# psweens/VAN-GAN

Measured on AMD Instinct MI355X. Metric: train Mvoxels/s (VanGan.train_step, 128^3 bf16), higher is better.
Workload: dtype bf16; 1 GPU; VanGan.train_step, 128x128x128 volumes, batch 1 per GPU (global 1), clDice on, disc noise+dropout on; parallelism=dp1

## Files before the change

### van_gan_amd/csrc/vg_c1k3.h

```cpp
#pragma once
#include "vg_common.h"

struct C1K3 {
    const void* x; int x_f32; float sc, sf; int act, pad_mode;
    int D, H, W, C, W4;
    int td0, th0, tw0;
    const void* w; int Ktot, CK;
    const float* bias; void* out; float* sums;
    const void* dy; float* dw; float* db;
    const float* scale; const float* shift;
    VgFin fin;
};
__device__ __forceinline__ int c1_resolve(int p, int n, int reflect, bool& ok) {
    ok = true;
    if (reflect) { if (p < 0) p = -p; if (p >= n) p = 2 * n - 2 - p; return p < 0 ? 0 : (p >= n ? n - 1 : p); }
    ok = p >= 0 && p < n;
    return ok ? p : 0;
}

struct C1M {
    const void* x; int x_f32; float sc, sf; int act, pad_mode;
    const float* scale; const float* shift;
    const void* noise;
    int D, H, W, OD, OH, OW, C;
    int td0, th0, tw0;
    const void* w; int Ktot, CK;
    const float* bias; void* out; float* sums;
    const void* dy; float* dw; float* db; float* part;
    VgFin fin;
};
int c1m_fwd(const vg_conv_desc* d, hipStream_t s);
int c1m_wgrad(const vg_conv_desc* d, const void* dy, int dy_f32, int T_total, float* dw, float* db, float* scratch, int64_t scratch_bytes, hipStream_t s);
```

### van_gan_amd/csrc/vg_c1k3.hip

```cpp
#include "vg_c1k3.h"

namespace {
constexpr int TW = 16, TD = 4;
constexpr int ROWB = TW * 8 + 8;

typedef __attribute__((ext_vector_type(2))) unsigned u32x2;
typedef __attribute__((ext_vector_type(4))) unsigned u32x4;
typedef __attribute__((ext_vector_type(4))) short s16x4;
typedef __attribute__((ext_vector_type(2))) float f32x2;

template <int KS, int ST, int TH> struct Geo {
    static constexpr int IH = ST * TH + KS - ST, ID = ST * TD + KS - ST;
    static constexpr int NROWS = ID * IH, IMGB = NROWS * ROWB;
    static constexpr int NI = 3 * ST + 4;
    static constexpr int NRT = KS * KS;
};

__device__ __forceinline__ float c1_slope(int act) { return act == VG_ACT_RELU ? 0.f : (act == VG_ACT_LRELU ? VG_LRELU : 1.f); }

template <typename S, int KS, int ST, int TH, bool NOISE>
__device__ __forceinline__ void c1_stage_image(const C1M& p, char* img, int n, int od0, int oh0, int ow0, float sc, float sf, float slope, int tid) {
    typedef Geo<KS, ST, TH> G;
    const bool refl = p.pad_mode == VG_PAD_REFLECT;
    for (int item = tid; item < G::NROWS * 4; item += 256) {
// ... 66 lines not shown
        for (int h = 0; h < 2; ++h) {
            const int t = min(8 * s + 2 * kg + h, G::NRT - 1), a = t / KS, b = t - a * KS;
            boff[s][h] = ((ST * wave + a) * G::IH + b) * ROWB + li * 8;
        }
    const int tiles_w = (p.OW + TW - 1) / TW, tiles_h = (p.OH + TH - 1) / TH, tiles_d = (p.OD + TD - 1) / TD;
    const int ntiles = tiles_w * tiles_h * tiles_d;
    float s1[MT][4], s2[MT][4];
#pragma unroll
    for (int mt = 0; mt < MT; ++mt)
#pragma unroll
        for (int r = 0; r < 4; ++r) { s1[mt][r] = 0.f; s2[mt][r] = 0.f; }
    const int cst = 8 * (kg >> 1), jodd = kg & 1;
    const size_t rowpitch = (size_t)p.OW * C;
    for (int tile = blockIdx.x; tile < ntiles; tile += gridDim.x) {
        const int tw = tile % tiles_w, t2 = tile / tiles_w, th = t2 % tiles_h, td = t2 / tiles_h;
        const int od0 = td * TD, oh0 = th * TH, ow0 = tw * TW;
        __syncthreads();
        c1_stage_image<S, KS, ST, TH, NOISE>(p, img, n, od0, oh0, ow0, sc, sf, slope, tid);
        __syncthreads();
        const int od = od0 + wave, ow = ow0 + li;
        const bool dw_ok = od < p.OD && ow < p.OW;
        T* const obase = (T*)p.out + ((((size_t)n * p.OD + min(od, p.OD - 1)) * p.OH + oh0) * p.OW + min(ow, p.OW - 1)) * C + cst;
#pragma unroll
        for (int mt = 0; mt < MT; ++mt) {
            f32x4 acc[8];
#pragma unroll
            for (int j = 0; j < 8; ++j) {
                const int jo = ST * j * ROWB;
                const u32x2 a0 = *(const u32x2*)(img + boff[0][0] + jo), a1 = *(const u32x2*)(img + boff[0][1] + jo);
                const u32x2 c0 = *(const u32x2*)(img + boff[1][0] + jo), c1 = *(const u32x2*)(img + boff[1][1] + jo);
                const bf16x8 b0 = __builtin_bit_cast(bf16x8, ((u32x4){a0[0], a0[1], a1[0], a1[1]}));
                const bf16x8 b1 = __builtin_bit_cast(bf16x8, ((u32x4){c0[0], c0[1], c1[0], c1[1]}));
                acc[j] = VG_MFMA16(wa[mt][0], b0, ((f32x4){0.f, 0.f, 0.f, 0.f}));
                acc[j] = VG_MFMA16(wa[mt][1], b1, acc[j]);
            }
            T* const optr = obase + 16 * mt;
#pragma unroll
            for (int jp = 0; jp < 8; jp += 2) {
                bf16x4 pk[2];
#pragma unroll
                for (int e = 0; e < 2; ++e) {
                    const int j = jp + e;
                    const bool ok = dw_ok && oh0 + j < p.OH;
                    f32x2 v0 = {acc[j][0], acc[j][1]}, v1 = {acc[j][2], acc[j][3]};
                    v0 += eb[mt][0]; v1 += eb[mt][1];
                    pk[e] = (bf16x4){(short)f2bf(v0[0]), (short)f2bf(v0[1]), (short)f2bf(v1[0]), (short)f2bf(v1[1])};
                    f32x2 q0 = {bf2f((bf16_t)pk[e][0]), bf2f((bf16_t)pk[e][1])}, q1 = {bf2f((bf16_t)pk[e][2]), bf2f((bf16_t)pk[e][3])};
                    if (!ok) { q0 = (f32x2){0.f, 0.f}; q1 = q0; }
                    s1[mt][0] += q0[0]; s1[mt][1] += q0[1]; s1[mt][2] += q1[0]; s1[mt][3] += q1[1];
                    s2[mt][0] += q0[0] * q0[0]; s2[mt][1] += q0[1] * q0[1]; s2[mt][2] += q1[0] * q1[0]; s2[mt][3] += q1[1] * q1[1];
                }
                const u32x2 wa_ = __builtin_bit_cast(u32x2, pk[0]), wb_ = __builtin_bit_cast(u32x2, pk[1]);
                const u32x2 x0 = __builtin_amdgcn_permlane16_swap(wa_[0], wb_[0], false, false);
                const u32x2 x1 = __builtin_amdgcn_permlane16_swap(wa_[1], wb_[1], false, false);
                const u32x4 outv = {x0[0], x1[0], x0[1], x1[1]};
                const int j = jp + jodd;
                if (dw_ok && oh0 + j < p.OH) *(u32x4*)(optr + j * rowpitch) = outv;
            }
        }
    }
    if (!p.sums) return;
#pragma unroll
    for (int mt = 0; mt < MT; ++mt)
#pragma unroll
        for (int r = 0; r < 4; ++r) {
            float a = s1[mt][r], b = s2[mt][r];
#pragma unroll
            for (int o = 1; o < 16; o <<= 1) { a += __shfl_xor(a, o); b += __shfl_xor(b, o); }
            if (li == 0) { atomicAdd(&stat[(16 * mt + 4 * kg + r) * 2], a); atomicAdd(&stat[(16 * mt + 4 * kg + r) * 2 + 1], b); }
        }
    __syncthreads();
    if (tid < 32 * MT) {
        const int stripe = blockIdx.x & (VG_STRIPES - 1);
        atomicAdd(&p.sums[((size_t)stripe * gridDim.y + n) * (2 * C) + tid], stat[tid]);
    }
    if (p.fin.ticket) vg_fin_tail(p.fin, p.sums, gridDim.y, C, gridDim.x * gridDim.y, (int*)img);
}

template <typename S, int KS, int ST, int TH, int NT, bool NOISE>
__global__ __launch_bounds__(256, 2) void c1m_wgrad_kernel(const C1M p) {
    typedef bf16_t T;
    typedef Geo<KS, ST, TH> G;
    constexpr int C = 16 * NT, VB = 2 * C;
    constexpr int DYROW = TW * VB, DYB = TD * TH * DYROW;
    constexpr int MTS = (G::NRT + 1 + 3) / 4;
    constexpr int UPT = DYB / 16 / 256;
    static_assert(MTS * NT * 1024 <= DYB, "the accumulator exchange reuses the dY tile");
    __shared__ __attribute__((aligned(16))) char img[G::IMGB + 16];
    __shared__ __attribute__((aligned(16))) char dyt[DYB];
    const int tid = threadIdx.x, lane = tid & 63, wave = __builtin_amdgcn_readfirstlane(tid >> 6);
    const int n = blockIdx.y;
    const float sc = p.scale ? p.scale[n] : p.sc, sf = p.scale ? p.shift[n] : p.sf, slope = c1_slope(p.act);
    if (tid == 0) {
        const unsigned one = f2bf(1.f);
        *(u32x4*)(img + G::IMGB) = (u32x4){one | (one << 16), one | (one << 16), 0u, 0u};
    }
    const int g = lane >> 4, q = (lane >> 2) & 3, pp = lane & 3;
    const int wq = 8 * (g & 1) + q, yq = g >> 1;
    int aoff[MTS], amove[MTS];
#pragma unroll
    for (int mt = 0; mt < MTS; ++mt) {
        const int r = 4 * mt + pp, a = r / KS, b = r - a * KS;
        amove[mt] = r < G::NRT ? 1 : 0;
        aoff[mt] = r < G::NRT ? ((ST * wave + a) * G::IH + ST * yq + b) * ROWB + wq * 8 : (r == G::NRT ? G::IMGB : G::IMGB + 8);
    }
    const int boff = ((wave * TH + yq) * TW + wq) * VB + pp * 8;
    const int tiles_w = (p.OW + TW - 1) / TW, tiles_h = (p.OH + TH - 1) / TH, tiles_d = (p.OD + TD - 1) / TD;
    const int ntiles = tiles_w * tiles_h * tiles_d;
    f32x4 acc[MTS][NT];
#pragma unroll
    for (int mt = 0; mt < MTS; ++mt)
#pragma unroll
        for (int nt = 0; nt < NT; ++nt) acc[mt][nt] = (f32x4){0.f, 0.f, 0.f, 0.f};
    typedef __attribute__((address_space(3))) s16x4 lds_s4;
    for (int tile = blockIdx.x; tile < ntiles; tile += gridDim.x) {
        const int tw = tile % tiles_w, t2 = tile / tiles_w, th = t2 % tiles_h, td = t2 / tiles_h;
        const int od0 = td * TD, oh0 = th * TH, ow0 = tw * TW;
        f32x4 dv[UPT];
#pragma unroll
        for (int i = 0; i < UPT; ++i) {
            const int u = tid + 256 * i, vox = u / (2 * NT), c16 = u - vox * (2 * NT);
            const int w = vox & 15, y = (vox >> 4) % TH, z = vox / (16 * TH);
            const bool ok = od0 + z < p.OD && oh0 + y < p.OH && ow0 + w < p.OW;
            const T* src = (const T*)p.dy + ((((size_t)n * p.OD + min(od0 + z, p.OD - 1)) * p.OH + min(oh0 + y, p.OH - 1)) * p.OW + min(ow0 + w, p.OW - 1)) * C + c16 * 8;
            dv[i] = *(const __attribute__((address_space(1))) f32x4*)(uintptr_t)src;
            if (!ok) dv[i] = (f32x4){0.f, 0.f, 0.f, 0.f};
        }
        __syncthreads();
        c1_stage_image<S, KS, ST, TH, NOISE>(p, img, n, od0, oh0, ow0, sc, sf, slope, tid);
#pragma unroll
        for (int i = 0; i < UPT; ++i) *(f32x4*)(dyt + (tid + 256 * i) * 16) = dv[i];
        __syncthreads();
#pragma unroll
        for (int s = 0; s < TH / 2; ++s) {
            bf16x8 a[MTS];
#pragma unroll
            for (int mt = 0; mt < MTS; ++mt) {
                const int o = aoff[mt] + amove[mt] * (s * 2 * ST * ROWB);
                const s16x4 lo = __builtin_amdgcn_ds_read_tr16_b64_v4i16((lds_s4*)(img + o));
                const s16x4 hi = __builtin_amdgcn_ds_read_tr16_b64_v4i16((lds_s4*)(img + o + amove[mt] * 32));
                a[mt] = (bf16x8){lo[0], lo[1], lo[2], lo[3], hi[0], hi[1], hi[2], hi[3]};
            }
#pragma unroll
            for (int nt = 0; nt < NT; ++nt) {
                const s16x4 lo = __builtin_amdgcn_ds_read_tr16_b64_v4i16((lds_s4*)(dyt + boff + s * 2 * DYROW + nt * 32));
                const s16x4 hi = __builtin_amdgcn_ds_read_tr16_b64_v4i16((lds_s4*)(dyt + boff + s * 2 * DYROW + nt * 32 + 4 * VB));
                const bf16x8 b = {lo[0], lo[1], lo[2], lo[3], hi[0], hi[1], hi[2], hi[3]};
#pragma unroll
                for (int mt = 0; mt < MTS; ++mt) acc[mt][nt] = VG_MFMA16(a[mt], b, acc[mt][nt]);
            }
        }
    }
    float* red = (float*)dyt;
    __syncthreads();
    for (int i = tid; i < MTS * NT * 256; i += 256) red[i] = 0.f;
    __syncthreads();
#pragma unroll
    for (int mt = 0; mt < MTS; ++mt)
#pragma unroll
        for (int nt = 0; nt < NT; ++nt)
#pragma unroll
            for (int e = 0; e < 4; ++e) atomicAdd(&red[((mt * NT + nt) * 4 + e) * 64 + lane], acc[mt][nt][e]);
    __syncthreads();
    float* slab = p.part ? p.part + ((size_t)blockIdx.y * gridDim.x + blockIdx.x) * (KS * KS * KS * C) : nullptr;
    for (int i = tid; i < MTS * NT * 256; i += 256) {
        const int l = i & 63, e = (i >> 6) & 3, t = i >> 8, nt = t % NT, mt = t / NT;
        const int r = 4 * mt + (l >> 4), co = 16 * nt + (l & 15);
        const float v = red[i];
        if (r < G::NRT && e < KS) {
            const int idx = (r * KS + e) * C + co;
            if (slab) slab[idx] = v; else atomicAdd(&p.dw[idx], v);
        } else if (r == G::NRT && e == 0 && p.db) atomicAdd(&p.db[co], v);
    }
}
}

static bool c1m_fill(const vg_conv_desc* d, C1M& p) {
    if (!vg_tune("C1M", 1) || d->f32 || d->out_f32 || d->c_src0 != 1 || d->src1 || d->c_src1 || d->nclass > 1) return false;
    const int KS = d->wpack;
    if (KS != 3 && KS != 4) return false;
    if (d->istr != KS - 2 || d->ntaps != KS * KS || d->Cout != (KS == 3 ? 16 : 64)) return false;
    for (int t = 0; t < KS * KS; ++t)
        if (d->tap_d[t] != d->tap_d[0] + t / KS || d->tap_h[t] != d->tap_h[0] + t % KS || d->tap_w[t] != 0) return false;
    if (d->noise && !(d->noise_pad == 1 && d->pad_mode == VG_PAD_REFLECT)) return false;
    if (d->D < 2 || d->H < 2 || d->W < 2 || d->OD < 1 || d->OH < 1 || d->OW < 1) return false;
    p = C1M{};
    p.x = d->src0; p.x_f32 = d->src_f32; p.sc = 1.f; p.sf = 0.f; p.scale = d->in_scale; p.shift = d->in_shift; p.act = d->act;
    p.pad_mode = d->pad_mode; p.noise = d->noise;
    p.D = d->D; p.H = d->H; p.W = d->W; p.OD = d->OD; p.OH = d->OH; p.OW = d->OW; p.C = d->Cout;
    p.td0 = d->tap_d[0]; p.th0 = d->tap_h[0]; p.tw0 = d->wpack_wmin;
    p.w = d->wpacked; p.CK = d->CK; p.Ktot = ((KS * KS * d->CK + 31) / 32) * 32;
    return true;
}
static dim3 c1m_grid(const C1M& c, int N, int th, int per_cu) {
    const int64_t tiles = (int64_t)((c.OD + TD - 1) / TD) * ((c.OH + th - 1) / th) * ((c.OW + TW - 1) / TW);
    int64_t b = (int64_t)256 * per_cu / (N > 0 ? N : 1);
    if (b > tiles) b = tiles;
    if (b < 1) b = 1;
    return dim3((unsigned)b, (unsigned)N);
}

template <typename S, int KS, int MT>
static void c1m_launch_fwd(const C1M& c, dim3 grid, hipStream_t s) {
    if (c.noise) hipLaunchKernelGGL((c1m_fwd_kernel<S, KS, KS - 2, MT, true>), grid, dim3(256), 0, s, c);
    else hipLaunchKernelGGL((c1m_fwd_kernel<S, KS, KS - 2, MT, false>), grid, dim3(256), 0, s, c);
}
int c1m_fwd(const vg_conv_desc* d, hipStream_t s) {
    C1M c;
    if (!c1m_fill(d, c)) return 1;
    c.bias = d->bias; c.out = d->out; c.sums = d->out_sums; c.fin = vg_fin_of(d);
    const int KS = d->wpack;
    if (vg_dry("c1m_fwd<%s,%d,%d,%d,n%d>", d->src_f32 ? "f32" : "bf16", KS, KS - 2, c.C / 16, c.noise ? 1 : 0)) return VG_OK;
    const dim3 grid = c1m_grid(c, d->N, 8, vg_tune("C1M_FWD_WGS", KS == 3 ? 4 : 2));
    if (KS == 3) { if (d->src_f32) c1m_launch_fwd<float, 3, 1>(c, grid, s); else c1m_launch_fwd<bf16_t, 3, 1>(c, grid, s); }
    else { if (d->src_f32) c1m_launch_fwd<float, 4, 4>(c, grid, s); else c1m_launch_fwd<bf16_t, 4, 4>(c, grid, s); }
    if (c.sums && c.fin.ticket) vg_fin_done = true;
    return vg_check_launch();
}

template <typename S, int KS, int TH, int NT>
static void c1m_launch_wgrad(const C1M& c, dim3 grid, hipStream_t s) {
    if (c.noise) hipLaunchKernelGGL((c1m_wgrad_kernel<S, KS, KS - 2, TH, NT, true>), grid, dim3(256), 0, s, c);
    else hipLaunchKernelGGL((c1m_wgrad_kernel<S, KS, KS - 2, TH, NT, false>), grid, dim3(256), 0, s, c);
}
int c1m_wgrad(const vg_conv_desc* d, const void* dy, int dy_f32, int T_total, float* dw, float* db, float* scratch, int64_t scratch_bytes, hipStream_t s) {
    C1M c;
    if (dy_f32 || !vg_tune("C1M_WGRAD", 1) || !c1m_fill(d, c)) return 1;
    const int KS = d->wpack;
    if (T_total != KS * KS) return 1;
    c.dy = dy; c.dw = dw; c.db = db;
    const int th = KS == 3 ? 8 : 4;
    const dim3 grid = c1m_grid(c, d->N, th, vg_tune("C1M_WGRAD_WGS", KS == 3 ? 2 : 1));
    const int nslab = (int)(grid.x * grid.y), dw_elems = KS * KS * KS * c.C;
    c.part = (nslab > 4 && scratch && (int64_t)nslab * dw_elems * 4 <= scratch_bytes && vg_tune("C1M_WGRAD_PART", 1)) ? scratch : nullptr;
    if (vg_dry("c1m_wgrad<%s,%d,%d,%d,n%d>|part%d", d->src_f32 ? "f32" : "bf16", KS, KS - 2, c.C / 16, c.noise ? 1 : 0, c.part ? 1 : 0)) return VG_OK;
    if (KS == 3) { if (d->src_f32) c1m_launch_wgrad<float, 3, 8, 1>(c, grid, s); else c1m_launch_wgrad<bf16_t, 3, 8, 1>(c, grid, s); }
    else { if (d->src_f32) c1m_launch_wgrad<float, 4, 4, 4>(c, grid, s); else c1m_launch_wgrad<bf16_t, 4, 4, 4>(c, grid, s); }
    if (c.part) vg_launch_reduce_partials(c.part, nslab, dw_elems, dw, s);
    return vg_check_launch();
}

namespace {
__global__ __launch_bounds__(256) void cell_pack_kernel(const float* __restrict__ w, int C, int Ktot, bf16_t* __restrict__ out) {
    const size_t total = (size_t)64 * Ktot;
    for (size_t i = (size_t)blockIdx.x * 256 + threadIdx.x; i < total; i += (size_t)gridDim.x * 256) {
        const int row = (int)(i / Ktot), k = (int)(i % Ktot);
        const int chunk = k / 448, kl = k % 448, tap = kl / 16, ch = chunk * 16 + (kl & 15);
        float v = 0.f;
        if (row < 8 && tap < 27 && ch < C) {
            const int nd = tap / 9, nh = (tap / 3) % 3, nw = tap % 3;
            const int td = ((row >> 2) & 1) + 2 - 2 * nd, th = ((row >> 1) & 1) + 2 - 2 * nh, tw = (row & 1) + 2 - 2 * nw;
            if (td >= 0 && th >= 0 && tw >= 0) v = w[(size_t)((td * 4 + th) * 4 + tw) * C + ch];
        }
        out[i] = f2bf(v);
    }
}
__global__ __launch_bounds__(256) void cells_fold_kernel(const bf16_t* __restrict__ cells, int D, int H, int W, float* __restrict__ dx) {
    const int n = blockIdx.y;
    const int CD = D / 2 + 1, CH = H / 2 + 1, CW = W / 2 + 1;
    const bf16_t* cb = cells + (size_t)n * CD * CH * CW * 16;
    const int64_t total = (int64_t)D * H * W;
    for (int64_t i = (int64_t)blockIdx.x * 256 + threadIdx.x; i < total; i += (int64_t)gridDim.x * 256) {
        const int iw = (int)(i % W); const int64_t r = i / W; const int ih = (int)(r % H), id = (int)(r / H);
        int pd[2], ph[2], pw[2], nd = 1, nh = 1, nw = 1;
        pd[0] = id + 1; ph[0] = ih + 1; pw[0] = iw + 1;
        if (id == 1) pd[nd++] = 0; else if (id == D - 2) pd[nd++] = D + 1;
        if (ih == 1) ph[nh++] = 0; else if (ih == H - 2) ph[nh++] = H + 1;
        if (iw == 1) pw[nw++] = 0; else if (iw == W - 2) pw[nw++] = W + 1;
        float s = 0.f;
        for (int a = 0; a < nd; ++a)
            for (int b = 0; b < nh; ++b)
                for (int c = 0; c < nw; ++c) {
                    const int qd = pd[a], qh = ph[b], qw = pw[c];
                    s += bf2f(cb[(((size_t)(qd >> 1) * CH + (qh >> 1)) * CW + (qw >> 1)) * 16 + ((qd & 1) * 4 + (qh & 1) * 2 + (qw & 1))]);
                }
        dx[(size_t)n * total + i] = s;
    }
}
}

extern "C" int vg_pack_cell_weights(const float* w, int C, void* out, vg_stream_t stream) {
    vg_begin();
    if (!w || !out || C < 16 || (C % 16)) return VG_EINVAL;
    const int Ktot = (C / 16) * 448;
    hipLaunchKernelGGL(cell_pack_kernel, dim3((64 * Ktot + 255) / 256), dim3(256), 0, (hipStream_t)stream, w, C, Ktot, (bf16_t*)out);
    return vg_check_launch();
}
extern "C" int vg_cells_fold(const void* cells, int N, int D, int H, int W, float* dx, vg_stream_t stream) {
    vg_begin();
    if (!cells || !dx || N < 1 || D < 4 || H < 4 || W < 4 || ((D | H | W) & 1)) return VG_EINVAL;
    int64_t b = ((int64_t)D * H * W + 255) / 256;
    if (b > 2047 / N) b = 2047 / N > 0 ? 2047 / N : 1;
    hipLaunchKernelGGL(cells_fold_kernel, dim3((unsigned)b, (unsigned)N), dim3(256), 0, (hipStream_t)stream, (const bf16_t*)cells, D, H, W, dx);
    return vg_check_launch();
}
```

### van_gan_amd/csrc/vg_common.h

```cpp
#pragma once
#include <hip/hip_runtime.h>
#include <stdint.h>
#include "../../include/vangan_hip.h"

typedef __attribute__((ext_vector_type(8))) short bf16x8;
typedef __attribute__((ext_vector_type(4))) short bf16x4;
typedef __attribute__((ext_vector_type(4))) float f32x4;
typedef unsigned short bf16_t;

#define VG_LDS_LIMIT 163840
#define VG_LRELU 0.2f

#ifdef VG_FP16
typedef __attribute__((ext_vector_type(8))) _Float16 vg_h8;
__device__ __forceinline__ float bf2f(bf16_t h) { return (float)__builtin_bit_cast(_Float16, h); }
__device__ __forceinline__ bf16_t f2bf(float f) { return __builtin_bit_cast(unsigned short, (_Float16)f); }
#define VG_MFMA16(a, b, c) __builtin_amdgcn_mfma_f32_16x16x32_f16(__builtin_bit_cast(vg_h8, a), __builtin_bit_cast(vg_h8, b), c, 0, 0, 0)
#define VG_MFMA32(a, b, c) __builtin_amdgcn_mfma_f32_32x32x16_f16(__builtin_bit_cast(vg_h8, a), __builtin_bit_cast(vg_h8, b), c, 0, 0, 0)
#define VG_STORAGE16 "fp16"
#else
__device__ __forceinline__ float bf2f(bf16_t h) { return __uint_as_float(((unsigned)h) << 16); }
__device__ __forceinline__ bf16_t f2bf(float f) {
    __bf16 b = (__bf16)f;
    return __builtin_bit_cast(unsigned short, b);
}
#define VG_MFMA16(a, b, c) __builtin_amdgcn_mfma_f32_16x16x32_bf16(a, b, c, 0, 0, 0)
#define VG_MFMA32(a, b, c) __builtin_amdgcn_mfma_f32_32x32x16_bf16(a, b, c, 0, 0, 0)
#define VG_STORAGE16 "bf16"
#endif
__device__ __forceinline__ float bfround(float f) { return bf2f(f2bf(f)); }

template <typename T> __device__ __forceinline__ void load8(const T* p, float* o);
template <> __device__ __forceinline__ void load8<bf16_t>(const bf16_t* p, float* o) {
    const bf16x8 r = *(const bf16x8*)p;
#pragma unroll
    for (int j = 0; j < 8; ++j) o[j] = bf2f((bf16_t)r[j]);
}
template <> __device__ __forceinline__ void load8<float>(const float* p, float* o) {
    const f32x4 a = *(const f32x4*)p, b = *(const f32x4*)(p + 4);
    o[0] = a[0]; o[1] = a[1]; o[2] = a[2]; o[3] = a[3]; o[4] = b[0]; o[5] = b[1]; o[6] = b[2]; o[7] = b[3];
}
template <typename T> __device__ __forceinline__ void store8(T* p, const float* v);
template <> __device__ __forceinline__ void store8<bf16_t>(bf16_t* p, const float* v) {
    bf16x8 r;
#pragma unroll
    for (int j = 0; j < 8; ++j) r[j] = (short)f2bf(v[j]);
    *(bf16x8*)p = r;
}
template <> __device__ __forceinline__ void store8<float>(float* p, const float* v) {
    *(f32x4*)p = (f32x4){v[0], v[1], v[2], v[3]}; *(f32x4*)(p + 4) = (f32x4){v[4], v[5], v[6], v[7]};
}
template <typename T> __device__ __forceinline__ float ld1(const T* p);
template <> __device__ __forceinline__ float ld1<bf16_t>(const bf16_t* p) { return bf2f(*p); }
template <> __device__ __forceinline__ float ld1<float>(const float* p) { return *p; }
template <typename T> __device__ __forceinline__ void st1(T* p, float v);
template <> __device__ __forceinline__ void st1<bf16_t>(bf16_t* p, float v) { *p = f2bf(v); }
template <> __device__ __forceinline__ void st1<float>(float* p, float v) { *p = v; }
template <typename T> __device__ __forceinline__ float rnd(float v);
template <> __device__ __forceinline__ float rnd<bf16_t>(float v) { return bfround(v); }
template <> __device__ __forceinline__ float rnd<float>(float v) { return v; }

__device__ __forceinline__ float vg_act(float x, int act) {
    if (act == VG_ACT_RELU) return fmaxf(x, 0.f);
    if (act == VG_ACT_LRELU) return x > 0.f ? x : VG_LRELU * x;
    return x;
}
__device__ __forceinline__ float vg_act_grad(float pre, int act) {
    if (act == VG_ACT_RELU) return pre > 0.f ? 1.f : 0.f;
    if (act == VG_ACT_LRELU) return pre > 0.f ? 1.f : VG_LRELU;
    return 1.f;
}

__device__ __forceinline__ float wave_sum(float v) {
#pragma unroll
    for (int o = 32; o > 0; o >>= 1) v += __shfl_xor(v, o);
    return v;
}
__device__ __forceinline__ float wave_min(float v) {
#pragma unroll
    for (int o = 32; o > 0; o >>= 1) v = fminf(v, __shfl_xor(v, o));
    return v;
}
__device__ __forceinline__ float wave_max(float v) {
#pragma unroll
    for (int o = 32; o > 0; o >>= 1) v = fmaxf(v, __shfl_xor(v, o));
    return v;
}

struct VgFin { unsigned* ticket; float count, eps; int njobs; vg_fin_job job[2]; };
static inline VgFin vg_fin_of(const vg_conv_desc* d) {
    VgFin f; f.ticket = nullptr; f.count = 1.f; f.eps = 0.f; f.njobs = 0;
    if (d->fin && d->out_sums) { f.ticket = d->fin->ticket; f.count = d->fin->count; f.eps = d->fin->eps; f.njobs = d->fin->njobs;
                                 f.job[0] = d->fin->job[0]; f.job[1] = d->fin->job[d->fin->njobs > 1 ? 1 : 0]; }
    return f;
}
__device__ __forceinline__ void vg_fin_one(const VgFin& f, float s, float ss, int n, int c) {
    const float mean = s / f.count;
    float var = ss / f.count - mean * mean;
    var = var < 0.f ? 0.f : var;
    const float rstd = rsqrtf(var + f.eps);
    for (int j = 0; j < f.njobs; ++j) {
        const vg_fin_job& q = f.job[j];
        const int cc = q.c_off + c, i = n * q.c_tot + cc;
        float sc = (q.gamma ? q.gamma[cc] : 1.f) * rstd;
        float sh = (q.beta ? q.beta[cc] : 0.f) - mean * sc;
        if (q.mult) { const float m = q.mult[i]; sc *= m; sh *= m; }
        q.scale[i] = sc; q.shift[i] = sh;
        if (q.mean) q.mean[i] = mean;
        if (q.rstd) q.rstd[i] = rstd;
    }
}
__device__ __forceinline__ void vg_fin_tail(const VgFin& f, const float* sums, int N, int C, unsigned nblocks, int* flag) {
    asm volatile("s_waitcnt vmcnt(0)" ::: "memory");
    __syncthreads();
    if (threadIdx.x == 0)
        *flag = __hip_atomic_fetch_add(f.ticket, 1u, __ATOMIC_RELAXED, __HIP_MEMORY_SCOPE_AGENT) == nblocks - 1u ? 1 : 0;
    __syncthreads();
    if (!*flag) return;
    for (int i = threadIdx.x; i < N * C; i += blockDim.x) {
        const int n = i / C, c = i - n * C;
        float s = 0.f, ss = 0.f;
        for (int t = 0; t < VG_STRIPES; ++t) {
            const float* p = sums + (((size_t)t * N + n) * C + c) * 2;
            s += __hip_atomic_load(p, __ATOMIC_RELAXED, __HIP_MEMORY_SCOPE_AGENT);
            ss += __hip_atomic_load(p + 1, __ATOMIC_RELAXED, __HIP_MEMORY_SCOPE_AGENT);
        }
        vg_fin_one(f, s, ss, n, c);
    }
}
int vg_launch_fin(const vg_conv_desc* d, hipStream_t s);
extern thread_local bool vg_fin_done;

int vg_tune(const char* key, int dflt);
bool vg_dry(const char* fmt, ...) __attribute__((format(printf, 1, 2)));
void vg_dry_begin(char* buf, int n);
void vg_dry_end();

bool vg_dry_on();
static inline void vg_begin() { (void)hipGetLastError(); }
static inline int vg_check_launch() {
    hipError_t e = hipGetLastError();
    return e == hipSuccess ? VG_OK : VG_ELAUNCH;
}
int vg_pointwise_conv(const vg_conv_desc* d, hipStream_t s);
int vg_pointwise_wgrad(const vg_conv_desc* d, const void* dy, int dy_f32, int T_total, float* dw, float* db, float* scratch,
                       int64_t scratch_bytes, hipStream_t s);
int vg_wgrad_dma(const vg_conv_desc* d, const void* dy, int dy_f32, const int32_t* tap_idx_host, int T_total, float* dw, float* db,
                 float* scratch, int64_t scratch_bytes, hipStream_t s);
int vg_wgrad_pw_dma(const vg_conv_desc* d, const void* dy, int dy_f32, int T_total, float* dw, float* db, float* scratch,
                    int64_t scratch_bytes, hipStream_t s);
int vg_wgrad_thin(const vg_conv_desc* d, const void* dy, int dy_f32, const int32_t* tap_idx_host, int T_total, float* dw, float* db,
                  float* scratch, int64_t scratch_bytes, hipStream_t s);
int vg_conv_dma(const vg_conv_desc* d, hipStream_t s, bool* did_stats = nullptr);
void vg_launch_reduce_partials(const float* part, int nb, int n, float* dw, hipStream_t s);
static inline int ilog2_exact(int v) { int l = 0; while ((1 << l) < v) ++l; return l; }
static inline int pow2_ceil(int v) { int p = 1; while (p < v) p <<= 1; return p; }
static inline int64_t cdiv64(int64_t a, int64_t b) { return (a + b - 1) / b; }

template <typename T> struct Raw8;
template <> struct Raw8<bf16_t> { bf16x8 v; };
template <> struct Raw8<float> { f32x4 a, b; };
__device__ __forceinline__ void raw_load(Raw8<bf16_t>& r, const bf16_t* p) { r.v = *(const __attribute__((address_space(1))) bf16x8*)(uintptr_t)p; }
__device__ __forceinline__ void raw_load(Raw8<float>& r, const float* p) {
    const __attribute__((address_space(1))) f32x4* q = (const __attribute__((address_space(1))) f32x4*)(uintptr_t)p;
    r.a = q[0]; r.b = q[1];
}
__device__ __forceinline__ void raw_unpack(const Raw8<bf16_t>& r, float* o) {
#pragma unroll
    for (int j = 0; j < 8; ++j) o[j] = bf2f((bf16_t)r.v[j]);
}
__device__ __forceinline__ void raw_unpack(const Raw8<float>& r, float* o) {
    o[0] = r.a[0]; o[1] = r.a[1]; o[2] = r.a[2]; o[3] = r.a[3]; o[4] = r.b[0]; o[5] = r.b[1]; o[6] = r.b[2]; o[7] = r.b[3];
}


__device__ __forceinline__ void raw_pin(Raw8<bf16_t>& r) { asm volatile("" : "+v"(r.v)); }
__device__ __forceinline__ void raw_pin(Raw8<float>& r) { asm volatile("" : "+v"(r.a), "+v"(r.b)); }
__device__ __forceinline__ void raw_mask(Raw8<bf16_t>& r, bool keep) { if (!keep) r.v = (bf16x8){0, 0, 0, 0, 0, 0, 0, 0}; }
__device__ __forceinline__ void raw_mask(Raw8<float>& r, bool keep) { if (!keep) { r.a = (f32x4){0.f, 0.f, 0.f, 0.f}; r.b = r.a; } }

__device__ __forceinline__ float ld_global(const float* p) { return *(const __attribute__((address_space(1))) float*)(uintptr_t)p; }
__device__ __forceinline__ float ld_global(const bf16_t* p) { return bf2f(*(const __attribute__((address_space(1))) bf16_t*)(uintptr_t)p); }
```

### van_gan_amd/csrc/vg_pointwise.hip

```cpp
#include "vg_common.h"
#include "vg_c1k3.h"
#include <stdlib.h>

namespace {

struct PW {
    const void* x; int x_f32;
    const float* scale; const float* shift; int act;
    const void* w; int kc_pad, CK;
    const float* bias;
    void* out; int out_f32, accumulate, tanh_out;
    float* sums;
    const void* dy; int dy_f32;
    float* dw; float* db;
    int N, C; int64_t S;
    VgFin fin;
};

__device__ __forceinline__ float pw_slope(int act) { return act == VG_ACT_RELU ? 0.f : (act == VG_ACT_LRELU ? VG_LRELU : 1.f); }
__device__ __forceinline__ float ld_single(const void* p, int f32, int64_t i) {
    return f32 ? ld_global((const float*)p + i) : ld_global((const bf16_t*)p + i);
}

template <typename T, int G>
// ... 334 lines not shown
                Raw8<bf16_t> t;
                raw_load(t, q);
                raw_mask(t, cok);
                xb[i][ks] = t.v;
            }
        if (p.stamps) { asm volatile("s_waitcnt vmcnt(0)" ::: "memory"); if (lane == 0) p.stamps[((size_t)blockIdx.x * 4 + wave) * 8 + 2] = __builtin_amdgcn_s_memrealtime(); }
        if constexpr (SPLIT == 2) {
            const int PH = p.OH + 2, PW_ = p.OW + 2;
            size_t gi[MS / 2], li[MS / 2], si[MS / 2];
            bool bord[MS / 2];
#pragma unroll
            for (int jh = 0; jh < MS / 2; ++jh) {
                const int fd = fdhw[jh] & 1023, fh = (fdhw[jh] >> 10) & 1023, fw = fdhw[jh] >> 20;
                gi[jh] = ((((size_t)n * (p.OD + 2) + fd + 1) * PH + fh + 1) * PW_ + fw + 1) * p.Cout + chof;
                li[jh] = ((((size_t)n * (p.OD >> 1) + (fd >> 1)) * (p.OH >> 1) + (fh >> 1)) * (p.OW >> 1) + (fw >> 1)) * p.sc0 + chof;
                si[jh] = ovf[jh] * (p.Cout - p.sc0) + chof;
                bord[jh] = fd == 1 || fd == p.OD - 2 || fh == 1 || fh == p.OH - 2 || fw == 1 || fw == p.OW - 2;
            }
            constexpr int C = NB * 16;
            const float slope = pw_slope(p.n_act);
            Raw8<bf16_t> gq[NB][MS / 2], xq[NB][MS / 2];
#pragma unroll
            for (int nb = 0; nb < NB; ++nb)
#pragma unroll
                for (int jh = 0; jh < MS / 2; ++jh) {
                    raw_load(gq[nb][jh], p.ng + gi[jh] + nb * 16);
                    raw_load(xq[nb][jh], nb * 16 < p.sc0 ? p.nx0 + li[jh] + nb * 16 : p.nx1 + si[jh] + (nb * 16 - p.sc0));
                }
#pragma unroll
            for (int nb = 0; nb < NB; ++nb) {
                f32x4 a[MS];
#pragma unroll
                for (int i = 0; i < MS; ++i) {
                    a[i] = (f32x4){0.f, 0.f, 0.f, 0.f};
#pragma unroll
                    for (int ks = 0; ks < KS; ++ks) a[i] = VG_MFMA16(wA[nb][ks], xb[i][ks], a[i]);
                }
                const float* tb = ntab + nb * 16 + chof;
#pragma unroll
                for (int jp = 0; jp < MS; jp += 2) {
                    float o[8];
#pragma unroll
                    for (int i = 0; i < 4; ++i) {
                        const pw_u32x2 x = __builtin_amdgcn_permlane16_swap(__float_as_uint(a[jp][i]), __float_as_uint(a[jp + 1][i]), false, false);
                        o[i] = __uint_as_float(x[0]); o[4 + i] = __uint_as_float(x[1]);
                    }
                    float q[8], xv[8];
                    raw_unpack(gq[nb][jp >> 1], q); raw_unpack(xq[nb][jp >> 1], xv);
                    if (bord[jp >> 1]) {
                        const int fd = fdhw[jp >> 1] & 1023, fh = (fdhw[jp >> 1] >> 10) & 1023, fw = fdhw[jp >> 1] >> 20;
                        vg_reflect_fold8(p.ng + (size_t)n * (p.OD + 2) * PH * PW_ * p.Cout + nb * 16 + chof, p.Cout, p.OD, p.OH, p.OW, fd, fh, fw, q);
                    }
#pragma unroll
                    for (int i = 0; i < 8; ++i) {
                        const float pre = xv[i] * tb[i] + tb[C + i];
                        const float m = (pre > 0.f || p.n_act == VG_ACT_NONE) ? 1.f : slope;
                        o[i] += tb[2 * C + i] * m * q[i] - tb[3 * C + i] - tb[4 * C + i] * xv[i];
                    }
                    split_store(wt, jp, nb, o, oks[jp >> 1], ovf[jp >> 1]);
                }
                __builtin_amdgcn_sched_barrier(0);
            }
            continue;
        }
        f32x4 acc[MS][NB];
#pragma unroll
        for (int i = 0; i < MS; ++i)
#pragma unroll
            for (int nb = 0; nb < NB; ++nb) {
                acc[i][nb] = (f32x4){0.f, 0.f, 0.f, 0.f};
#pragma unroll
                for (int ks = 0; ks < KS; ++ks) acc[i][nb] = VG_MFMA16(wA[nb][ks], xb[i][ks], acc[i][nb]);
            }
#pragma unroll
        for (int jp = 0; jp < MS; jp += 2) {
            const bool ok = oks[jp >> 1];
            const size_t ob = ovs[jp >> 1];
#pragma unroll
            for (int nb = 0; nb < NB; ++nb) {
                if (nb * 16 >= p.Cout) continue;
                bf16_t* optr = p.out + ob + nb * 16;
                pw_u32x4 outv;
                if (ACC) {
                    float o[8];
#pragma unroll
                    for (int i = 0; i < 4; ++i) {
                        const pw_u32x2 x = __builtin_amdgcn_permlane16_swap(__float_as_uint(acc[jp][nb][i] + e_b[nb][i >> 1][i & 1]),
                                                                            __float_as_uint(acc[jp + 1][nb][i] + e_b[nb][i >> 1][i & 1]), false, false);
                        o[i] = __uint_as_float(x[0]); o[4 + i] = __uint_as_float(x[1]);
                    }
                    float q[8]; raw_unpack(oldv[ACC ? jp >> 1 : 0][ACC ? nb : 0], q);
                    if (SPLIT) {
#pragma unroll
                        for (int i = 0; i < 8; ++i) o[i] += q[i];
                        split_store(wt, jp, nb, o, ok, ovf[jp >> 1]);
                        continue;
                    }
                    bf16x8 pk;
#pragma unroll
                    for (int i = 0; i < 8; ++i) pk[i] = (short)f2bf(o[i] + q[i]);
                    outv = __builtin_bit_cast(pw_u32x4, pk);
                } else {
                    bf16x4 pk[2];
#pragma unroll
                    for (int e = 0; e < 2; ++e) {
                        pw_f32x2 v0 = {acc[jp + e][nb][0], acc[jp + e][nb][1]}, v1 = {acc[jp + e][nb][2], acc[jp + e][nb][3]};
                        v0 += e_b[nb][0]; v1 += e_b[nb][1];
                        pk[e] = (bf16x4){(short)f2bf(v0[0]), (short)f2bf(v0[1]), (short)f2bf(v1[0]), (short)f2bf(v1[1])};
                        if (STATS) {
                            const bool okv = vok[jp + e];
#pragma unroll
                            for (int i = 0; i < 4; ++i) {
                                const float qv = okv ? bf2f((bf16_t)pk[e][i]) : 0.f;
                                s1[nb][i] += qv; s2[nb][i] += qv * qv;
                            }
                        }
                    }
                    const pw_u32x2 wa = __builtin_bit_cast(pw_u32x2, pk[0]), wb = __builtin_bit_cast(pw_u32x2, pk[1]);
                    const pw_u32x2 x0 = __builtin_amdgcn_permlane16_swap(wa[0], wb[0], false, false);
                    const pw_u32x2 x1 = __builtin_amdgcn_permlane16_swap(wa[1], wb[1], false, false);
                    outv = (pw_u32x4){x0[0], x1[0], x0[1], x1[1]};
                }
                if (ok) *(pw_u32x4*)optr = outv;
            }
        }
    }
    if (p.stamps && lane == 0) { asm volatile("s_waitcnt vmcnt(0)" ::: "memory"); p.stamps[((size_t)blockIdx.x * 4 + wave) * 8 + 7] = __builtin_amdgcn_s_memrealtime(); }
    if (STATS && p.sums) {
#pragma unroll
        for (int nb = 0; nb < NB; ++nb)
#pragma unroll
            for (int i = 0; i < 4; ++i) {
                float a = s1[nb][i], b = s2[nb][i];
#pragma unroll
                for (int o = 1; o < 16; o <<= 1) { a += __shfl_xor(a, o); b += __shfl_xor(b, o); }
                if (r == 0) { atomicAdd(&stat[(nb * 16 + 4 * kg + i) * 2], a); atomicAdd(&stat[(nb * 16 + 4 * kg + i) * 2 + 1], b); }
            }
        __syncthreads();
        if (tid < NB * 32) {
            const int co = tid >> 1;
            const int stripe = blockIdx.x & (VG_STRIPES - 1);
            if (co < p.Cout) atomicAdd(&p.sums[(((size_t)stripe * gridDim.y + n) * p.Cout + co) * 2 + (tid & 1)], stat[tid]);
        }
        if (p.fin.ticket) vg_fin_tail(p.fin, p.sums, gridDim.y, p.Cout, gridDim.x * gridDim.y, (int*)stat);
    }
}

struct PWW {
    const bf16_t* x0; const bf16_t* x1; int c0, c1, Cin, sh;
    const bf16_t* dy; int Cout;
    int N, ID, IH, IW, OD, OH, OW, istr, SO;
    int gin, roles, rp, vpb;
    float* dw; float* db; float* part; int dw_elems;
};

__global__ __launch_bounds__(256) void pw_wgrad_cc_kernel(const PWW p) {
    __shared__ float red[4 * 64 * 16];
    const int tid = threadIdx.x, n = blockIdx.y;
    const int role = tid & (p.rp - 1), vl = tid / p.rp;
    const bool live = role < p.roles;
    const int rl = live ? role : 0;
    const int cg = rl % p.gin, cob = rl / p.gin, c = cg * 8;
    const bool from0 = c < p.c0;
    const float bmask = cg == 0 ? 1.f : 0.f;
    pw_f32x2 acc[8][8], bs[8];
#pragma unroll
    for (int i = 0; i < 8; ++i) {
        bs[i] = (pw_f32x2){0.f, 0.f};
#pragma unroll
        for (int j = 0; j < 8; ++j) acc[i][j] = (pw_f32x2){0.f, 0.f};
    }
    const int ID2 = p.ID >> p.sh, IH2 = p.IH >> p.sh, IW2 = p.IW >> p.sh;
    const int step = gridDim.x * p.vpb;
    int v = blockIdx.x * p.vpb + vl;
    const int OHW = p.OH * p.OW;
    int od = v / OHW, oh = (v - od * OHW) / p.OW, ow = v - od * OHW - oh * p.OW;
    const int sd = step / OHW, sh_ = (step - sd * OHW) / p.OW, sw = step - sd * OHW - sh_ * p.OW;
    const bf16_t* xb = from0 ? p.x0 + c : p.x1 + (c - p.c0);
    const int cs = from0 ? p.c0 : p.c1, shx = from0 ? p.sh : 0;
    const int XD = from0 ? ID2 : p.ID, XH = from0 ? IH2 : p.IH, XW = from0 ? IW2 : p.IW;
    const bf16_t* yb = p.dy + (size_t)n * p.SO * p.Cout + cob * 16;
    if (live)
    for (; v < p.SO; v += 2 * step) {
        Raw8<bf16_t> xr[2], yr[2][2]; bool okv[2];
#pragma unroll
        for (int k = 0; k < 2; ++k) {
            const int vk = v + k * step;
            okv[k] = vk < p.SO;
            const int dq = okv[k] ? od : 0, hq = okv[k] ? oh : 0, wq = okv[k] ? ow : 0, vq = okv[k] ? vk : 0;
            const size_t xi = (((size_t)n * XD + ((dq * p.istr) >> shx)) * XH + ((hq * p.istr) >> shx)) * XW + ((wq * p.istr) >> shx);
            raw_load(xr[k], xb + xi * cs);
            raw_load(yr[k][0], yb + (size_t)vq * p.Cout);
            raw_load(yr[k][1], yb + (size_t)vq * p.Cout + 8);
            ow += sw; if (ow >= p.OW) { ow -= p.OW; ++oh; }
            oh += sh_; if (oh >= p.OH) { oh -= p.OH; ++od; }
            od += sd;
        }
#pragma unroll
        for (int k = 0; k < 2; ++k) {
            float x[8], y[16];
            raw_unpack(xr[k], x); raw_unpack(yr[k][0], y); raw_unpack(yr[k][1], y + 8);
            pw_f32x2 y2[8];
#pragma unroll
            for (int j = 0; j < 8; ++j) y2[j] = okv[k] ? (pw_f32x2){y[2 * j], y[2 * j + 1]} : (pw_f32x2){0.f, 0.f};
#pragma unroll
            for (int i = 0; i < 8; ++i) {
                const pw_f32x2 xi2 = {x[i], x[i]};
#pragma unroll
                for (int j = 0; j < 8; ++j) acc[i][j] += xi2 * y2[j];
            }
            const pw_f32x2 bm = {bmask, bmask};
#pragma unroll
            for (int j = 0; j < 8; ++j) bs[j] += y2[j] * bm;
        }
    }
    for (int off = 32; off >= p.rp; off >>= 1) {
#pragma unroll
        for (int j = 0; j < 8; ++j) {
            bs[j][0] += __shfl_xor(bs[j][0], off); bs[j][1] += __shfl_xor(bs[j][1], off);
#pragma unroll
            for (int i = 0; i < 8; ++i) { acc[i][j][0] += __shfl_xor(acc[i][j][0], off); acc[i][j][1] += __shfl_xor(acc[i][j][1], off); }
        }
    }
    float* slab = p.part ? p.part + (size_t)(blockIdx.y * gridDim.x + blockIdx.x) * p.dw_elems : nullptr;
    const int lane = tid & 63, wave = tid >> 6;
#pragma unroll
    for (int ch = 0; ch < 9; ++ch) {
        __syncthreads();
        if (lane < p.rp) {
            float* dst = red + (size_t)(wave * p.rp + lane) * 16;
#pragma unroll
            for (int j = 0; j < 8; ++j) {
                const pw_f32x2 val = ch < 8 ? acc[ch < 8 ? ch : 0][j] : bs[j];
                dst[2 * j] = val[0]; dst[2 * j + 1] = val[1];
            }
        }
        __syncthreads();
        for (int o = tid; o < p.rp * 16; o += 256) {
            const int ro = o >> 4, i = o & 15;
            if (ro >= p.roles) continue;
            const float sacc = red[o] + red[p.rp * 16 + o] + red[2 * p.rp * 16 + o] + red[3 * p.rp * 16 + o];
            const int rcg = ro % p.gin, rcob = ro / p.gin, co = rcob * 16 + i;
            if (ch < 8) {
                const size_t idx = (size_t)(rcg * 8 + ch) * p.Cout + co;
                if (slab) slab[idx] = sacc; else atomicAdd(&p.dw[idx], sacc);
            } else if (rcg == 0 && p.db) atomicAdd(&p.db[co], sacc);
        }
    }
}

template <typename T, bool MULTI_X>
__global__ __launch_bounds__(256) void pw_wgrad_kernel(const PW p) {
    __shared__ float part[16 * 256];
    const int n = blockIdx.y, tid = threadIdx.x;
    const int gpc = p.C >> 3, vpb = 256 / gpc;
    const int cg = tid % gpc, vl = tid / gpc;
    const bool live = tid < gpc * vpb;
    float a[8], bsum[8], sc[8], sf[8];
#pragma unroll
    for (int j = 0; j < 8; ++j) {
        a[j] = 0.f; bsum[j] = 0.f;
        const int ci = MULTI_X ? n * p.C + cg * 8 + j : n;
        sc[j] = (p.scale && live) ? p.scale[ci] : 1.f; sf[j] = (p.scale && live) ? p.shift[ci] : 0.f;
    }
    const float slope = pw_slope(p.act);
    const T* mb = (const T*)(MULTI_X ? p.x : p.dy) + (size_t)n * p.S * p.C + cg * 8;
    const void* sb = MULTI_X ? p.dy : p.x;
    const int sb_f32 = MULTI_X ? p.dy_f32 : p.x_f32;
    const int64_t soff = (int64_t)n * p.S;
    const int64_t stride = (int64_t)gridDim.x * vpb;
    if (live)
    for (int64_t v = (int64_t)blockIdx.x * vpb + vl; v < p.S; v += 4 * stride) {
        Raw8<T> m[4]; float sv[4];
#pragma unroll
        for (int k = 0; k < 4; ++k) {
            const int64_t vv = v + k * stride < p.S ? v + k * stride : v;
            raw_load(m[k], mb + vv * p.C);
            sv[k] = ld_single(sb, sb_f32, soff + vv);
        }
#pragma unroll
        for (int k = 0; k < 4; ++k) {
            if (v + k * stride >= p.S) continue;
            float q[8]; raw_unpack(m[k], q);
            if (MULTI_X) {
                const float g = rnd<T>(sv[k]);
#pragma unroll
                for (int j = 0; j < 8; ++j) { float y = q[j] * sc[j] + sf[j]; y = rnd<T>(fmaxf(y, y * slope)); a[j] += y * g; }
                bsum[0] += g;
            } else {
                float y = sv[k] * sc[0] + sf[0]; y = rnd<T>(fmaxf(y, y * slope));
#pragma unroll
                for (int j = 0; j < 8; ++j) { a[j] += y * q[j]; bsum[j] += q[j]; }
            }
        }
    }
#pragma unroll
    for (int j = 0; j < 8; ++j) { part[(2 * j) * 256 + tid] = live ? a[j] : 0.f; part[(2 * j + 1) * 256 + tid] = live ? bsum[j] : 0.f; }
    __syncthreads();
    for (int o = tid; o < p.C * 2; o += 256) {
        const int ch = o >> 1, mom = o & 1, g8 = ch >> 3, j = ch & 7;
        const float* src = part + (2 * j + mom) * 256 + g8;
        float s = 0.f;
        for (int t = 0; t < vpb; ++t) s += src[t * gpc];
        if (mom == 0) atomicAdd(&p.dw[ch], s);
        else if (p.db) {
            if (!MULTI_X) atomicAdd(&p.db[ch], s);
            else if (ch == 0) {
                atomicAdd(&p.db[0], s);
            }
        }
    }
}

template <typename T, typename S, int NA>
__device__ __forceinline__ void c1_window(const C1K3& p, int n, int d, int h, int w0, int a0, float (&xv)[NA][3][6]) {
    const bool refl = p.pad_mode == VG_PAD_REFLECT;
    const float slope = pw_slope(p.act);
    int cw[6]; bool okw[6];
#pragma unroll
    for (int i = 0; i < 6; ++i) cw[i] = c1_resolve(w0 + p.tw0 + i, p.W, refl, okw[i]);
    const int64_t base = (int64_t)n * p.D * p.H * p.W;
#pragma unroll
    for (int a = 0; a < NA; ++a) {
        bool okd; const int rd = c1_resolve(d + p.td0 + a0 + a, p.D, refl, okd);
#pragma unroll
        for (int b = 0; b < 3; ++b) {
            bool okh; const int rh = c1_resolve(h + p.th0 + b, p.H, refl, okh);
            const int64_t row = base + ((int64_t)rd * p.H + rh) * p.W;
#pragma unroll
            for (int i = 0; i < 6; ++i) xv[a][b][i] = ld_global((const S*)p.x + row + cw[i]);
#pragma unroll
            for (int i = 0; i < 6; ++i) {
                float y = xv[a][b][i] * p.sc + p.sf;
                y = rnd<T>(fmaxf(y, y * slope));
                xv[a][b][i] = (okd && okh && okw[i]) ? y : 0.f;
            }
        }
    }
}

template <typename T, typename S>
__global__ __launch_bounds__(256, 3) void c1k3_fwd_kernel(C1K3 p) {
    __shared__ float wl[27 * 32];
    __shared__ float part[16 * 256];
    const int n = blockIdx.y, tid = threadIdx.x;
    const int gpc = p.C >> 3, qpb = 256 / gpc;
    const int cg = tid % gpc, ql = tid / gpc;
    const bool live = tid < gpc * qpb;
    if (p.scale) { p.sc = p.scale[n]; p.sf = p.shift[n]; }
    for (int i = tid; i < 27 * p.C; i += 256) {
        const int co = i % p.C, tj = i / p.C, t = tj / 3, j = tj - t * 3;
        wl[i] = ld1<T>((const T*)p.w + (size_t)co * p.Ktot + t * p.CK + j);
    }
    __syncthreads();
    float bv[8], s1[8], s2[8];
#pragma unroll
    for (int j = 0; j < 8; ++j) { bv[j] = (live && p.bias) ? p.bias[cg * 8 + j] : 0.f; s1[j] = 0.f; s2[j] = 0.f; }
    const int64_t nq = (int64_t)p.D * p.H * p.W4;
    if (live)
    for (int64_t q = (int64_t)blockIdx.x * qpb + ql; q < nq; q += (int64_t)gridDim.x * qpb) {
        const int wq = (int)(q % p.W4); const int64_t r = q / p.W4;
        const int h = (int)(r % p.H), d = (int)(r / p.H), w0 = wq * 4;
        float acc[4][8];
#pragma unroll
        for (int v = 0; v < 4; ++v)
#pragma unroll
            for (int j = 0; j < 8; ++j) acc[v][j] = bv[j];
#pragma unroll 1
        for (int a = 0; a < 3; ++a) {
            float xv[1][3][6];
            c1_window<T, S, 1>(p, n, d, h, w0, a, xv);
#pragma unroll
            for (int b = 0; b < 3; ++b)
#pragma unroll
                for (int j = 0; j < 3; ++j) {
                    const float* wp = wl + ((a * 3 + b) * 3 + j) * p.C + cg * 8;
                    const f32x4 w0v = *(const f32x4*)wp, w1v = *(const f32x4*)(wp + 4);
#pragma unroll
                    for (int v = 0; v < 4; ++v) {
                        const float x = xv[0][b][v + j];
                        acc[v][0] += x * w0v[0]; acc[v][1] += x * w0v[1]; acc[v][2] += x * w0v[2]; acc[v][3] += x * w0v[3];
                        acc[v][4] += x * w1v[0]; acc[v][5] += x * w1v[1]; acc[v][6] += x * w1v[2]; acc[v][7] += x * w1v[3];
                    }
                }
        }
        T* ob = (T*)p.out + (((size_t)n * p.D + d) * p.H + h) * p.W * p.C + cg * 8;
#pragma unroll
        for (int v = 0; v < 4; ++v) {
            if (w0 + v >= p.W) continue;
            store8<T>(ob + (size_t)(w0 + v) * p.C, acc[v]);
#pragma unroll
            for (int j = 0; j < 8; ++j) { const float rr = rnd<T>(acc[v][j]); s1[j] += rr; s2[j] += rr * rr; }
        }
    }
    if (!p.sums) return;
#pragma unroll
    for (int j = 0; j < 8; ++j) { part[(2 * j) * 256 + tid] = live ? s1[j] : 0.f; part[(2 * j + 1) * 256 + tid] = live ? s2[j] : 0.f; }
    __syncthreads();
    const int stripe = blockIdx.x & (VG_STRIPES - 1);
    float* dst = p.sums + ((size_t)stripe * gridDim.y + n) * p.C * 2;
    for (int o = tid; o < p.C * 2; o += 256) {
// ... 47 lines not shown
                for (int c = 0; c < 8; ++c) acc[72 + c] += g[c];
            }
        }
    }
#pragma unroll
    for (int chunk = 0; chunk < 4; ++chunk) {
        __syncthreads();
#pragma unroll
        for (int i = 0; i < 20; ++i) part[i * 256 + tid] = live ? acc[chunk * 20 + i] : 0.f;
        __syncthreads();
        for (int o = tid; o < roles * 20; o += 256) {
            const int i = o / roles, ro = o - i * roles;
            const float* src = part + i * 256 + ro;
            float sacc = 0.f;
            for (int t = 0; t < qpb; ++t) sacc += src[t * roles];
            const int val = chunk * 20 + i, rcg = ro % gpc, ra = ro / gpc;
            if (val < 72) {
                const int b = val / 24, j = (val / 8) % 3, c = val & 7;
                atomicAdd(&p.dw[(size_t)(((ra * 3 + b) * 3) + j) * p.C + rcg * 8 + c], sacc);
            } else if (ra == 0 && p.db) atomicAdd(&p.db[rcg * 8 + (val - 72)], sacc);
        }
    }
}

bool c1k3_fill(const vg_conv_desc* d, C1K3& p) {
    if (d->c_src0 != 1 || d->src1 || d->c_src1 || d->wpack != 3 || d->ntaps != 9 || d->istr != 1 || d->noise || d->nclass > 1) return false;
    if (d->Cout < 8 || d->Cout > 32 || (d->Cout % 8)) return false;
    if (d->OD != d->D || d->OH != d->H || d->OW != d->W) return false;
    for (int t = 0; t < 9; ++t)
        if (d->tap_d[t] != d->tap_d[0] + t / 3 || d->tap_h[t] != d->tap_h[0] + t % 3 || d->tap_w[t] != 0) return false;
    p.x = d->src0; p.x_f32 = d->src_f32; p.sc = 1.f; p.sf = 0.f; p.scale = d->in_scale; p.shift = d->in_shift; p.act = d->act;
    p.pad_mode = d->pad_mode; p.D = d->D; p.H = d->H; p.W = d->W; p.C = d->Cout; p.W4 = (d->W + 3) / 4;
    p.td0 = d->tap_d[0]; p.th0 = d->tap_h[0]; p.tw0 = d->wpack_wmin;
    p.CK = d->CK; p.Ktot = ((9 * d->CK + 31) / 32) * 32;
    return true;
}

bool pw_enabled() { return vg_tune("PW", 1) != 0; }
bool pw_shape_ok(const vg_conv_desc* d) {
    if (!pw_enabled() || d->ntaps != 1 || d->tap_d[0] || d->tap_h[0] || d->tap_w[0]) return false;
    if (d->istr != 1 || d->src1 || d->c_src1 || d->src0_shift || d->noise || d->wpack || d->nclass > 1) return false;
    if (d->OD != d->D || d->OH != d->H || d->OW != d->W) return false;
    return true;
}
int pw_blocks(int64_t work_items, int N) {
    int64_t b = (work_items + 255) / 256;
    const int64_t cap = 2047 / (N > 0 ? N : 1);
    if (b > cap) b = cap;
    return b < 1 ? 1 : (int)b;
}

template <bool GEO, bool ACC, bool STATS>
bool pwg_launch(int KS, int NB, dim3 grid, hipStream_t s, const PWG& p) {
#define PWG_CASE(ks, nb) if (KS == ks && NB == nb) { hipLaunchKernelGGL((pw_gemm_kernel<ks, nb, GEO, ACC, STATS>), grid, dim3(256), 0, s, p); return true; }
    PWG_CASE(1, 1) PWG_CASE(1, 2) PWG_CASE(1, 3) PWG_CASE(1, 4) PWG_CASE(1, 6) PWG_CASE(2, 1) PWG_CASE(2, 2) PWG_CASE(3, 2)
    PWG_CASE(4, 4) PWG_CASE(6, 4) PWG_CASE(2, 8)
#undef PWG_CASE
    return false;
}
template <int SPLIT>
bool pwg_launch_split(int KS, int NB, dim3 grid, hipStream_t s, const PWG& p) {
#define PWG_CASE(ks, nb) if (KS == ks && NB == nb) { hipLaunchKernelGGL((pw_gemm_kernel<ks, nb, false, true, false, SPLIT>), grid, dim3(256), 0, s, p); return true; }
    PWG_CASE(1, 3) PWG_CASE(1, 6) PWG_CASE(2, 6)
#undef PWG_CASE
    return false;
}
bool pwg_case_ok(int KS, int NB) {
    static const int tab[][2] = {{1, 1}, {1, 2}, {1, 3}, {1, 4}, {1, 6}, {2, 1}, {2, 2}, {3, 2}, {4, 4}, {6, 4}, {2, 8}};
    for (auto& t : tab) if (t[0] == KS && t[1] == NB) return true;
    return false;
}
int pw_gemm_conv(const vg_conv_desc* d, hipStream_t s) {
    if (!pw_enabled() || !vg_tune("PW_GEMM", 1)) return 1;
    if (d->ntaps != 1 || d->tap_d[0] || d->tap_h[0] || d->tap_w[0] || d->noise || d->wpack || d->nclass > 1) return 1;
    if (d->f32 || d->src_f32 || d->out_f32 || d->in_scale || d->act != VG_ACT_NONE || d->res || d->tanh_out) return 1;
    const int Cin = d->c_src0 + d->c_src1;
    if (Cin < 8 || (Cin % 8) || (d->c_src1 && (d->c_src0 % 8)) || d->Cout < 16 || (d->Cout % 16) || (d->CK % 8)) return 1;
    if (d->c_src1 && !d->src1) return 1;
    if (d->src0_shift && ((d->D | d->H | d->W) & 1)) return 1;
    if (d->istr < 1 || d->ostr < 1 || (d->OD - 1) * d->istr >= d->D || (d->OH - 1) * d->istr >= d->H || (d->OW - 1) * d->istr >= d->W) return 1;
    if (d->accumulate && d->out_sums) return 1;
    const int64_t SO = (int64_t)d->OD * d->OH * d->OW;
    if (SO < 1 || SO > (1 << 30)) return 1;
    const int KS = (Cin + 31) / 32, NB = d->Cout / 16;
    if (!pwg_case_ok(KS, NB)) return 1;
    const bool geo = d->src0_shift || d->istr != 1 || d->ostr != 1 || d->ooff_d || d->ooff_h || d->ooff_w || d->BD != d->OD || d->BH != d->OH
                     || d->BW != d->OW || d->OD != d->D || d->OH != d->H || d->OW != d->W;
    PWG p = {};
    p.x0 = (const bf16_t*)d->src0; p.x1 = (const bf16_t*)(d->c_src1 ? d->src1 : d->src0); p.c0 = d->c_src0; p.c1 = d->c_src1 ? d->c_src1 : 1;
    p.Cin = Cin; p.sh = d->src0_shift ? 1 : 0;
    p.w = (const bf16_t*)d->wpacked; p.CK = d->CK; p.kc_pad = ((d->CK + 31) / 32) * 32; p.Ktot = ((Cin + d->CK - 1) / d->CK) * p.kc_pad;
    p.bias = d->bias; p.out = (bf16_t*)d->out; p.sums = d->out_sums;
    p.N = d->N; p.ID = d->D; p.IH = d->H; p.IW = d->W; p.OD = d->OD; p.OH = d->OH; p.OW = d->OW; p.istr = d->istr;
    p.BD = d->BD; p.BH = d->BH; p.BW = d->BW; p.ostr = d->ostr; p.od0 = d->ooff_d; p.oh0 = d->ooff_h; p.ow0 = d->ooff_w;
    p.Cout = d->Cout; p.SO = (int)SO; p.stamps = g_vg_stamps;
    p.fin = vg_fin_of(d);
    const int MS = (KS * NB <= 2) ? 4 : 2;
    const int64_t nwt = (SO + MS * 16 - 1) / (MS * 16);
    int64_t b = (nwt + 3) / 4;
    const int capt = vg_tune("PW_GEMM_CAP", 2047);
    const int64_t cap = (capt / d->N) > 0 ? (capt / d->N) : 1;
    if (b > cap) b = cap;
    const dim3 grid((int)b, d->N);
    if (vg_dry("pw_gemm<%d,%d,g%d,a%d>", KS, NB, (geo || !d->accumulate) ? 1 : 0, d->accumulate ? 1 : 0)) return VG_OK;
    bool ok;
    if (!d->accumulate) { ok = pwg_launch<true, false, true>(KS, NB, grid, s, p); if (ok && p.sums && p.fin.ticket) vg_fin_done = true; }
    else ok = geo ? pwg_launch<true, true, false>(KS, NB, grid, s, p) : pwg_launch<false, true, false>(KS, NB, grid, s, p);
    return ok ? vg_check_launch() : 1;
}

int pw_gemm_split(const vg_conv_desc* d, const vg_actnorm_bwd_desc* nb_, void* dlow, void* dskip, int c_low, int acc, hipStream_t s) {
    if (!pw_enabled() || !vg_tune("PW_GEMM", 1) || !vg_tune("PW_SPLIT", 1)) return 1;
    if (d->ntaps != 1 || d->tap_d[0] || d->tap_h[0] || d->tap_w[0] || d->noise || d->wpack || d->nclass > 1) return 1;
    if (d->f32 || d->src_f32 || d->out_f32 || d->in_scale || d->act != VG_ACT_NONE || d->res || d->tanh_out || d->out_sums || d->bias) return 1;
    const int Cin = d->c_src0;
    if (d->c_src1 || d->src0_shift || Cin < 8 || (Cin % 8) || d->Cout < 32 || (d->Cout % 16) || (d->CK % 8) || (!d->accumulate && !nb_)) return 1;
    if (nb_) {
        if (!nb_->norm || !nb_->g_padded || nb_->f32 || nb_->x_f32 || !nb_->g || !nb_->x || !nb_->x1 || !nb_->x0_shift || nb_->c_x0 != c_low) return 1;
        if (nb_->C != d->Cout || nb_->N != d->N || nb_->D != d->D || nb_->H != d->H || nb_->W != d->W || !nb_->gamma || !nb_->mean || !nb_->rstd || !nb_->red) return 1;
        if (d->D < 4 || d->H < 4 || d->W < 4 || d->D > 1023 || d->H > 1023 || d->W > 1023) return 1;
    }
    if (c_low < 16 || (c_low % 16) || c_low >= d->Cout) return 1;
    if (d->istr != 1 || d->ostr != 1 || d->ooff_d || d->ooff_h || d->ooff_w || d->BD != d->OD || d->BH != d->OH || d->BW != d->OW
        || d->OD != d->D || d->OH != d->H || d->OW != d->W || ((d->D | d->H | d->W) & 1)) return 1;
    const int64_t SO = (int64_t)d->OD * d->OH * d->OW;
    if (SO < 8 || SO > (1 << 30)) return 1;
    const int KS = (Cin + 31) / 32, NB = d->Cout / 16;
    if (!((KS == 1 && (NB == 3 || NB == 6)) || (KS == 2 && NB == 6))) return 1;
    PWG p = {};
    p.x0 = (const bf16_t*)d->src0; p.x1 = p.x0; p.c0 = Cin; p.c1 = 1; p.Cin = Cin; p.sh = 0;
    p.w = (const bf16_t*)d->wpacked; p.CK = d->CK; p.kc_pad = ((d->CK + 31) / 32) * 32; p.Ktot = ((Cin + d->CK - 1) / d->CK) * p.kc_pad;
    p.bias = nullptr; p.out = (bf16_t*)d->out; p.sums = nullptr;
    p.N = d->N; p.ID = d->D; p.IH = d->H; p.IW = d->W; p.OD = d->OD; p.OH = d->OH; p.OW = d->OW; p.istr = 1;
    p.BD = d->BD; p.BH = d->BH; p.BW = d->BW; p.ostr = 1;
    p.Cout = d->Cout; p.SO = (int)SO; p.stamps = g_vg_stamps;
    p.dlow = (bf16_t*)dlow; p.dskip = (bf16_t*)dskip; p.sc0 = c_low; p.sacc = acc;
    if (nb_) {
        p.ng = (const bf16_t*)nb_->g; p.nx0 = (const bf16_t*)nb_->x; p.nx1 = (const bf16_t*)nb_->x1;
        p.n_scale = nb_->scale; p.n_shift = nb_->shift; p.n_mean = nb_->mean; p.n_rstd = nb_->rstd; p.n_gamma = nb_->gamma; p.n_mult = nb_->mult;
        p.n_red = nb_->red; p.n_dgamma = (nb_->dgamma && nb_->dbeta) ? nb_->dgamma : nullptr; p.n_dbeta = nb_->dbeta; p.n_act = nb_->act;
    }
    const int MS = (KS * NB <= 2) ? 4 : 2;
    const int64_t nwt = (SO + MS * 16 - 1) / (MS * 16);
    int64_t b = (nwt + 3) / 4;
    const int capt = vg_tune("PW_GEMM_CAP", 2047);
    const int64_t cap = (capt / d->N) > 0 ? (capt / d->N) : 1;
    if (b > cap) b = cap;
    if (vg_dry("pw_gemm_split<%d,%d,n%d>", KS, NB, nb_ ? 1 : 0)) return VG_OK;
    const bool ok = nb_ ? pwg_launch_split<2>(KS, NB, dim3((int)b, d->N), s, p) : pwg_launch_split<1>(KS, NB, dim3((int)b, d->N), s, p);
    return ok ? vg_check_launch() : 1;
}

int pw_wgrad_cc(const vg_conv_desc* d, const void* dy, int dy_f32, int T_total, float* dw, float* db, float* scratch,
                int64_t scratch_bytes, hipStream_t s) {
    if (!pw_enabled() || !vg_tune("PW_WGRAD_CC", 1)) return 1;
    if (T_total != 1 || d->ntaps != 1 || d->tap_d[0] || d->tap_h[0] || d->tap_w[0] || d->noise || d->wpack || d->nclass > 1) return 1;
    if (d->f32 || d->src_f32 || dy_f32 || d->in_scale || d->act != VG_ACT_NONE) return 1;
    const int Cin = d->c_src0 + d->c_src1;
    if (Cin < 8 || (Cin % 8) || (d->c_src1 && (d->c_src0 % 8)) || d->Cout < 16 || (d->Cout % 16)) return 1;
    if (d->c_src1 && !d->src1) return 1;
    if (d->src0_shift && ((d->D | d->H | d->W) & 1)) return 1;
    if (d->istr < 1 || (d->OD - 1) * d->istr >= d->D || (d->OH - 1) * d->istr >= d->H || (d->OW - 1) * d->istr >= d->W) return 1;
    const int64_t SO = (int64_t)d->OD * d->OH * d->OW;
    if (SO < 1 || SO > (1 << 30)) return 1;
    PWW p = {};
    p.gin = Cin / 8; p.roles = p.gin * (d->Cout / 16);
    if (p.roles > vg_tune("PW_WGRAD_ROLES", 16)) return 1;
    p.rp = pow2_ceil(p.roles); p.vpb = 256 / p.rp;
    p.x0 = (const bf16_t*)d->src0; p.x1 = (const bf16_t*)(d->c_src1 ? d->src1 : d->src0); p.c0 = d->c_src0; p.c1 = d->c_src1 ? d->c_src1 : 1;
    p.Cin = Cin; p.sh = d->src0_shift ? 1 : 0; p.dy = (const bf16_t*)dy; p.Cout = d->Cout;
    p.N = d->N; p.ID = d->D; p.IH = d->H; p.IW = d->W; p.OD = d->OD; p.OH = d->OH; p.OW = d->OW; p.istr = d->istr; p.SO = (int)SO;
    p.dw = dw; p.db = db; p.dw_elems = Cin * d->Cout;
    int64_t b = (SO + (int64_t)p.vpb * 8 - 1) / ((int64_t)p.vpb * 8);
    const int capt = vg_tune("PW_WGRAD_CAP", 511);
    const int64_t cap = (capt / d->N) > 0 ? (capt / d->N) : 1;
    if (b > cap) b = cap;
    if (b < 1) b = 1;
    const int nslab = (int)b * d->N;
    p.part = (nslab > 4 && scratch && (int64_t)nslab * p.dw_elems * 4 <= scratch_bytes) ? scratch : nullptr;
    if (vg_dry("pw_wgrad_cc<r%d>|part%d", p.roles, p.part ? 1 : 0)) return VG_OK;
    hipLaunchKernelGGL(pw_wgrad_cc_kernel, dim3((int)b, d->N), dim3(256), 0, s, p);
    if (p.part) vg_launch_reduce_partials(p.part, nslab, p.dw_elems, dw, s);
    return vg_check_launch();
}

}

extern "C" int vg_shortcut_dgrad_concat(const vg_conv_desc* d, void* dlow, void* dskip, int c_low, int accumulate, vg_stream_t stream) {
    vg_begin();
    if (!d || !d->src0 || !d->out || !d->wpacked || !dlow || !dskip) return VG_EINVAL;
    return pw_gemm_split(d, nullptr, dlow, dskip, c_low, accumulate, (hipStream_t)stream);
}
extern "C" int vg_shortcut_dgrad_concat_norm(const vg_conv_desc* d, const vg_actnorm_bwd_desc* b, void* dlow, void* dskip, int c_low,
                                             int accumulate, vg_stream_t stream) {
    vg_begin();
    if (!d || !b || !d->src0 || !d->wpacked || !dlow || !dskip) return VG_EINVAL;
    if (!vg_tune("PW_SPLIT_NORM", 1)) return 1;
    return pw_gemm_split(d, b, dlow, dskip, c_low, accumulate, (hipStream_t)stream);
}

int vg_pointwise_conv(const vg_conv_desc* d, hipStream_t s) {
    if (pw_enabled() && !d->res && !d->tanh_out && !d->accumulate && d->ostr == 1 && !d->ooff_d && !d->ooff_h && !d->ooff_w
        && d->BD == d->OD && d->BH == d->OH && d->BW == d->OW && !(d->out_f32 && !d->f32)) {
        { const int mrc = c1m_fwd(d, s); if (mrc <= 0) return mrc; }
        C1K3 c;
        if (c1k3_fill(d, c)) {
            c.w = d->wpacked; c.bias = d->bias; c.out = d->out; c.sums = d->out_sums;
            c.fin = vg_fin_of(d);
            const int qpb = 256 / (c.C >> 3);
            int64_t b = ((int64_t)c.D * c.H * c.W4 + qpb - 1) / qpb;
            const int64_t cap = (2047 / d->N) > 0 ? (2047 / d->N) : 1;
            if (b > cap) b = cap;
            const dim3 grid((int)b, d->N);
            if (vg_dry("c1k3_fwd<%s,%s>", d->f32 ? "f32" : "bf16", d->src_f32 ? "f32" : "bf16")) return VG_OK;
            if (d->f32) {
                if (d->src_f32) hipLaunchKernelGGL((c1k3_fwd_kernel<float, float>), grid, dim3(256), 0, s, c);
                else hipLaunchKernelGGL((c1k3_fwd_kernel<float, bf16_t>), grid, dim3(256), 0, s, c);
            } else {
                if (d->src_f32) hipLaunchKernelGGL((c1k3_fwd_kernel<bf16_t, float>), grid, dim3(256), 0, s, c);
                else hipLaunchKernelGGL((c1k3_fwd_kernel<bf16_t, bf16_t>), grid, dim3(256), 0, s, c);
            }
            if (c.sums && c.fin.ticket) vg_fin_done = true;
            return vg_check_launch();
        }
    }
    { const int grc = pw_gemm_conv(d, s); if (grc <= 0) return grc; }
    if (!pw_shape_ok(d) || d->res) return 1;
    if (d->ostr != 1 || d->ooff_d || d->ooff_h || d->ooff_w || d->BD != d->OD || d->BH != d->OH || d->BW != d->OW) return 1;
    if (d->tanh_out && d->accumulate) return 1;
    const int Cin = d->c_src0;
    PW p = {};
    p.x = d->src0; p.x_f32 = d->src_f32; p.scale = d->in_scale; p.shift = d->in_shift; p.act = d->act;
    p.w = d->wpacked; p.CK = d->CK; p.kc_pad = ((d->CK + 31) / 32) * 32;
    p.bias = d->bias; p.out = d->out; p.out_f32 = (d->out_f32 || d->f32) ? 1 : 0; p.accumulate = d->accumulate; p.tanh_out = d->tanh_out;
    p.sums = d->out_sums; p.N = d->N; p.S = (int64_t)d->D * d->H * d->W;
    if (d->Cout == 1 && Cin >= 8 && Cin <= 32 && (Cin % 8) == 0) {
        p.C = Cin;
        const dim3 grid(pw_blocks((p.S + 1) / 2, d->N), d->N);
        if (vg_dry("pw_cto1<%s,%d>", d->f32 ? "f32" : "bf16", Cin / 8 > 4 ? 4 : Cin / 8)) return VG_OK;
#define PW_CTO1(T)                                                                                                      \
        switch (Cin / 8) {                                                                                              \
            case 1: hipLaunchKernelGGL((pw_cto1_kernel<T, 1>), grid, dim3(256), 0, s, p); break;                        \
            case 2: hipLaunchKernelGGL((pw_cto1_kernel<T, 2>), grid, dim3(256), 0, s, p); break;                        \
            case 3: hipLaunchKernelGGL((pw_cto1_kernel<T, 3>), grid, dim3(256), 0, s, p); break;                        \
            default: hipLaunchKernelGGL((pw_cto1_kernel<T, 4>), grid, dim3(256), 0, s, p); break;                       \
        }
        if (d->f32) { PW_CTO1(float) } else { PW_CTO1(bf16_t) }
#undef PW_CTO1
        return vg_check_launch();
    }
    if (Cin == 1 && d->Cout >= 8 && d->Cout <= 256 && (d->Cout % 8) == 0 && !d->tanh_out && !(d->out_f32 && !d->f32)) {
        p.C = d->Cout;
        p.kc_pad = ((d->CK + 31) / 32) * 32;
        const int vpb = 256 / (p.C >> 3);
        const dim3 grid(pw_blocks((p.S + 3) / 4 * (256 / vpb), d->N), d->N);
        if (vg_dry("pw_1toc<%s>", d->f32 ? "f32" : "bf16")) return VG_OK;
        p.fin = vg_fin_of(d);
        if (d->f32) hipLaunchKernelGGL((pw_1toc_kernel<float>), grid, dim3(256), 0, s, p);
        else hipLaunchKernelGGL((pw_1toc_kernel<bf16_t>), grid, dim3(256), 0, s, p);
        if (p.sums && p.fin.ticket) vg_fin_done = true;
        return vg_check_launch();
    }
    if ((Cin == 8 || Cin == 16) && d->Cout >= 16 && d->Cout <= 128 && (d->Cout % 8) == 0 && !d->in_scale && d->act == VG_ACT_NONE
        && !d->tanh_out && !d->out_sums && !d->src_f32 && !(d->out_f32 && !d->f32)) {
        p.C = d->Cout;
        const int nchunks = (Cin + d->CK - 1) / d->CK;
        const int Ktot = nchunks * p.kc_pad;
        const int vpb = 256 / (p.C >> 3);
        const dim3 grid(pw_blocks((p.S + 1) / 2 * (256 / vpb), d->N), d->N);
        if (vg_dry("pw_ctoc<%s,%d>", d->f32 ? "f32" : "bf16", Cin / 8)) return VG_OK;
        if (d->f32) {
            if (Cin == 8) hipLaunchKernelGGL((pw_ctoc_kernel<float, 1>), grid, dim3(256), 0, s, p, Cin, Ktot);
            else hipLaunchKernelGGL((pw_ctoc_kernel<float, 2>), grid, dim3(256), 0, s, p, Cin, Ktot);
        } else {
            if (Cin == 8) hipLaunchKernelGGL((pw_ctoc_kernel<bf16_t, 1>), grid, dim3(256), 0, s, p, Cin, Ktot);
            else hipLaunchKernelGGL((pw_ctoc_kernel<bf16_t, 2>), grid, dim3(256), 0, s, p, Cin, Ktot);
        }
        return vg_check_launch();
    }
    return 1;
}

int vg_pointwise_wgrad(const vg_conv_desc* d, const void* dy, int dy_f32, int T_total, float* dw, float* db, float* scratch,
                       int64_t scratch_bytes, hipStream_t s) {
    if (pw_enabled()) { const int mrc = c1m_wgrad(d, dy, dy_f32, T_total, dw, db, scratch, scratch_bytes, s); if (mrc <= 0) return mrc; }
    if (pw_enabled() && T_total == 9 && !(dy_f32 && !d->f32)) {
        C1K3 c;
        if (c1k3_fill(d, c)) {
            c.dy = dy; c.dw = dw; c.db = db;
            const int qpb = 256 / (3 * (c.C >> 3));
            int64_t b = ((int64_t)c.D * c.H * c.W4 + (int64_t)qpb * 8 - 1) / ((int64_t)qpb * 8);
            const int64_t cap = (767 / d->N) > 0 ? (767 / d->N) : 1;
            if (b > cap) b = cap;
            if (b < 1) b = 1;
            const dim3 grid((int)b, d->N);
            if (vg_dry("c1k3_wgrad<%s,%s>", d->f32 ? "f32" : "bf16", d->src_f32 ? "f32" : "bf16")) return VG_OK;
            if (d->f32) {
                if (d->src_f32) hipLaunchKernelGGL((c1k3_wgrad_kernel<float, float>), grid, dim3(256), 0, s, c);
                else hipLaunchKernelGGL((c1k3_wgrad_kernel<float, bf16_t>), grid, dim3(256), 0, s, c);
            } else {
                if (d->src_f32) hipLaunchKernelGGL((c1k3_wgrad_kernel<bf16_t, float>), grid, dim3(256), 0, s, c);
                else hipLaunchKernelGGL((c1k3_wgrad_kernel<bf16_t, bf16_t>), grid, dim3(256), 0, s, c);
            }
            return vg_check_launch();
        }
    }
    { const int wrc = pw_wgrad_cc(d, dy, dy_f32, T_total, dw, db, scratch, scratch_bytes, s); if (wrc <= 0) return wrc; }
    if (!pw_shape_ok(d) || T_total != 1) return 1;
    const int Cin = d->c_src0;
    PW p = {};
    p.x = d->src0; p.x_f32 = d->src_f32; p.scale = d->in_scale; p.shift = d->in_shift; p.act = d->act;
    p.dy = dy; p.dy_f32 = dy_f32; p.dw = dw; p.db = db; p.N = d->N; p.S = (int64_t)d->D * d->H * d->W;
    const bool c_to_1 = d->Cout == 1 && Cin >= 8 && Cin <= 256 && (Cin % 8) == 0;
    const bool one_to_c = Cin == 1 && d->Cout >= 8 && d->Cout <= 256 && (d->Cout % 8) == 0 && !(dy_f32 && !d->f32);
    if (!c_to_1 && !one_to_c) return 1;
    p.C = c_to_1 ? Cin : d->Cout;
    const int vpb = 256 / (p.C >> 3);
    int64_t b = (p.S + (int64_t)vpb * 16 - 1) / ((int64_t)vpb * 16);
    const int64_t cap = (511 / d->N) > 0 ? (511 / d->N) : 1;
    if (b > cap) b = cap;
    if (b < 1) b = 1;
    const dim3 grid((int)b, d->N);
    if (vg_dry("pw_wgrad<%s,%s>", d->f32 ? "f32" : "bf16", c_to_1 ? "cto1" : "1toc")) return VG_OK;
    if (c_to_1) {
        if (d->f32) hipLaunchKernelGGL((pw_wgrad_kernel<float, true>), grid, dim3(256), 0, s, p);
        else hipLaunchKernelGGL((pw_wgrad_kernel<bf16_t, true>), grid, dim3(256), 0, s, p);
    } else {
        if (d->f32) hipLaunchKernelGGL((pw_wgrad_kernel<float, false>), grid, dim3(256), 0, s, p);
        else hipLaunchKernelGGL((pw_wgrad_kernel<bf16_t, false>), grid, dim3(256), 0, s, p);
    }
    return vg_check_launch();
}
```

### van_gan_amd/csrc/vg_wgrad.hip

```cpp
#include "vg_gather.h"

struct WgradK {
    const void* dy; int dy_f32; int Cout;
    int OD, OH, OW;
    int CIB, COB, ncib, ncob, tpg, ntg;
    int tap_src[VG_MAX_TAPS];
    float* dw; float* db;
    int total_tiles, DYS;
    float* part; int dw_elems;
};

#ifndef VG_WGRAD_UB
#define VG_WGRAD_UB (NOISE ? VG_WGRAD_UBN : (RMAX * Q > 4 ? 2 : 4))
#endif
#ifndef VG_WGRAD_UBN
#define VG_WGRAD_UBN 4
#endif
#ifndef VG_WGRAD_2W
#define VG_WGRAD_2W 16
#endif
typedef __attribute__((address_space(3))) bf16x4 lds_bf16x4;
#define VG_WSTAMP(slot) do { if (g.stamps && tid == 0 && it < 8) g.stamps[((size_t)blockIdx.y * gridDim.x + blockIdx.x) * 64 + it * 8 + (slot)] = __builtin_readcyclecounter(); } while (0)

__device__ __forceinline__ bf16x8 tr_frag(const char* base0, const char* base1) {
    bf16x4 lo = __builtin_amdgcn_ds_read_tr16_b64_v4i16((lds_bf16x4*)base0);
    bf16x4 hi = __builtin_amdgcn_ds_read_tr16_b64_v4i16((lds_bf16x4*)base1);
    return (bf16x8){lo[0], lo[1], lo[2], lo[3], hi[0], hi[1], hi[2], hi[3]};
}

template <typename T, int RMAX, int Q, bool NOISE>
__global__ __launch_bounds__(256, (RMAX * Q >= VG_WGRAD_2W ? 2 : 3)) void wgrad_kernel(const GatherIn g, const WgradK p) {
    constexpr bool F32 = sizeof(T) == 4;
    extern __shared__ __attribute__((aligned(16))) char smem[];
    const int tid = threadIdx.x, lane = tid & 63;
    const int wave = __builtin_amdgcn_readfirstlane(tid >> 6);
    const int lg = lane >> 4, li = lane & 15;
    int by = blockIdx.y;
    const int cob = by % p.ncob; by /= p.ncob;
    const int cib = by % p.ncib; const int tg = by / p.ncib;
    const int tap0 = tg * p.tpg;
    const int ntap_here = min(p.tpg, g.ntaps - tap0);
    const int tci = p.CIB >> 4;
    const int nrows = ntap_here * tci;

    const int BM = 1 << (g.tdl + g.thl + g.twl);
    char* halo = smem;
    const int hbytes = g.planar ? (g.CK >> 3) * g.PSB : g.HD * g.DS;
    char* dyt = smem + hbytes;
    const int dybytes = BM * p.DYS;
    int* tapoff = (int*)(dyt + dybytes);
    int* tapsrc = tapoff + 64;
    float* scs = (float*)((char*)tapoff + 512);
    int* utab = (int*)(scs + 2 * g.CK);
    int* rtab = utab + 2 * stage_ncols(g);
    const int RTN = 3 * stage_axis_len(g);
    int* ktab = rtab + 2 * RTN;

    if (tid < g.ntaps)
        tapoff[tid] = (g.td[tid] - g.tmin_d) * g.DS + ((g.th[tid] - g.tmin_h) * g.HWp + halo_pos_w(g, g.tw[tid] - g.tmin_w)) * g.VS;
    if (tid < VG_MAX_TAPS) tapsrc[tid] = p.tap_src[tid];
    build_column_table(g, utab, tid);
    if ((int)blockIdx.x < p.total_tiles) {
        int t2 = blockIdx.x % (g.tiles_d * g.tiles_h * g.tiles_w);
        const int fw_i = t2 % g.tiles_w; t2 /= g.tiles_w;
        const int fh_i = t2 % g.tiles_h;
        stage_resolve_axes(g, rtab, fh_i << g.thl, fw_i << g.twl, tid);
    }
    if constexpr (!F32) {
        const int TWm_ = (1 << g.twl) - 1, THm_ = (1 << g.thl) - 1;
        for (int e = tid; e < (BM / 32) * 64; e += 256) {
            const int ks = e >> 6, l2 = e & 63, lg2 = l2 >> 4, li2 = l2 & 15;
            const int m0 = ks * 32 + 8 * lg2 + (li2 >> 2), m1 = m0 + 4;
            const int w0 = m0 & TWm_, h0 = (m0 >> g.twl) & THm_, d0 = m0 >> (g.twl + g.thl);
            const int w1 = m1 & TWm_, h1 = (m1 >> g.twl) & THm_, d1 = m1 >> (g.twl + g.thl);
            const int lo = ((li2 & 3) >> 1) * g.CS + 8 * (li2 & 1);
            ktab[2 * e] = d0 * g.istr * g.DS + (h0 * g.istr * g.HWp + w0) * g.VS + lo;
            ktab[2 * e + 1] = d1 * g.istr * g.DS + (h1 * g.istr * g.HWp + w1) * g.VS + lo;
        }
    }
    __syncthreads();

    int aoff[RMAX];
#pragma unroll
    for (int j = 0; j < RMAX; ++j) {
        const int r = wave + 4 * j;
        const int rr = r < nrows ? r : 0;
        aoff[j] = tapoff[tap0 + rr / tci] + (rr % tci) * 2 * g.CS;
    }
    f32x4 acc[RMAX][Q];
#pragma unroll
    for (int j = 0; j < RMAX; ++j)
#pragma unroll
        for (int q = 0; q < Q; ++q) acc[j][q] = (f32x4){0.f, 0.f, 0.f, 0.f};
    float dbsum = 0.f;
    int cur_n = -1;

    const int TWm = (1 << g.twl) - 1, THm = (1 << g.thl) - 1;
    const int tiles_per_n = g.tiles_d * g.tiles_h * g.tiles_w;
    constexpr int gcol = (Q * 16) >> 3, gcol_l = Q == 1 ? 1 : (Q == 2 ? 2 : 3);
    const bool do_db = p.db && cib == 0 && tg == 0;

    int it = -1;
    int gs_w, gs_h, gs_d, gs_n;
    { int t = gridDim.x; gs_w = t % g.tiles_w; t /= g.tiles_w; gs_h = t % g.tiles_h; t /= g.tiles_h; gs_d = t % g.tiles_d; gs_n = t / g.tiles_d; }
    int ti_w, ti_h, ti_d, ti_n;
    { int t = blockIdx.x; ti_w = t % g.tiles_w; t /= g.tiles_w; ti_h = t % g.tiles_h; t /= g.tiles_h; ti_d = t % g.tiles_d; ti_n = t / g.tiles_d; }
    for (int tile = blockIdx.x; tile < p.total_tiles; tile += gridDim.x) {
        ++it;
        VG_WSTAMP(0);
        const int n = ti_n;
        const int od0 = ti_d << g.tdl, oh0 = ti_h << g.thl, ow0 = ti_w << g.twl;
        ti_w += gs_w; if (ti_w >= g.tiles_w) { ti_w -= g.tiles_w; ++ti_h; }
        ti_h += gs_h; if (ti_h >= g.tiles_h) { ti_h -= g.tiles_h; ++ti_d; }
        ti_d += gs_d; if (ti_d >= g.tiles_d) { ti_d -= g.tiles_d; ++ti_n; }
        ti_n += gs_n;
        __syncthreads();
        if (n != cur_n) {
            stage_scale_shift(g, scs, n, cib, tid);
            cur_n = n;
            __syncthreads();
        }
        int* rt = rtab + (it & 1) * RTN;
        Raw8<T> yraw[4]; float y1[4]; bool yok[4];
        const bool dy_on = !(g.dbg & 2) || tile == (int)blockIdx.x;
        if (dy_on) {
#pragma unroll
            for (int k = 0; k < 4; ++k) {
                const int u = min(tid + k * 256, BM * gcol - 1);
                const int m = u >> gcol_l, cg = u & (gcol - 1);
                const int w = m & TWm, h = (m >> g.twl) & THm, d = m >> (g.twl + g.thl);
                const int od = od0 + d, oh = oh0 + h, ow = ow0 + w;
                const int c = cob * p.COB + cg * 8;
                yok[k] = od < p.OD && oh < p.OH && ow < p.OW && c < p.Cout;
                const size_t vox = yok[k] ? ((size_t)(n * p.OD + od) * p.OH + oh) * p.OW + ow : 0;
                if (p.Cout == 1) y1[k] = p.dy_f32 ? ld_global((const float*)p.dy + vox) : ld_global((const bf16_t*)p.dy + vox);
                else raw_load(yraw[k], (const T*)p.dy + vox * p.Cout + (yok[k] ? c : 0));
            }
        }
        if (!(g.dbg & 1) || tile == (int)blockIdx.x) stage_halo_tile<T, NOISE, VG_WGRAD_UB>(g, halo, scs, utab, rt, n, od0, cib, tid);
        if (tile + (int)gridDim.x < p.total_tiles) {
            stage_resolve_axes(g, rtab + ((it + 1) & 1) * RTN, ti_h << g.thl, ti_w << g.twl, tid);
        }
        if (dy_on) {
#pragma unroll
            for (int k = 0; k < 4; ++k) {
                const int u = tid + k * 256;
                if (u < BM * gcol) {
                    const int m = u >> gcol_l, cg = u & (gcol - 1);
                    T* dst = (T*)(dyt + (size_t)m * p.DYS) + cg * 8;
                    if (p.Cout == 1) {
                        const float v[8] = {yok[k] ? y1[k] : 0.f, 0.f, 0.f, 0.f, 0.f, 0.f, 0.f, 0.f};
                        store8<T>(dst, v);
                    } else {
                        raw_mask(yraw[k], yok[k]);
                        *(Raw8<T>*)dst = yraw[k];
                    }
                }
            }
        }
        VG_WSTAMP(1);
        __syncthreads();
        VG_WSTAMP(2);
        if (do_db) {
            const int nrg = 256 / p.COB;
            if (tid < nrg * p.COB) {
                const int c = tid % p.COB;
                float s = 0.f;
                for (int m = tid / p.COB; m < BM; m += nrg) s += ld1<T>((const T*)(dyt + (size_t)m * p.DYS) + c);
                dbsum += s;
            }
        }
        if (g.dbg & 4) continue;
        if constexpr (F32) {
            for (int s = 0; s < BM / 4; ++s) {
                const int m0 = s * 4 + lg;
                const int w0 = m0 & TWm, h0 = (m0 >> g.twl) & THm, d0 = m0 >> (g.twl + g.thl);
                const int r0 = d0 * g.istr * g.DS + (h0 * g.istr * g.HWp + w0) * g.VS + (li >> 3) * g.CS + (li & 7) * 4;
                const char* y0 = dyt + (size_t)m0 * p.DYS + li * 4;
                float b[Q];
#pragma unroll
                for (int q = 0; q < Q; ++q) b[q] = *(const float*)(y0 + q * 64);
#pragma unroll
                for (int j = 0; j < RMAX; ++j) {
                    const float a = *(const float*)(halo + r0 + aoff[j]);
#pragma unroll
                    for (int q = 0; q < Q; ++q) acc[j][q] = __builtin_amdgcn_mfma_f32_16x16x4f32(a, b[q], acc[j][q], 0, 0, 0);
                }
            }
        } else {
            constexpr int RC = RMAX <= 8 ? RMAX : 6;
            static_assert(RMAX % RC == 0, "rows per wave must be a multiple of the chunk");
            constexpr int NCH = RMAX / RC;
            const int nks = BM / 32;
            const int2* kt = (const int2*)ktab + lane;
            const char* ybase = dyt + (size_t)(8 * lg + (li >> 2)) * p.DYS + 8 * (li & 3);
            const int ystep = 32 * p.DYS, y4 = 4 * p.DYS;
            bf16x8 A[2][RC], B[2][Q];
            {
                const int2 r = kt[0];
#pragma unroll
                for (int q = 0; q < Q; ++q) B[0][q] = tr_frag(ybase + q * 32, ybase + y4 + q * 32);
#pragma unroll
                for (int j = 0; j < RC; ++j) A[0][j] = tr_frag(halo + r.x + aoff[j], halo + r.y + aoff[j]);
            }
            for (int ks = 0; ks < nks; ks += 2) {
#pragma unroll
                for (int u = 0; u < 2; ++u) {
                    const int2 rc = kt[(ks + u) * 64];
                    const int kn = min(ks + u + 1, nks - 1);
                    const int2 rn = kt[kn * 64];
                    const char* yn = ybase + (size_t)kn * ystep;
#pragma unroll
                    for (int c = 0; c < NCH; ++c) {
                        constexpr int dummy = 0; (void)dummy;
                        const int s = (u * NCH + c) & 1;
                        if (c + 1 < NCH) {
#pragma unroll
                            for (int j = 0; j < RC; ++j) A[s ^ 1][j] = tr_frag(halo + rc.x + aoff[(c + 1) * RC + j], halo + rc.y + aoff[(c + 1) * RC + j]);
                        } else {
#pragma unroll
                            for (int q = 0; q < Q; ++q) B[u ^ 1][q] = tr_frag(yn + q * 32, yn + y4 + q * 32);
#pragma unroll
                            for (int j = 0; j < RC; ++j) A[s ^ 1][j] = tr_frag(halo + rn.x + aoff[j], halo + rn.y + aoff[j]);
                        }
                        __builtin_amdgcn_sched_barrier(0);
#pragma unroll
                        for (int j = 0; j < RC; ++j)
#pragma unroll
                            for (int q = 0; q < Q; ++q)
                                acc[c * RC + j][q] = VG_MFMA16(A[s][j], B[u][q], acc[c * RC + j][q]);
                        __builtin_amdgcn_sched_barrier(0);
                    }
                }
            }
        }
        VG_WSTAMP(3);
    }
    { const int it = 7; VG_WSTAMP(7); }
#pragma unroll
    for (int j = 0; j < RMAX; ++j) {
        const int r = wave + 4 * j;
        if (r >= nrows) continue;
        const int tap = tap0 + r / tci, ci0 = cib * p.CIB + (r % tci) * 16 + 4 * lg;
#pragma unroll
        for (int q = 0; q < Q; ++q) {
            const int co = cob * p.COB + q * 16 + li;
            if (co >= p.Cout) continue;
#pragma unroll
            for (int e = 0; e < 4; ++e)
                if (ci0 + e < g.Cw) {
                    const size_t i = ((size_t)tapsrc[tap] * g.Cw + ci0 + e) * p.Cout + co;
                    if (p.part) p.part[(size_t)blockIdx.x * p.dw_elems + i] = acc[j][q][e];
                    else atomicAdd(&p.dw[i], acc[j][q][e]);
                }
        }
    }
    if (do_db) {
        __syncthreads();
        float* red = (float*)halo;
        if (tid < p.COB) red[tid] = 0.f;
        __syncthreads();
        if (tid < (256 / p.COB) * p.COB) atomicAdd(&red[tid % p.COB], dbsum);
        __syncthreads();
        if (tid < p.COB) {
            const int co = cob * p.COB + tid;
            if (co < p.Cout) atomicAdd(&p.db[co], red[tid]);
        }
    }
}

__global__ __launch_bounds__(256) void reduce_partials_kernel(const float* part, int nb, int n, float* dw) {
    __shared__ float sm[4][64];
    const int lane = threadIdx.x & 63, w = threadIdx.x >> 6;
    const int i = blockIdx.x * 64 + lane;
    float s = 0.f;
    if (i < n) {
        int b = w;
        for (; b + 28 < nb; b += 32) {
            float v[8];
#pragma unroll
            for (int k = 0; k < 8; ++k) v[k] = part[(size_t)(b + 4 * k) * n + i];
#pragma unroll
            for (int k = 0; k < 8; ++k) s += v[k];
        }
        for (; b < nb; b += 4) s += part[(size_t)b * n + i];
    }
    sm[w][lane] = s;
    __syncthreads();
    if (w == 0 && i < n) atomicAdd(&dw[i], sm[0][lane] + sm[1][lane] + sm[2][lane] + sm[3][lane]);
}

void vg_launch_reduce_partials(const float* part, int nb, int n, float* dw, hipStream_t s) {
    hipLaunchKernelGGL(reduce_partials_kernel, dim3((n + 63) / 64), dim3(256), 0, s, part, nb, n, dw);
}

template <typename T, int RMAX, int Q, bool NOISE>
static void launch_wgrad2(const GatherIn& g, const WgradK& k, dim3 grid, int lds, hipStream_t s) {
    static bool attr_set = false;
    if (!attr_set) {
        (void)hipFuncSetAttribute((const void*)wgrad_kernel<T, RMAX, Q, NOISE>, hipFuncAttributeMaxDynamicSharedMemorySize, VG_LDS_LIMIT);
        attr_set = true;
    }
    hipLaunchKernelGGL((wgrad_kernel<T, RMAX, Q, NOISE>), grid, dim3(256), lds, s, g, k);
}
template <typename T, int RMAX, int Q>
static void launch_wgrad(const GatherIn& g, const WgradK& k, dim3 grid, int lds, hipStream_t s) {
    if (g.noise) launch_wgrad2<T, RMAX, Q, true>(g, k, grid, lds, s); else launch_wgrad2<T, RMAX, Q, false>(g, k, grid, lds, s);
}

extern "C" int vg_conv3d_wgrad(const vg_conv_desc* d, const void* dy, int dy_f32, const int32_t* tap_idx_host,
                               int T_total, float* dw, float* db, float* scratch, int64_t scratch_bytes,
                               vg_stream_t stream) {
    vg_begin();
    if (!d || !dy || !dw || !tap_idx_host) return VG_EINVAL;
    if (d->Cout < 1 || (d->Cout != 1 && (d->Cout % 8))) return VG_EINVAL;
    if (dy_f32 && d->Cout != 1 && !d->f32) return VG_EINVAL;
    if (d->src0 && tap_idx_host[0] == 0) {
        const int wrc = vg_wgrad_pw_dma(d, dy, dy_f32, T_total, dw, db, scratch, scratch_bytes, (hipStream_t)stream);
        if (wrc <= 0) return wrc;
        const int prc = vg_pointwise_wgrad(d, dy, dy_f32, T_total, dw, db, scratch, scratch_bytes, (hipStream_t)stream);
        if (prc <= 0) return prc;
    }
    {
        const int trc = vg_wgrad_thin(d, dy, dy_f32, tap_idx_host, T_total, dw, db, scratch, scratch_bytes, (hipStream_t)stream);
        if (trc <= 0) return trc;
    }
    {
        const int drc = vg_wgrad_dma(d, dy, dy_f32, tap_idx_host, T_total, dw, db, scratch, scratch_bytes, (hipStream_t)stream);
        if (drc <= 0) return drc;
    }
    const int Cin = d->c_src0 + d->c_src1;
    const int Cinp = ((Cin + 15) / 16) * 16, Coutp = ((d->Cout + 15) / 16) * 16;
    const int COB = Coutp >= 64 ? 64 : (Coutp >= 32 ? 32 : 16);
    if (Coutp % COB) return VG_EINVAL;
    const int Q = COB / 16;
    int RMAX = Q == 1 ? 24 : (Q == 2 ? 12 : 6);
    const int esz = d->f32 ? 4 : 2;
    GatherIn g; WgradK k;
    int max_bm = vg_tune("WGRAD_BM", 256), max_cib = vg_tune("WGRAD_CIB", 64);
    if (d->ntaps >= 64 && max_cib > 16 && vg_tune("WGRAD_CIB16_K4", 1)) max_cib = 16;
    const bool k3_all_taps = d->ntaps == 27 && Coutp >= 32 && !d->f32 && vg_tune("WGRAD_CIB16", 1);
    if (k3_all_taps && max_cib > 16) max_cib = 16;
    int best_bm = 0, best_cib = 0, best_lds = 0;
    for (int pass = 0; pass < 2 && !best_bm; ++pass) {
        const int limit = pass == 0 ? vg_tune("WGRAD_LDS0", 80 * 1024) : VG_LDS_LIMIT;
        for (int bm = 256; bm >= 64 && !best_bm; bm = bm == 256 ? 128 : bm - 64)
            for (int c = max_cib; c >= 16; c -= 16) {
                if (Cinp % c) continue;
                if (bm == 256 && (Q > 2 || max_bm < 256)) continue;
                int rc = fill_gather(d, g, c, bm, d->f32 ? 0 : 64);
                if (rc != VG_OK) return rc;
                const int lds = halo_bytes(g) + bm * (COB * esz + 16) + 512 + 2 * c * 4 + stage_table_ints(g) * 4 + (bm / 32) * 512;
                if (lds <= limit) { best_bm = bm; best_cib = c; best_lds = lds; break; }
            }
    }
    if (!best_bm) return VG_ELDS;
    const int CIB = best_cib, lds = best_lds;
    int rc = fill_gather(d, g, CIB, best_bm, d->f32 ? 0 : 64);
    if (rc != VG_OK) return rc;
    k.DYS = COB * esz + 16;
    k.dy = dy; k.dy_f32 = dy_f32; k.Cout = d->Cout; k.OD = d->OD; k.OH = d->OH; k.OW = d->OW;
    k.CIB = CIB; k.COB = COB; k.ncib = Cinp / CIB; k.ncob = Coutp / COB;
    const int rows_per_tap = CIB / 16;
    if (Q == 4 && k3_all_taps && CIB == 16) RMAX = 7;
    k.tpg = (4 * RMAX) / rows_per_tap; if (k.tpg < 1) return VG_EINVAL;
    if (k.tpg > d->ntaps) k.tpg = d->ntaps;
    k.ntg = (d->ntaps + k.tpg - 1) / k.tpg;
    k.tpg = (d->ntaps + k.ntg - 1) / k.ntg;
    for (int i = 0; i < VG_MAX_TAPS; ++i) k.tap_src[i] = i < d->ntaps ? tap_idx_host[i] : 0;
    k.dw = dw; k.db = db;
    k.total_tiles = d->N * g.tiles_d * g.tiles_h * g.tiles_w;
    const int by = k.ntg * k.ncib * k.ncob;
    const int wg_env = vg_tune("WGRAD_WGS", 0);
    const int rw_ = (k.tpg * rows_per_tap + 3) / 4;
    const int rmax_sel = d->f32 ? RMAX : (rw_ <= 2 ? 2 : (rw_ <= 8 && Q <= 2 ? 8 : (Q == 4 && rw_ == 7 ? 7 : RMAX)));
    int per_cu = (rmax_sel * Q >= VG_WGRAD_2W) ? 2 : 3;
    if (VG_LDS_LIMIT / lds < per_cu) per_cu = VG_LDS_LIMIT / lds;
    if (per_cu < 1) per_cu = 1;
    const int wg_target = wg_env > 0 ? wg_env : (256 * per_cu < 384 ? 256 * per_cu : 384);
    int bx = wg_target / by; if (bx < 1) bx = 1; if (bx > k.total_tiles) bx = k.total_tiles;
    k.dw_elems = T_total * (d->wpack ? d->wpack : Cin) * d->Cout;
    k.part = nullptr;
    if (bx > 8 && scratch && (int64_t)bx * k.dw_elems * 4 <= scratch_bytes) k.part = scratch;
    const dim3 grid(bx, by, 1);
    hipStream_t s = (hipStream_t)stream;
    const int rw = (k.tpg * rows_per_tap + 3) / 4;
    {
        const int rsel = d->f32 ? RMAX : (rw <= 2 ? 2 : ((rw <= 8 && Q <= 2) ? 8 : (Q == 4 && rw == 7 ? 7 : RMAX)));
        if (vg_dry("wgrad<%s,%d,%d,n%d>|bm%d|cib%d|part%d|walk%d", d->f32 ? "f32" : "bf16", rsel, Q, g.noise ? 1 : 0, best_bm, CIB,
                   k.part ? 1 : 0, k.total_tiles > bx ? 1 : 0)) return VG_OK;
    }
    if (d->f32) {
        if (Q == 1) launch_wgrad<float, 24, 1>(g, k, grid, lds, s);
        else if (Q == 2) launch_wgrad<float, 12, 2>(g, k, grid, lds, s);
        else launch_wgrad<float, 6, 4>(g, k, grid, lds, s);
    } else if (Q == 1) {
        if (rw <= 2) launch_wgrad<bf16_t, 2, 1>(g, k, grid, lds, s);
        else if (rw <= 8) launch_wgrad<bf16_t, 8, 1>(g, k, grid, lds, s);
        else launch_wgrad<bf16_t, 24, 1>(g, k, grid, lds, s);
    } else if (Q == 2) {
        if (rw <= 2) launch_wgrad<bf16_t, 2, 2>(g, k, grid, lds, s);
        else if (rw <= 8) launch_wgrad<bf16_t, 8, 2>(g, k, grid, lds, s);
        else launch_wgrad<bf16_t, 12, 2>(g, k, grid, lds, s);
    } else {
        if (rw <= 2) launch_wgrad<bf16_t, 2, 4>(g, k, grid, lds, s);
        else if (rw == 7) launch_wgrad<bf16_t, 7, 4>(g, k, grid, lds, s);
        else launch_wgrad<bf16_t, 6, 4>(g, k, grid, lds, s);
    }
    if (k.part) {
        hipLaunchKernelGGL(reduce_partials_kernel, dim3((k.dw_elems + 63) / 64), dim3(256), 0, s, k.part, bx, k.dw_elems, dw);
    }
    return vg_check_launch();
}

extern "C" int vg_conv3d_wgrad_variant(const vg_conv_desc* d, int dy_f32, const int32_t* tap_idx_host, int T_total,
                                       int64_t scratch_bytes, char* buf, int buflen) {
    if (!buf || buflen < 64) return VG_EINVAL;
    vg_dry_begin(buf, buflen);
    const int rc = vg_conv3d_wgrad(d, (const void*)(uintptr_t)0x1000, dy_f32, tap_idx_host, T_total, (float*)(uintptr_t)0x1000,
                                   (float*)(uintptr_t)0x1000, scratch_bytes > 0 ? (float*)(uintptr_t)0x1000 : nullptr, scratch_bytes, nullptr);
    vg_dry_end();
    return rc;
}
```

### van_gan_amd/csrc/vg_wgrad_dma.hip

```cpp
#include "vg_dma_common.h"

__global__ __launch_bounds__(256) void materialize_kernel(const MatK p) {
    const int tid = threadIdx.x;
    int row = blockIdx.x;
    const int hp = row % p.Hp; row /= p.Hp;
    const int dp = row % p.Dp; const int n = row / p.Dp;
    int pd = dp + p.pmin_d, ph = hp + p.pmin_h;
    const int qd = pd + p.npad, qh = ph + p.npad;
    const bool vd = resolve_pos(pd, p.D, p.pad_mode), vh = resolve_pos(ph, p.H, p.pad_mode);
    const int npl = p.Cin >> 4;
    const int units = npl * p.Wps * 2;
    const int sh = p.shift0;
    const float slope = p.act == VG_ACT_RELU ? 0.f : (p.act == VG_ACT_LRELU ? VG_LRELU : 1.f);
    const int ND = p.D + 2 * p.npad, NH = p.H + 2 * p.npad, NW = p.W + 2 * p.npad;
    const bool nrow = p.noise && vd && vh && qd >= 0 && qd < ND && qh >= 0 && qh < NH;
    const size_t s0row = (((size_t)n * (p.D >> sh) + (pd >> sh)) * (p.H >> sh) + (ph >> sh)) * (p.W >> sh);
    const size_t s1row = (((size_t)n * p.D + pd) * p.H + ph) * p.W;
    const size_t nzrow = (((size_t)n * ND + (nrow ? qd : 0)) * NH + (nrow ? qh : 0)) * NW;
    for (int u = tid; u < units; u += 256) {
        const int plane = u / (p.Wps * 2), r = u - plane * p.Wps * 2;
        const int ws = r >> 1, half = r & 1;
        const int j = p.deint ? (ws < p.WE ? 2 * ws : 2 * (ws - p.WE) + 1) : ws;
        int pw = j + p.pmin_w;
        const int qw = pw + p.npad;
        const bool vw = j < p.Wp && resolve_pos(pw, p.W, p.pad_mode);
        const bool valid = vd && vh && vw;
        const int c = plane * 16 + half * 8;
        float x[8];
        {
            const bool from0 = c < p.c0;
            const bf16_t* src = from0 ? (const bf16_t*)p.src0 + (s0row + (valid ? (pw >> sh) : 0)) * p.c0 + c
                                      : (const bf16_t*)p.src1 + (s1row + (valid ? pw : 0)) * p.c1 + (c - p.c0);
            if (!valid) src = (const bf16_t*)p.src0;
            Raw8<bf16_t> raw; raw_load(raw, src);
            raw_unpack(raw, x);
        }
        if (p.in_scale) {
            const f32x4* sc = (const f32x4*)(p.in_scale + n * p.Cin + c);
            const f32x4* sf = (const f32x4*)(p.in_shift + n * p.Cin + c);
            const f32x4 s0 = sc[0], s1 = sc[1], f0 = sf[0], f1 = sf[1];
#pragma unroll
            for (int e = 0; e < 4; ++e) { x[e] = x[e] * s0[e] + f0[e]; x[4 + e] = x[4 + e] * s1[e] + f1[e]; }
        }
#pragma unroll
        for (int e = 0; e < 8; ++e) x[e] = fmaxf(x[e], x[e] * slope);
        if (p.noise) {
            const bool nok = nrow && valid && qw >= 0 && qw < NW;
            Raw8<bf16_t> nz; raw_load(nz, p.noise + (nzrow + (nok ? qw : 0)) * p.Cin + c);
            float z[8]; raw_unpack(nz, z);
#pragma unroll
            for (int e = 0; e < 8; ++e) x[e] += nok ? z[e] : 0.f;
        }
#pragma unroll
        for (int e = 0; e < 8; ++e) x[e] = valid ? x[e] : 0.f;
        bf16_t* dst = p.out + ((((size_t)(n * npl + plane) * p.Dp + dp) * p.Hp + hp) * p.Wps + ws) * 16 + half * 8;
        store8<bf16_t>(dst, x);
    }
}

void vg_launch_materialize(const MatK& m, hipStream_t s) { hipLaunchKernelGGL(materialize_kernel, dim3(m.N * m.Dp * m.Hp), dim3(256), 0, s, m); }

#define VG_WD_MAXA 9
#define VG_WD_MAXB 4
#define VG_WD_TAB 64

struct WgdK {
    const char* P; const char* dy;
    int N, OD, OH, OW, Cout, Cin;
    int plane_bytes;
    int Hp, Wps, WEP;
    int istr, deint;
    int ntaps; int tap_src[VG_MAX_TAPS]; int8_t td[VG_MAX_TAPS], th[VG_MAX_TAPS], tw[VG_MAX_TAPS];
    int PL, NPL, ncob, CO2;
    int tdl, thl, twl, tiles_d, tiles_h, tiles_w, total_tiles;
    int HD, HH, HW, HWE;
    int imgp, nA, nB, bufb, nbuf;
    float* dw; float* db; float* part; int dw_elems;
    unsigned m_imgp, m_hhw, m_hw, m_pl, m_tpn, m_tw, m_th, m_ncob;
    int co2l;
    const char* x0; const char* x1; int c0, c1, sh0;
    int D, H, W, pmin_d, pmin_h, pmin_w;
    const float* in_scale; const float* in_shift; float slope;
    unsigned long long* stamps;
};

__device__ __forceinline__ bf16x8 tr_frag_d(const char* base0, const char* base1) {
    bf16x4 lo = __builtin_amdgcn_ds_read_tr16_b64_v4i16((lds_bf16x4_d*)base0);
    bf16x4 hi = __builtin_amdgcn_ds_read_tr16_b64_v4i16((lds_bf16x4_d*)base1);
    return (bf16x8){lo[0], lo[1], lo[2], lo[3], hi[0], hi[1], hi[2], hi[3]};
}

template <int R, int Q, bool DIRECT>
__global__ __launch_bounds__(512, 2) void wgrad_dma_kernel(const WgdK p) {
    extern __shared__ __attribute__((aligned(16))) char smem[];
    const int tid = threadIdx.x, lane = tid & 63;
    const int wave = __builtin_amdgcn_readfirstlane(tid >> 6);
    const int lg = lane >> 4, li = lane & 15;
    const int cib = fast_div(blockIdx.y, p.m_ncob), cob = blockIdx.y - cib * p.ncob;
    const int BM = 1 << (p.tdl + p.thl + p.twl);
    const int nks = BM >> 5;
    const int TWm = (1 << p.twl) - 1, THm = (1 << p.thl) - 1;
    int* tapoff = (int*)(smem + p.nbuf * p.bufb);
    const int CO = p.CO2 >> 1;
    const int nrows = p.ntaps * p.PL;
    const bool stamp = p.stamps != nullptr;
    unsigned long long t_begin = 0, t_loop = 0, t_a = 0, s_wait = 0, s_issue = 0, s_k = 0;
    if (stamp) t_begin = __builtin_readcyclecounter();

    int aoffs[VG_WD_MAXA], boffs[VG_WD_MAXB];
    int acst[DIRECT ? VG_WD_MAXA : 1];
    {
        const int nvox = p.HD * p.HH * p.HW;
#pragma unroll
        for (int k = 0; k < VG_WD_MAXA; ++k) {
            const int piece = wave + 8 * k;
            const int pl = fast_div(piece, p.m_imgp), pk = piece - pl * p.imgp;
            int iv = pk * 32 + (lane >> 1);
            if (iv >= nvox) iv = 0;
            const int hd = fast_div(iv, p.m_hhw), rem = iv - hd * (p.HH * p.HW);
            const int hh = fast_div(rem, p.m_hw), ws = rem - hh * p.HW;
            if constexpr (DIRECT) {
                const int j = p.deint ? (ws < p.HWE ? 2 * ws : 2 * (ws - p.HWE) + 1) : ws;
                const int c = (cib * p.PL + pl) * 16 + (lane & 1) * 8;
                const int src1 = c >= p.c0 ? 1 : 0;
                aoffs[k] = hd | ((p.HD + hh) << 8) | ((p.HD + p.HH + j) << 16) | (src1 << 24);
                acst[k] = (src1 ? c - p.c0 : c) * 2;
            } else {
                const int gw = p.deint ? (ws < p.HWE ? ws : p.WEP + ws - p.HWE) : ws;
                aoffs[k] = pl * p.plane_bytes + ((hd * p.Hp + hh) * p.Wps + gw) * 32 + (lane & 1) * 16;
            }
        }
#pragma unroll
        for (int k = 0; k < VG_WD_MAXB; ++k) {
            const int byte = (wave + 8 * k) * 1024 + lane * 16;
            int m = byte >> p.co2l; const int s = (byte - (m << p.co2l)) >> 4;
            if (m >= BM) m = 0;
            const int f = p.CO2 == 128 ? (m >> 1) & 3 : (p.CO2 == 64 ? (m >> 2) & 1 : 0);
            const int blk = (s >> 1) ^ f;
            const int w = m & TWm, h = (m >> p.twl) & THm, d = m >> (p.twl + p.thl);
            boffs[k] = (((d * p.OH + h) * p.OW + w) * p.Cout + cob * CO + blk * 16 + (s & 1) * 8) * 2;
        }
    }
    const int tiles_per_n = p.tiles_d * p.tiles_h * p.tiles_w;
    const unsigned lds0 = (unsigned)(uintptr_t)(lds_void_d*)smem;
    int* otab = tapoff + VG_MAX_TAPS;
    float* scs = (float*)(otab + 4 * VG_WD_TAB);
    auto build_tab = [&](int tile, int tb) {
        const int L = p.HD + p.HH + p.HW;
        if (tid >= 2 * L) return;
        int t = tile;
        const int n = fast_div(t, p.m_tpn); t -= n * tiles_per_n;
        const int t1 = fast_div(t, p.m_tw), ti_w = t - t1 * p.tiles_w;
        const int ti_d = fast_div(t1, p.m_th), ti_h = t1 - ti_d * p.tiles_h;
        const int src1 = tid >= L ? 1 : 0, e = tid - src1 * L;
        const int sh = src1 ? 0 : p.sh0, C2 = (src1 ? p.c1 : p.c0) * 2;
        const int Hs = p.H >> sh, Ws = p.W >> sh;
        int pos, nn, mul;
        if (e < p.HD) { pos = (ti_d << p.tdl) * p.istr + p.pmin_d + e; nn = p.D; mul = Hs * Ws * C2; }
        else if (e < p.HD + p.HH) { pos = (ti_h << p.thl) * p.istr + p.pmin_h + e - p.HD; nn = p.H; mul = Ws * C2; }
        else { pos = (ti_w << p.twl) * p.istr + p.pmin_w + e - p.HD - p.HH; nn = p.W; mul = C2; }
        pos = pos < 0 ? -pos : pos; pos = pos >= nn ? 2 * nn - 2 - pos : pos;
        pos = min(max(pos, 0), nn - 1);
        otab[(tb * 2 + src1) * VG_WD_TAB + e] = (pos >> sh) * mul;
    };
    auto issue = [&](int tile, int bufoff, int tb) {
        int t = tile;
        const int n = fast_div(t, p.m_tpn); t -= n * tiles_per_n;
        const int t1 = fast_div(t, p.m_tw), ti_w = t - t1 * p.tiles_w;
        const int ti_d = fast_div(t1, p.m_th), ti_h = t1 - ti_d * p.tiles_h;
        const int od0 = ti_d << p.tdl, oh0 = ti_h << p.thl, ow0 = ti_w << p.twl;
        const char* bbase = p.dy + ((((size_t)n * p.OD + od0) * p.OH + oh0) * p.OW + ow0) * p.Cout * 2;
        if constexpr (DIRECT) {
            const char* a0 = p.x0 + (size_t)n * (p.D >> p.sh0) * (p.H >> p.sh0) * (p.W >> p.sh0) * p.c0 * 2;
            const char* a1 = p.x1 + (size_t)n * p.D * p.H * p.W * p.c1 * 2;
            const int* tb0 = otab + tb * 2 * VG_WD_TAB;
#pragma unroll
            for (int k = 0; k < VG_WD_MAXA; ++k) {
                const int piece = wave + 8 * k;
                if (piece < p.nA) {
                    const int cr = aoffs[k];
                    const int* tq = tb0 + (cr >> 24) * VG_WD_TAB;
                    const int off = tq[cr & 255] + tq[(cr >> 8) & 255] + tq[(cr >> 16) & 255] + acst[k];
                    const bool lo = (fast_div(piece, p.m_imgp) + cib * p.PL) * 16 < p.c0;
                    glds16(lo ? a0 : a1, off, lds0 + bufoff + piece * 1024);
                }
            }
        } else {
            const char* abase = p.P + (size_t)(n * p.NPL + cib * p.PL) * p.plane_bytes
                                + (size_t)((od0 * p.istr * p.Hp + oh0 * p.istr) * p.Wps + (p.deint ? ow0 : ow0 * p.istr)) * 32;
#pragma unroll
            for (int k = 0; k < VG_WD_MAXA; ++k) {
                const int piece = wave + 8 * k;
                if (piece < p.nA) glds16(abase, aoffs[k], lds0 + bufoff + piece * 1024);
            }
        }
#pragma unroll
        for (int k = 0; k < VG_WD_MAXB; ++k) {
            const int piece = wave + 8 * k;
            if (piece < p.nB) glds16(bbase, boffs[k], lds0 + bufoff + (p.nA + piece) * 1024);
        }
    };
    const int ntw = ((int)blockIdx.x < p.total_tiles) ? (p.total_tiles - (int)blockIdx.x + (int)gridDim.x - 1) / (int)gridDim.x : 0;
    const int n_w = (wave < p.nA ? (p.nA - wave + 7) >> 3 : 0) + (wave < p.nB ? (p.nB - wave + 7) >> 3 : 0);
    if constexpr (DIRECT) {
        for (int i = tid; i < p.N * 2 * p.PL * 16; i += 512) {
            const int n = i / (2 * p.PL * 16), r = i - n * 2 * p.PL * 16, sf = r >= p.PL * 16 ? 1 : 0, c = r - sf * p.PL * 16;
            const float* src = sf ? p.in_shift : p.in_scale;
            scs[i] = src ? src[n * p.Cin + cib * p.PL * 16 + c] : (sf ? 0.f : 1.f);
        }
        for (int j = 0; j < p.nbuf - 1 && j < ntw; ++j) {
            build_tab(blockIdx.x + j * gridDim.x, j & 1);
            __syncthreads();
            issue(blockIdx.x + j * gridDim.x, j * p.bufb, j & 1);
        }
    } else {
        for (int j = 0; j < p.nbuf - 1 && j < ntw; ++j) issue(blockIdx.x + j * gridDim.x, j * p.bufb, 0);
    }

    if (tid < p.ntaps)
        tapoff[tid] = ((p.td[tid] * p.HH + p.th[tid]) * p.HW + (p.deint ? (p.tw[tid] & 1) * p.HWE + (p.tw[tid] >> 1) : p.tw[tid])) * 32;
    __syncthreads();

    int aoff[R];
#pragma unroll
    for (int j = 0; j < R; ++j) {
        const int r = wave + 8 * j, rr = r < nrows ? r : 0;
        const int tp = fast_div(rr, p.m_pl);
        aoff[j] = (rr - tp * p.PL) * p.imgp * 1024 + tapoff[tp];
    }
    f32x4 acc[R][Q];
#pragma unroll
    for (int j = 0; j < R; ++j)
#pragma unroll
        for (int q = 0; q < Q; ++q) acc[j][q] = (f32x4){0.f, 0.f, 0.f, 0.f};
    const int m0l = 4 * lg + (li >> 2);
    const int fsw = p.CO2 == 128 ? (m0l >> 1) & 3 : (p.CO2 == 64 ? (m0l >> 2) & 1 : 0);
    int yq[Q];
#pragma unroll
    for (int q = 0; q < Q; ++q) yq[q] = m0l * p.CO2 + 32 * (q ^ fsw) + 8 * (li & 3);
    const int ystep = 32 * p.CO2, y16 = 16 * p.CO2;
    const int rps_l = 5 - p.twl;
    const int wsx = p.deint ? 1 : p.istr;
    const int lx = (((m0l >> p.twl) * p.istr) * p.HW + (m0l & TWm) * wsx) * 32 + 8 * (li & 3);
    const int ly = ((((m0l + 16) >> p.twl) * p.istr) * p.HW + ((m0l + 16) & TWm) * wsx) * 32 + 8 * (li & 3);
    auto soff = [&](int ks) { const int q32 = ks << rps_l; return (((q32 >> p.thl) * p.istr * p.HH + (q32 & THm) * p.istr) * p.HW) << 5; };
    const bool do_db = p.db && cib == 0;
    float dbs[8];
#pragma unroll
    for (int e = 0; e < 8; ++e) dbs[e] = 0.f;
    const int nslots = CO >> 3;
    const int db_s = tid % nslots, db_v0 = tid / nslots, db_vs = 512 / nslots;

    constexpr int RC = R <= 4 ? R : 4;
    constexpr int NCH = (R + RC - 1) / RC;
    int cur = 0, nxt = p.nbuf - 1;
    if (stamp) t_loop = __builtin_readcyclecounter();
    for (int it = 0; it < ntw; ++it) {
        char* hb = smem + cur * p.bufb;
        if (stamp) t_a = __builtin_readcyclecounter();
        const int newer = min(p.nbuf - 2, ntw - 1 - it);
        const int itn = it + p.nbuf - 1;
        if constexpr (DIRECT) { if (itn < ntw) build_tab(blockIdx.x + itn * gridDim.x, itn & 1); }
        wait_vmcnt(newer * n_w);
        if constexpr (DIRECT) {
            const int n_cur = fast_div((int)blockIdx.x + it * (int)gridDim.x, p.m_tpn);
            const float* sc0 = scs + n_cur * 2 * p.PL * 16 + (lane & 1) * 8;
#pragma unroll
            for (int k = 0; k < VG_WD_MAXA; ++k) {
                const int piece = wave + 8 * k;
                if (piece < p.nA) {
                    const int pl = fast_div(piece, p.m_imgp);
                    bf16x8* u = (bf16x8*)(hb + piece * 1024 + lane * 16);
                    const f32x4 s0 = *(const f32x4*)(sc0 + pl * 16), s1 = *(const f32x4*)(sc0 + pl * 16 + 4);
                    const f32x4 f0 = *(const f32x4*)(sc0 + (p.PL + pl) * 16), f1 = *(const f32x4*)(sc0 + (p.PL + pl) * 16 + 4);
                    const bf16x8 raw = *u;
                    bf16x8 o;
#pragma unroll
                    for (int e = 0; e < 4; ++e) {
                        float a = bf2f((bf16_t)raw[e]) * s0[e] + f0[e], b = bf2f((bf16_t)raw[4 + e]) * s1[e] + f1[e];
                        a = fmaxf(a, a * p.slope); b = fmaxf(b, b * p.slope);
                        o[e] = (short)f2bf(a); o[4 + e] = (short)f2bf(b);
                    }
                    *u = o;
                }
            }
        }
        __syncthreads();
        if (stamp) { const unsigned long long t = __builtin_readcyclecounter(); s_wait += t - t_a; t_a = t; }
        if (itn < ntw) issue(blockIdx.x + itn * gridDim.x, nxt * p.bufb, itn & 1);
        if (stamp) { const unsigned long long t = __builtin_readcyclecounter(); s_issue += t - t_a; t_a = t; }
        cur = cur + 1 == p.nbuf ? 0 : cur + 1; nxt = nxt + 1 == p.nbuf ? 0 : nxt + 1;
        const char* yb = hb + p.nA * 1024;
        if (do_db) {
            for (int v = db_v0; v < BM; v += db_vs) {
                const bf16x8 r = *(const bf16x8*)(yb + v * p.CO2 + db_s * 16);
#pragma unroll
                for (int e = 0; e < 8; ++e) dbs[e] += bf2f((bf16_t)r[e]);
            }
        }
        {
            bf16x8 A[2][RC], B[2][Q];
            {
#pragma unroll
                for (int q = 0; q < Q; ++q) B[0][q] = tr_frag_d(yb + yq[q], yb + yq[q] + y16);
#pragma unroll
                for (int j = 0; j < RC; ++j) A[0][j] = tr_frag_d(hb + lx + aoff[j], hb + ly + aoff[j]);
            }
            for (int ks = 0; ks < nks; ks += 2) {
#pragma unroll
                for (int u = 0; u < 2; ++u) {
                    const int kn = min(ks + u + 1, nks - 1);
                    const char* hc = hb + soff(ks + u);
                    const char* hn = hb + soff(kn);
                    const char* yn = yb + kn * ystep;
#pragma unroll
                    for (int c = 0; c < NCH; ++c) {
                        const int s = (u * NCH + c) & 1;
                        if (c + 1 < NCH) {
#pragma unroll
                            for (int j = 0; j < RC; ++j) {
                                const int jj = (c + 1) * RC + j < R ? (c + 1) * RC + j : R - 1;
                                A[s ^ 1][j] = tr_frag_d(hc + lx + aoff[jj], hc + ly + aoff[jj]);
                            }
                        } else {
#pragma unroll
                            for (int q = 0; q < Q; ++q) B[u ^ 1][q] = tr_frag_d(yn + yq[q], yn + yq[q] + y16);
#pragma unroll
                            for (int j = 0; j < RC; ++j) A[s ^ 1][j] = tr_frag_d(hn + lx + aoff[j], hn + ly + aoff[j]);
                        }
                        __builtin_amdgcn_sched_barrier(0);
#pragma unroll
                        for (int j = 0; j < RC; ++j)
                            if (c * RC + j < R) {
#pragma unroll
                                for (int q = 0; q < Q; ++q)
                                    acc[c * RC + j][q] = VG_MFMA16(A[s][j], B[u][q], acc[c * RC + j][q]);
                            }
                        __builtin_amdgcn_sched_barrier(0);
                    }
                }
            }
        }
        if (stamp) { asm volatile("s_waitcnt lgkmcnt(0)" ::: "memory"); s_k += __builtin_readcyclecounter() - t_a; }
    }
    unsigned long long t_slab = 0;
    if (stamp) t_slab = __builtin_readcyclecounter();
#pragma unroll
    for (int j = 0; j < R; ++j) {
        const int r = wave + 8 * j;
        if (r >= nrows) continue;
        const int tap = fast_div(r, p.m_pl), ci0 = (cib * p.PL + r - tap * p.PL) * 16 + 4 * lg;
#pragma unroll
        for (int q = 0; q < Q; ++q) {
            const int co = cob * CO + q * 16 + li;
#pragma unroll
            for (int e = 0; e < 4; ++e) {
                const size_t i = ((size_t)p.tap_src[tap] * p.Cin + ci0 + e) * p.Cout + co;
                if (p.part) p.part[(size_t)blockIdx.x * p.dw_elems + i] = acc[j][q][e];
                else atomicAdd(&p.dw[i], acc[j][q][e]);
            }
        }
    }
    if (do_db) {
        __syncthreads();
        float* red = (float*)smem;
        if (tid < CO) red[tid] = 0.f;
        __syncthreads();
        if (db_v0 < BM) {
            const int fv = p.CO2 == 128 ? (db_v0 >> 1) & 3 : (p.CO2 == 64 ? (db_v0 >> 2) & 1 : 0);
            const int ch = 16 * ((db_s >> 1) ^ fv) + 8 * (db_s & 1);
#pragma unroll
            for (int e = 0; e < 8; ++e) atomicAdd(&red[ch + e], dbs[e]);
        }
        __syncthreads();
        if (tid < CO) atomicAdd(&p.db[cob * CO + tid], red[tid]);
    }
    if (stamp && tid == 0) {
        asm volatile("s_waitcnt vmcnt(0)" ::: "memory");
        unsigned long long* o = p.stamps + ((size_t)blockIdx.y * gridDim.x + blockIdx.x) * 8;
        o[0] = t_loop - t_begin; o[1] = s_wait; o[2] = s_issue; o[3] = s_k; o[4] = __builtin_readcyclecounter() - t_slab;
        o[5] = __builtin_readcyclecounter() - t_begin; o[6] = ntw; o[7] = __builtin_amdgcn_s_memrealtime();
    }
}

template <int R, int Q, bool DIRECT>
static void launch_wd2(const WgdK& k, dim3 grid, int lds, hipStream_t s) {
    static bool attr_set = false;
    if (!attr_set) {
        (void)hipFuncSetAttribute((const void*)wgrad_dma_kernel<R, Q, DIRECT>, hipFuncAttributeMaxDynamicSharedMemorySize, VG_LDS_LIMIT);
        attr_set = true;
    }
    hipLaunchKernelGGL((wgrad_dma_kernel<R, Q, DIRECT>), grid, dim3(512), lds, s, k);
}
template <int R, int Q>
static void launch_wd(const WgdK& k, bool direct, dim3 grid, int lds, hipStream_t s) {
    if (direct) launch_wd2<R, Q, true>(k, grid, lds, s); else launch_wd2<R, Q, false>(k, grid, lds, s);
}

int vg_wgrad_dma(const vg_conv_desc* d, const void* dy, int dy_f32, const int32_t* tap_idx_host, int T_total, float* dw, float* db,
                 float* scratch, int64_t scratch_bytes, hipStream_t s) {
    if (!vg_tune("WGRAD_DMA", 1)) return 1;
    const int Cin = d->c_src0 + d->c_src1;
    if (d->f32 || dy_f32 || d->src_f32 || d->wpack || Cin < 16 || (Cin % 16) || (d->Cout % 16) || d->ntaps < 8 || d->ntaps > VG_MAX_TAPS) return 1;
    if (d->istr < 1 || d->istr > 2 || !scratch || T_total < 1) return 1;
    if ((d->OW % 8) || d->OD < 2 || d->OH < 2) return 1;
    if (d->c_src1 > 0 && ((d->c_src0 % 8) || (d->c_src1 % 8))) return 1;
    int mn[3] = {127, 127, 127}, mx[3] = {-128, -128, -128};
    for (int i = 0; i < d->ntaps; ++i) {
        const int v[3] = {d->tap_d[i], d->tap_h[i], d->tap_w[i]};
        for (int a = 0; a < 3; ++a) { if (v[a] < mn[a]) mn[a] = v[a]; if (v[a] > mx[a]) mx[a] = v[a]; }
    }
    const int ex[3] = {mx[0] - mn[0] + 1, mx[1] - mn[1] + 1, mx[2] - mn[2] + 1};
    if (d->pad_mode == VG_PAD_REFLECT) {
        const int od[3] = {d->OD, d->OH, d->OW}, nn[3] = {d->D, d->H, d->W};
        for (int a = 0; a < 3; ++a) if (mn[a] < -(nn[a] - 1) || (od[a] - 1) * d->istr + mx[a] > 2 * nn[a] - 2) return 1;
    }
    const int NPL = Cin / 16;
    const int deint = d->istr == 2 ? 1 : 0;
    const int Dp = (d->OD - 1) * d->istr + ex[0], Hp = (d->OH - 1) * d->istr + ex[1], Wp = (d->OW - 1) * d->istr + ex[2];
    const int WE = (Wp + 1) / 2, Wps = deint ? 2 * WE : Wp;
    const int64_t plane_bytes = (int64_t)Dp * Hp * Wps * 32;
    const bool direct = vg_tune("WGRAD_DMA_DIRECT", 1) && d->pad_mode == VG_PAD_REFLECT && !d->noise && Cin <= vg_tune("WGRAD_DMA_DIRECT_CIN", 48)
                        && (d->c_src1 == 0 || (d->c_src0 % 16) == 0) && (!d->src0_shift || (!(d->D & 1) && !(d->H & 1) && !(d->W & 1)))
                        && (int64_t)d->D * d->H * d->W * (d->c_src0 > d->c_src1 ? d->c_src0 : d->c_src1) * 2 < (1LL << 31);
    const int64_t p_bytes = direct ? 0 : ((plane_bytes * NPL * d->N + 255) / 256) * 256;
    if (p_bytes >= (1LL << 31)) return 1;
    const int64_t dw_elems = (int64_t)T_total * Cin * d->Cout;
    struct Plan { int CO, PL, R, TD, TH, TW, lds, columns, tiles, bx, nbuf; double cost; };
    Plan best; best.cost = -1;
    const int f_co = vg_tune("WGRAD_DMA_CO", 0), f_pl = vg_tune("WGRAD_DMA_PL", 0), f_bx = vg_tune("WGRAD_DMA_BX", 0);
    const int bm_cap = vg_tune("WGRAD_DMA_BM", 512), nbuf_cap = vg_tune("WGRAD_DMA_NBUF", 5), wg_target = vg_tune("WGRAD_DMA_WGS", 256);
    static const int RQ4[] = {8, 0}, RQ2[] = {4, 8, 0}, RQ1[] = {4, 8, 12, 0};
    for (int CO = 64; CO >= 16; CO >>= 1) {
        if (CO > d->Cout || (d->Cout % CO) || (f_co && CO != f_co)) continue;
        const int Q = CO / 16;
        const int* ravail = Q == 4 ? RQ4 : (Q == 2 ? RQ2 : RQ1);
        for (int PL = NPL; PL >= 1; --PL) {
            if ((NPL % PL) || (f_pl && PL != f_pl) || plane_bytes * PL >= (1LL << 30)) continue;
            const int rneed = (d->ntaps * PL + 7) / 8;
            int R = 0; for (int i = 0; ravail[i]; ++i) if (ravail[i] >= rneed) { R = ravail[i]; break; }
            if (!R) continue;
            const int columns = (NPL / PL) * (d->Cout / CO);
            const int per_cu = 1;
            const int lds_cap = VG_LDS_LIMIT / per_cu;
            for (int bm = 512; bm >= 64; bm >>= 1) {
                if (bm > bm_cap) continue;
                long bvol = -1; int t3[5] = {0, 0, 0, 0, 0}, bufb = 0;
                for (int tw = 8; tw <= 16; tw <<= 1) {
                    if (d->OW % tw) continue;
                    for (int th = 1; th <= d->OH && tw * th <= bm; th <<= 1) {
                        if ((d->OH % th) || tw * th < 32) continue;
                        const int td = bm / (tw * th);
                        if (td > d->OD || (d->OD % td)) continue;
                        const int HD = (td - 1) * d->istr + ex[0], HH = (th - 1) * d->istr + ex[1], HW = (tw - 1) * d->istr + ex[2];
                        const int imgp = (HD * HH * HW * 32 + 1023) / 1024;
                        const int nA = PL * imgp, nB = bm * CO * 2 / 1024;
                        if (nA > 8 * VG_WD_MAXA || nB > 8 * VG_WD_MAXB || nB < 1) continue;
                        if (direct && (HD + HH + HW > VG_WD_TAB || d->N * PL > 16)) continue;
                        const int tabs = VG_MAX_TAPS * 4 + (direct ? 4 * VG_WD_TAB * 4 + d->N * 2 * PL * 16 * 4 : 0);
                        if (2 * (nA + nB) * 1024 + tabs > lds_cap) continue;
                        int nb_ = (lds_cap - tabs) / ((nA + nB) * 1024); if (nb_ > nbuf_cap) nb_ = nbuf_cap; if (nb_ < 2) nb_ = 2;
                        const int lds = nb_ * (nA + nB) * 1024 + tabs;
                        const long vol = (long)HD * HH * HW;
                        if (bvol < 0 || vol < bvol) { bvol = vol; t3[0] = td; t3[1] = th; t3[2] = tw; t3[3] = lds; t3[4] = nb_; bufb = (nA + nB) * 1024; }
                    }
                }
                if (bvol < 0) continue;
                const int tiles = d->N * (d->OD / t3[0]) * (d->OH / t3[1]) * (d->OW / t3[2]);
                if ((int64_t)tiles * (tiles / d->N) >= (1LL << 32)) continue;
                static const int BXC[] = {1, 2, 3, 4, 6, 8, 12, 16, 24, 32, 48, 64, 96, 128, 192, 256, 0};
                for (int ib = 0; ib < 17; ++ib) {
                    int bxx = BXC[ib] ? BXC[ib] : wg_target * per_cu / columns;
                    if (bxx < 1) bxx = 1;
                    if (bxx > tiles) bxx = tiles;
                    if (f_bx) bxx = f_bx < tiles ? f_bx : tiles;
                    else if ((long)bxx * columns > (long)wg_target * per_cu && bxx > 1) continue;
                    const int64_t part_bytes = bxx > 1 ? (int64_t)bxx * dw_elems * 4 : 0;
                    if (p_bytes + part_bytes > scratch_bytes) { if (f_bx) break; continue; }
                    const double ntile = (double)((tiles + bxx - 1) / bxx);
                    const double rounds = (double)(((long)bxx * columns + 256 * per_cu - 1) / (256 * per_cu));
                    const double mfma = (bm / 32) * R * Q * 16.0 * 2.0 * per_cu, stage = bufb / 14.0 * per_cu;
                    const double lat = 4500.0 / (t3[4] - 1);
                    double per = mfma > stage ? mfma : stage; if (lat > per) per = lat;
                    const double loop = ntile * per + 5000.0;
                    const double slab = (double)dw_elems / columns * 4.0 / 16.0;
                    double tail;
                    if (bxx > 1) tail = ((double)(bxx + 1) * dw_elems * 4.0 + dw_elems * 4.0 * 3.0) / 2500.0 + 12000.0;
                    else tail = (double)dw_elems * 4.0 * 3.0 / 2500.0;
                    const double cost = rounds * (loop + slab) + tail + 6000.0;
                    if (best.cost < 0 || cost < best.cost) best = Plan{CO, PL, R, t3[0], t3[1], t3[2], t3[3], columns, tiles, bxx, t3[4], cost};
                    if (f_bx) break;
                }
            }
        }
    }
    if (best.cost < 0) return 1;
    const int CO = best.CO, Q = CO / 16, PL = best.PL, Rsel = best.R;
    const int TD = best.TD, TH = best.TH, TW = best.TW, lds = best.lds, columns = best.columns, ncob = d->Cout / CO;
    const int BM = TD * TH * TW;
    WgdK k;
    k.N = d->N; k.OD = d->OD; k.OH = d->OH; k.OW = d->OW; k.Cout = d->Cout; k.Cin = Cin;
    k.plane_bytes = (int)plane_bytes; k.Hp = Hp; k.Wps = Wps; k.WEP = deint ? WE : 0; k.istr = d->istr; k.deint = deint;
    k.ntaps = d->ntaps;
    for (int i = 0; i < VG_MAX_TAPS; ++i) {
        k.tap_src[i] = i < d->ntaps ? tap_idx_host[i] : 0;
        k.td[i] = i < d->ntaps ? d->tap_d[i] - mn[0] : 0; k.th[i] = i < d->ntaps ? d->tap_h[i] - mn[1] : 0; k.tw[i] = i < d->ntaps ? d->tap_w[i] - mn[2] : 0;
    }
    k.PL = PL; k.NPL = NPL; k.ncob = ncob; k.CO2 = CO * 2;
    k.tdl = ilog2_exact(TD); k.thl = ilog2_exact(TH); k.twl = ilog2_exact(TW);
    k.tiles_d = d->OD / TD; k.tiles_h = d->OH / TH; k.tiles_w = d->OW / TW;
    k.total_tiles = d->N * k.tiles_d * k.tiles_h * k.tiles_w;
    k.HD = (TD - 1) * d->istr + ex[0]; k.HH = (TH - 1) * d->istr + ex[1]; k.HW = (TW - 1) * d->istr + ex[2];
    k.HWE = deint ? (k.HW + 1) / 2 : 0;
    k.imgp = (k.HD * k.HH * k.HW * 32 + 1023) / 1024; k.nA = PL * k.imgp; k.nB = BM * CO * 2 / 1024; k.bufb = (k.nA + k.nB) * 1024; k.nbuf = best.nbuf;
    k.dw = dw; k.db = db; k.dw_elems = (int)dw_elems; k.stamps = g_vg_stamps;
    auto magic = [](int dd) { return dd <= 1 ? 0u : (unsigned)((1ULL << 32) / (unsigned)dd + 1ULL); };
    k.m_imgp = magic(k.imgp); k.m_hhw = magic(k.HH * k.HW); k.m_hw = magic(k.HW); k.m_pl = magic(PL);
    k.m_tpn = magic(k.tiles_d * k.tiles_h * k.tiles_w); k.m_tw = magic(k.tiles_w); k.m_th = magic(k.tiles_h); k.m_ncob = magic(ncob);
    k.co2l = ilog2_exact(CO * 2);
    const int bx = best.bx;
    k.P = (const char*)scratch; k.dy = (const char*)dy;
    k.part = bx > 1 ? (float*)((char*)scratch + p_bytes) : nullptr;
    k.x0 = (const char*)d->src0; k.x1 = (const char*)d->src1; k.c0 = d->c_src0; k.c1 = d->c_src1; k.sh0 = d->src0_shift ? 1 : 0;
    k.D = d->D; k.H = d->H; k.W = d->W; k.pmin_d = mn[0]; k.pmin_h = mn[1]; k.pmin_w = mn[2];
    k.in_scale = d->in_scale; k.in_shift = d->in_shift;
    k.slope = d->act == VG_ACT_RELU ? 0.f : (d->act == VG_ACT_LRELU ? VG_LRELU : 1.f);
    if (vg_dry("wgrad_dma<%d,%d,d%d>|bm%d|pl%d|s%d|nb%d|part%d|walk%d", Rsel, Q, direct ? 1 : 0, BM, PL, d->istr, k.nbuf, k.part ? 1 : 0, k.total_tiles > bx ? 1 : 0)) return VG_OK;
    const dim3 grid(bx, columns, 1);
    if (!direct) {
    MatK m;
    m.src0 = d->src0; m.src1 = d->src1; m.c0 = d->c_src0; m.c1 = d->c_src1; m.shift0 = d->src0_shift ? 1 : 0;
    m.N = d->N; m.D = d->D; m.H = d->H; m.W = d->W; m.Cin = Cin;
    m.in_scale = d->in_scale; m.in_shift = d->in_shift; m.act = d->act;
    m.noise = (const bf16_t*)d->noise; m.npad = d->noise ? d->noise_pad : 0; m.pad_mode = d->pad_mode;
    m.pmin_d = mn[0]; m.pmin_h = mn[1]; m.pmin_w = mn[2]; m.Dp = Dp; m.Hp = Hp; m.Wp = Wp;
    m.deint = deint; m.WE = WE; m.Wps = Wps; m.out = (bf16_t*)scratch;
    vg_launch_materialize(m, s);
    }
    if (Q == 4) launch_wd<8, 4>(k, direct, grid, lds, s);
    else if (Q == 2) { if (Rsel == 4) launch_wd<4, 2>(k, direct, grid, lds, s); else launch_wd<8, 2>(k, direct, grid, lds, s); }
    else { if (Rsel == 4) launch_wd<4, 1>(k, direct, grid, lds, s); else if (Rsel == 8) launch_wd<8, 1>(k, direct, grid, lds, s); else launch_wd<12, 1>(k, direct, grid, lds, s); }
    if (k.part) vg_launch_reduce_partials(k.part, bx, k.dw_elems, dw, s);
    return vg_check_launch();
}

struct WpwK {
    const char* x0; const char* x1; const char* dy;
    int c0, c1, sh0, istr;
    int N, D, H, W, OD, OH, OW, Cin, Cout;
    int FA, RS, KS, ksl, ncob, CO2, co2l;
    int tdl, thl, twl, tiles_d, tiles_h, tiles_w, total_tiles;
    int ppp, nA, nB, bufb, nbuf;
    unsigned m_tpn, m_tw, m_th, m_ppp, m_ncob;
    float* dw; float* db; float* part; int dw_elems;
};

template <int R, int Q>
__global__ __launch_bounds__(512, 2) void wgrad_pw_dma_kernel(const WpwK p) {
    extern __shared__ __attribute__((aligned(16))) char smem[];
    const int tid = threadIdx.x, lane = tid & 63;
    const int wave = __builtin_amdgcn_readfirstlane(tid >> 6);
    const int lg = lane >> 4, li = lane & 15;
    const int rgrp0 = fast_div(blockIdx.y, p.m_ncob), cob = blockIdx.y - rgrp0 * p.ncob;
    (void)rgrp0;
    const int kgrp = wave & (p.KS - 1), rgrp = wave >> p.ksl;
    const int BM = 1 << (p.tdl + p.thl + p.twl);
    const int nks = BM >> 5;
    const int TWm = (1 << p.twl) - 1, THm = (1 << p.thl) - 1;
    const int CO = p.CO2 >> 1;
    const int Hs = p.H >> p.sh0, Ws = p.W >> p.sh0;
    int aoffs[VG_WD_MAXA], boffs[VG_WD_MAXB];
#pragma unroll
    for (int k = 0; k < VG_WD_MAXA; ++k) {
        const int piece = wave + 8 * k;
        const int plane = fast_div(piece, p.m_ppp), pk = piece - plane * p.ppp;
        const int m = pk * 32 + (lane >> 1);
        const int c = plane * 16 + (lane & 1) * 8;
        const int w = (m & TWm) * p.istr, h = ((m >> p.twl) & THm) * p.istr, d = (m >> (p.twl + p.thl)) * p.istr;
        aoffs[k] = c < p.c0 ? ((((d >> p.sh0) * Hs + (h >> p.sh0)) * Ws + (w >> p.sh0)) * p.c0 + c) * 2
                            : (((d * p.H + h) * p.W + w) * p.c1 + (c - p.c0)) * 2;
    }
#pragma unroll
    for (int k = 0; k < VG_WD_MAXB; ++k) {
        const int byte = (wave + 8 * k) * 1024 + lane * 16;
        int m = byte >> p.co2l; const int s = (byte - (m << p.co2l)) >> 4;
        if (m >= BM) m = 0;
        const int f = p.CO2 == 128 ? (m >> 1) & 3 : (p.CO2 == 64 ? (m >> 2) & 1 : 0);
        const int blk = (s >> 1) ^ f;
        const int w = m & TWm, h = (m >> p.twl) & THm, d = m >> (p.twl + p.thl);
        boffs[k] = (((d * p.OH + h) * p.OW + w) * p.Cout + cob * CO + blk * 16 + (s & 1) * 8) * 2;
    }
    const int tiles_per_n = p.tiles_d * p.tiles_h * p.tiles_w;
    const unsigned lds0 = (unsigned)(uintptr_t)(lds_void_d*)smem;
    auto issue = [&](int tile, int bufoff) {
        int t = tile;
        const int n = fast_div(t, p.m_tpn); t -= n * tiles_per_n;
        const int t1 = fast_div(t, p.m_tw), ti_w = t - t1 * p.tiles_w;
        const int ti_d = fast_div(t1, p.m_th), ti_h = t1 - ti_d * p.tiles_h;
        const int od0 = ti_d << p.tdl, oh0 = ti_h << p.thl, ow0 = ti_w << p.twl;
        const int id0 = od0 * p.istr, ih0 = oh0 * p.istr, iw0 = ow0 * p.istr;
        const char* a0 = p.x0 + ((((size_t)n * (p.D >> p.sh0) + (id0 >> p.sh0)) * Hs + (ih0 >> p.sh0)) * Ws + (iw0 >> p.sh0)) * p.c0 * 2;
        const char* a1 = p.x1 + ((((size_t)n * p.D + id0) * p.H + ih0) * p.W + iw0) * p.c1 * 2;
        const char* bbase = p.dy + ((((size_t)n * p.OD + od0) * p.OH + oh0) * p.OW + ow0) * p.Cout * 2;
#pragma unroll
        for (int k = 0; k < VG_WD_MAXA; ++k) {
            const int piece = wave + 8 * k;
            if (piece < p.nA) {
                const bool lo = fast_div(piece, p.m_ppp) * 16 < p.c0;
                glds16(lo ? a0 : a1, aoffs[k], lds0 + bufoff + piece * 1024);
            }
        }
#pragma unroll
        for (int k = 0; k < VG_WD_MAXB; ++k) {
            const int piece = wave + 8 * k;
            if (piece < p.nB) glds16(bbase, boffs[k], lds0 + bufoff + (p.nA + piece) * 1024);
        }
    };
    const int ntw = ((int)blockIdx.x < p.total_tiles) ? (p.total_tiles - (int)blockIdx.x + (int)gridDim.x - 1) / (int)gridDim.x : 0;
    const int n_w = (wave < p.nA ? (p.nA - wave + 7) >> 3 : 0) + (wave < p.nB ? (p.nB - wave + 7) >> 3 : 0);
    for (int j = 0; j < p.nbuf - 1 && j < ntw; ++j) issue(blockIdx.x + j * gridDim.x, j * p.bufb);

    int poff[R];
#pragma unroll
    for (int j = 0; j < R; ++j) { const int pl = rgrp + p.RS * j; poff[j] = (pl < p.FA ? pl : 0) * (BM * 32); }
    f32x4 acc[R][Q];
#pragma unroll
    for (int j = 0; j < R; ++j)
#pragma unroll
        for (int q = 0; q < Q; ++q) acc[j][q] = (f32x4){0.f, 0.f, 0.f, 0.f};
    const int m0l = 4 * lg + (li >> 2);
    const int fsw = p.CO2 == 128 ? (m0l >> 1) & 3 : (p.CO2 == 64 ? (m0l >> 2) & 1 : 0);
    int yq[Q];
#pragma unroll
    for (int q = 0; q < Q; ++q) yq[q] = m0l * p.CO2 + 32 * (q ^ fsw) + 8 * (li & 3);
    const int lx = m0l * 32 + 8 * (li & 3);
    const int ystep = 32 * p.CO2, y16 = 16 * p.CO2;
    const bool do_db = p.db != nullptr;
    float dbs[8];
#pragma unroll
    for (int e = 0; e < 8; ++e) dbs[e] = 0.f;
    const int nslots = CO >> 3;
    const int db_s = tid % nslots, db_v0 = tid / nslots, db_vs = 512 / nslots;

    int cur = 0, nxt = p.nbuf - 1;
    for (int it = 0; it < ntw; ++it) {
        const char* hb = smem + cur * p.bufb;
        const int newer = min(p.nbuf - 2, ntw - 1 - it);
        wait_vmcnt(newer * n_w);
        __syncthreads();
        if (it + p.nbuf - 1 < ntw) issue(blockIdx.x + (it + p.nbuf - 1) * gridDim.x, nxt * p.bufb);
        cur = cur + 1 == p.nbuf ? 0 : cur + 1; nxt = nxt + 1 == p.nbuf ? 0 : nxt + 1;
        const char* yb = hb + p.nA * 1024;
        if (do_db) {
            for (int v = db_v0; v < BM; v += db_vs) {
                const bf16x8 r = *(const bf16x8*)(yb + v * p.CO2 + db_s * 16);
#pragma unroll
                for (int e = 0; e < 8; ++e) dbs[e] += bf2f((bf16_t)r[e]);
            }
        }
        for (int ks = kgrp; ks < nks; ks += p.KS) {
            bf16x8 A[R], B[Q];
            const char* hk = hb + ks * 1024 + lx;
            const char* yk = yb + ks * ystep;
#pragma unroll
            for (int q = 0; q < Q; ++q) B[q] = tr_frag_d(yk + yq[q], yk + yq[q] + y16);
#pragma unroll
            for (int j = 0; j < R; ++j) A[j] = tr_frag_d(hk + poff[j], hk + poff[j] + 512);
#pragma unroll
            for (int j = 0; j < R; ++j)
#pragma unroll
                for (int q = 0; q < Q; ++q) acc[j][q] = VG_MFMA16(A[j], B[q], acc[j][q]);
        }
    }
    float* red = (float*)smem;
    int sl = 1;
    for (int step = 1; step < p.KS; step <<= 1, ++sl) {
        const int slot = rgrp * (p.KS >> sl) + (kgrp >> sl);
        __syncthreads();
        if ((kgrp & (2 * step - 1)) == step) {
            float* dst = red + (size_t)(slot * R * Q) * 256 + lane * 4;
#pragma unroll
            for (int j = 0; j < R; ++j)
#pragma unroll
                for (int q = 0; q < Q; ++q) *(f32x4*)(dst + (j * Q + q) * 256) = acc[j][q];
        }
        __syncthreads();
        if ((kgrp & (2 * step - 1)) == 0) {
            const float* src = red + (size_t)(slot * R * Q) * 256 + lane * 4;
#pragma unroll
            for (int j = 0; j < R; ++j)
#pragma unroll
                for (int q = 0; q < Q; ++q) acc[j][q] += *(const f32x4*)(src + (j * Q + q) * 256);
        }
    }
    if (kgrp == 0) {
#pragma unroll
        for (int j = 0; j < R; ++j) {
            const int pl = rgrp + p.RS * j;
            if (pl >= p.FA) continue;
            const int ci0 = pl * 16 + 4 * lg;
#pragma unroll
            for (int q = 0; q < Q; ++q) {
                const int co = cob * CO + q * 16 + li;
#pragma unroll
                for (int e = 0; e < 4; ++e) {
                    const size_t i = (size_t)(ci0 + e) * p.Cout + co;
                    if (p.part) p.part[(size_t)blockIdx.x * p.dw_elems + i] = acc[j][q][e];
                    else atomicAdd(&p.dw[i], acc[j][q][e]);
                }
            }
        }
    }
    if (do_db) {
        __syncthreads();
        if (tid < CO) red[tid] = 0.f;
        __syncthreads();
        if (db_v0 < BM) {
            const int fv = p.CO2 == 128 ? (db_v0 >> 1) & 3 : (p.CO2 == 64 ? (db_v0 >> 2) & 1 : 0);
            const int ch = 16 * ((db_s >> 1) ^ fv) + 8 * (db_s & 1);
#pragma unroll
            for (int e = 0; e < 8; ++e) atomicAdd(&red[ch + e], dbs[e]);
        }
        __syncthreads();
        if (tid < CO) atomicAdd(&p.db[cob * CO + tid], red[tid]);
    }
}

template <int R, int Q>
static void launch_wpw(const WpwK& k, dim3 grid, int lds, hipStream_t s) {
    static bool attr_set = false;
    if (!attr_set) {
        (void)hipFuncSetAttribute((const void*)wgrad_pw_dma_kernel<R, Q>, hipFuncAttributeMaxDynamicSharedMemorySize, VG_LDS_LIMIT);
        attr_set = true;
    }
    hipLaunchKernelGGL((wgrad_pw_dma_kernel<R, Q>), grid, dim3(512), lds, s, k);
}

int vg_wgrad_pw_dma(const vg_conv_desc* d, const void* dy, int dy_f32, int T_total, float* dw, float* db, float* scratch,
                    int64_t scratch_bytes, hipStream_t s) {
    if (!vg_tune("WGRAD_PW_DMA", 1)) return 1;
    const int Cin = d->c_src0 + d->c_src1;
    if (d->f32 || dy_f32 || d->src_f32 || d->wpack || d->ntaps != 1 || T_total != 1 || d->tap_d[0] || d->tap_h[0] || d->tap_w[0]) return 1;
    if (d->in_scale || d->act != VG_ACT_NONE || d->noise || !scratch) return 1;
    if (Cin < 16 || (Cin % 16) || (d->Cout % 16) || (d->c_src0 % 16) || (d->c_src1 % 16)) return 1;
    if (d->istr < 1 || d->istr > 2 || d->OD * d->istr != d->D || d->OH * d->istr != d->H || d->OW * d->istr != d->W) return 1;
    if (d->src0_shift && d->istr != 1) return 1;
    const int FA = Cin / 16;
    const int CO = d->Cout >= 64 ? 64 : d->Cout;
    if ((d->Cout % CO) || FA > 24) return 1;
    const int Q = CO / 16, ncob = d->Cout / CO;
    int R = 0, RS = 1;
    if (Q == 1) { R = 3; } else if (Q == 2) { R = 6; } else { R = FA <= 4 ? 4 : 6; }
    while (RS < 8 && RS * R < FA) RS <<= 1;
    if (RS * R < FA) return 1;
    const int KS = 8 / RS;
    int best[5] = {0, 0, 0, 0, 0};
    for (int bm = 512; bm >= 64 && !best[0]; bm >>= 1) {
        const int nA = FA * (bm / 32), nB = bm * CO * 2 / 1024;
        if (nA > 8 * VG_WD_MAXA || nB > 8 * VG_WD_MAXB || nB < 1) continue;
        const int bufb = (nA + nB) * 1024;
        if (2 * bufb > VG_LDS_LIMIT || (bm / 32) < KS) continue;
        if (8 * R * Q * 1024 / 2 > VG_LDS_LIMIT) continue;
        for (int tw = 16; tw >= 8 && !best[0]; tw >>= 1) {
            if (d->OW % tw) continue;
            for (int th = 2; th <= d->OH && tw * th <= bm; th <<= 1) {
                if ((d->OH % th) || tw * th < 32) continue;
                const int td = bm / (tw * th);
                if (td > d->OD || (d->OD % td) || (d->src0_shift && (td & 1))) continue;
                int nb = VG_LDS_LIMIT / bufb; if (nb > 4) nb = 4;
                best[0] = td; best[1] = th; best[2] = tw; best[3] = bufb; best[4] = nb;
                break;
            }
        }
    }
    if (!best[0]) return 1;
    const int TD = best[0], TH = best[1], TW = best[2], BM = TD * TH * TW;
    if (d->src0_shift && ((TD | TH | TW) & 1)) return 1;
    WpwK k;
    k.x0 = (const char*)d->src0; k.x1 = (const char*)d->src1; k.dy = (const char*)dy;
    k.c0 = d->c_src0; k.c1 = d->c_src1; k.sh0 = d->src0_shift ? 1 : 0; k.istr = d->istr;
    k.N = d->N; k.D = d->D; k.H = d->H; k.W = d->W; k.OD = d->OD; k.OH = d->OH; k.OW = d->OW; k.Cin = Cin; k.Cout = d->Cout;
    k.FA = FA; k.RS = RS; k.KS = KS; k.ksl = ilog2_exact(KS); k.ncob = ncob; k.CO2 = CO * 2; k.co2l = ilog2_exact(CO * 2);
    k.tdl = ilog2_exact(TD); k.thl = ilog2_exact(TH); k.twl = ilog2_exact(TW);
    k.tiles_d = d->OD / TD; k.tiles_h = d->OH / TH; k.tiles_w = d->OW / TW;
    k.total_tiles = d->N * k.tiles_d * k.tiles_h * k.tiles_w;
    k.ppp = BM / 32; k.nA = FA * k.ppp; k.nB = BM * CO * 2 / 1024; k.bufb = best[3]; k.nbuf = best[4];
    auto magic = [](int dd) { return dd <= 1 ? 0u : (unsigned)((1ULL << 32) / (unsigned)dd + 1ULL); };
    k.m_tpn = magic(k.tiles_d * k.tiles_h * k.tiles_w); k.m_tw = magic(k.tiles_w); k.m_th = magic(k.tiles_h); k.m_ppp = magic(k.ppp); k.m_ncob = magic(ncob);
    k.dw = dw; k.db = db; k.dw_elems = Cin * d->Cout;
    if ((int64_t)k.total_tiles * (k.total_tiles / d->N) >= (1LL << 32)) return 1;
    if (k.total_tiles * ncob < 32) return 1;
    int bx = vg_tune("WGRAD_PW_WGS", 256) / ncob; if (bx < 1) bx = 1; if (bx > k.total_tiles) bx = k.total_tiles;
    const int64_t part_bytes = (int64_t)bx * k.dw_elems * 4;
    if (part_bytes > scratch_bytes) return 1;
    k.part = (float*)scratch;
    int lds = k.nbuf * k.bufb; { const int rl = 4 * R * Q * 1024; if (rl > lds) lds = rl; }
    if (vg_dry("wgrad_pw_dma<%d,%d>|bm%d|rs%d|s%d|u%d|nb%d|walk%d", R, Q, BM, RS, d->istr, k.sh0, k.nbuf, k.total_tiles > bx ? 1 : 0)) return VG_OK;
    const dim3 grid(bx, ncob, 1);
    if (Q == 1) launch_wpw<3, 1>(k, grid, lds, s);
    else if (Q == 2) launch_wpw<6, 2>(k, grid, lds, s);
    else if (R == 4) launch_wpw<4, 4>(k, grid, lds, s);
    else launch_wpw<6, 4>(k, grid, lds, s);
    vg_launch_reduce_partials(k.part, bx, k.dw_elems, dw, s);
    return vg_check_launch();
}
```

### van_gan_amd/ops.py

```python
from __future__ import annotations

import ctypes as C
import os
import math
from typing import List, Optional, Sequence, Tuple

import torch

from . import _lib
from ._lib import ACT_LRELU, ACT_NONE, ACT_RELU, PAD_REFLECT, PAD_ZERO, ActNormBwdDesc, ConvDesc, FinDesc, check, lib

IN_EPS = 1e-3
STRIPES = 8


def _p(t: Optional[torch.Tensor]) -> Optional[int]:
    return None if t is None else t.data_ptr()


def conv_variant(d) -> str:
    buf = C.create_string_buffer(512)
    _lib.lib.vg_conv3d_variant(C.byref(d), buf, 512)
    return buf.value.decode()

# ... 201 lines not shown
        self._saved = lib
        lib = _lib.lib_fp16()
        return self

    def __exit__(self, *exc):
        global lib
        lib = self._saved
        return False


class KernelProfile:

    def __init__(self):
        self.rows = {}
        self.vrows = {}
        self.lrows = {}

    def begin(self):
        e = torch.cuda.Event(enable_timing=True)
        e.record()
        return e

    def end(self, kind: str, flops: float, e0, nbytes: float = 0.0, variant: Optional[str] = None, layer: Optional[str] = None):
        e1 = torch.cuda.Event(enable_timing=True)
        e1.record()
        r = self.rows.setdefault(kind, [0, 0.0, [], 0.0])
        r[0] += 1; r[1] += flops; r[2].append((e0, e1)); r[3] += nbytes
        if variant:
            tmpl = variant.split('|')[0].replace(',bs1>', ',bs>').replace(',bs2>', ',bs>').replace(',bs1,pl>', ',bs,pl>').replace(',bs2,pl>', ',bs,pl>')
            v = self.vrows.setdefault((kind, tmpl), [0, 0.0, [], 0.0])
            v[0] += 1; v[1] += flops; v[2].append((e0, e1)); v[3] += nbytes
            if layer:
                v = self.lrows.setdefault((kind, layer, tmpl), [0, 0.0, [], 0.0])
                v[0] += 1; v[1] += flops; v[2].append((e0, e1)); v[3] += nbytes

    def by_layer(self):
        torch.cuda.synchronize()
        rows = []
        for (kind, layer, var), (n, fl, evs, nb) in self.lrows.items():
            ms = sum(a.elapsed_time(b) for a, b in evs)
            rows.append(dict(kind=kind, layer=layer, kernel=var, launches=n, ms=ms, gflop=fl / 1e9,
                             tflops=fl / (ms * 1e-3) / 1e12 if ms > 0 else None, algorithmic_bytes=nb))
        return sorted(rows, key=lambda r: -r['ms'])

    def summary(self):
        torch.cuda.synchronize()
        out = {}
        for k, (n, fl, evs, nb) in self.rows.items():
            ms = sum(a.elapsed_time(b) for a, b in evs)
            out[k] = dict(launches=n, flops=fl, ms=ms, bytes=nb)
        return out

    def by_variant(self):
        torch.cuda.synchronize()
        rows = []
        for (kind, var), (n, fl, evs, nb) in self.vrows.items():
            ms = sum(a.elapsed_time(b) for a, b in evs)
            rows.append(dict(kind=kind, kernel=var, launches=n, ms=ms, gflop=fl / 1e9, tflops=fl / (ms * 1e-3) / 1e12 if ms > 0 else None,
                             algorithmic_bytes=nb))
        return sorted(rows, key=lambda r: -r['ms'])


PROF: Optional[KernelProfile] = None

FUSE_CONCAT_NORM = os.environ.get('VG_FUSE_CONCAT_NORM', '1') != '0'
FUSE_CONCAT = os.environ.get('VG_FUSE_CONCAT', '1') != '0'
BSTAT = os.environ.get('VG_BSTAT', '1') != '0'
BSTAT_DMA = os.environ.get('VG_BSTAT_DMA', '0') != '0'
SIDE: Optional[bool] = None
_SIDE_OF = {}


def side_enable(device, on: bool = True):
    global SIDE
    SIDE = True if on else None


def _side_key(cur: torch.cuda.Stream):
    return (cur.device.index, cur.cuda_stream)


def _side_of(cur: torch.cuda.Stream) -> torch.cuda.Stream:
    sd = _SIDE_OF.get(_side_key(cur))
    if sd is None:
        sd = _SIDE_OF[_side_key(cur)] = torch.cuda.Stream(device=cur.device)
    return sd


class fork_side:

    def __init__(self):
        self.on = SIDE is not None and PROF is None and DRY is None
        self.cur = self.sd = self.ctx = None

    def __enter__(self):
        if self.on:
            self.cur = current_stream_obj()
            self.sd = _side_of(self.cur)
            wait_stream(self.sd, self.cur)
            self.ctx = torch.cuda.stream(self.sd)
            self.ctx.__enter__()
        return self

    def __exit__(self, *exc):
        if self.on:
            self.ctx.__exit__(*exc)
        return False

    def join(self):
        if self.on:
            wait_stream(self.cur, self.sd)


def side_event():
    if SIDE is None:
        return None
    sd = _SIDE_OF.get(_side_key(current_stream_obj()))
    return None if sd is None else record_event(sd)


def side_join():
    if SIDE is not None:
        cur = current_stream_obj()
        sd = _SIDE_OF.get(_side_key(cur))
        if sd is not None:
            wait_stream(cur, sd)


CONV_SCRATCH = {}
CONV_SCRATCH_BYTES = _lib.SCRATCH_CTR_BYTES + (int(os.environ.get('VG_CONV_SCRATCH_MB', '160')) << 20)
_SCRATCH_RETIRED = []


def conv_scratch(d: ConvDesc, s_: int, device=None):
    need = CONV_SCRATCH_BYTES
    if d.wlayout:
        need = max(need, int(lib.vg_conv3d_scratch_bytes(C.byref(d))))
    if DRY is not None:
        d.scratch, d.scratch_bytes = 1 << 20, need
        return
    key = (_DEV if device is None else device, s_)
    sc = CONV_SCRATCH.get(key)
    if sc is None or sc.numel() < need:
        dev = torch.device('cuda', key[0]) if key[0] is not None else torch.device('cuda')
        if sc is not None:
            _SCRATCH_RETIRED.append(sc)
        sc = torch.empty(need, dtype=torch.uint8, device=dev)
        sc[:_lib.SCRATCH_CTR_BYTES].zero_()
        CONV_SCRATCH[key] = sc
    d.scratch, d.scratch_bytes = sc.data_ptr(), sc.numel()


WGRAD_SCRATCH = {}
WGRAD_SCRATCH_ELEMS = 96 << 20


class Arena:
    ZPOOL = 8 << 20

    def __init__(self, nbytes: int, device):
        self.buf = torch.empty(nbytes + self.ZPOOL, dtype=torch.uint8, device=device)
        self.zpool = self.buf[nbytes:]
        self.buf = self.buf[:nbytes]
        self.off = 0
        self.zoff = 0
        self.peak = 0
        self.lazy_ok = True
        self.zpool.zero_()
        self._pair, self._pairs, self._pair_pos, self._full = None, {}, {}, {}
        self._cache, self._cpos, self._halves = [], 0, {}

    def pair_begin(self, key, slot: int):
        self._pair = (key, slot)
        self._pair_pos[key] = 0
        if slot == 0:
            self._pairs[key] = []

    def pair_end(self):
        self._pair = None

    def full_of(self, t):
        return None if t is None else self._full.get(t.data_ptr())

    def reset(self):
        self._pair, self._pairs, self._pair_pos, self._full = None, {}, {}, {}
        self._cpos = 0
        self.off = 0
        self.zmax = max(getattr(self, 'zmax', 0), self.zoff)
        nz = self.zoff if REC is None else self.ZPOOL
        if nz:
            zero_fill(self.zpool[:nz])
        self.zoff = 0

    _ESZ = {torch.float32: 4, torch.bfloat16: 2, torch.float16: 2, torch.int32: 4, torch.int64: 8, torch.uint8: 1, torch.float64: 8}

    def alloc(self, shape: Sequence[int], dtype: torch.dtype, zero: bool = False) -> torch.Tensor:
        shape = tuple(shape)
        if self._pair is not None and not zero:
            key, slot = self._pair
            if slot == 0:
                self._pair = None
                full = self.alloc((2 * shape[0],) + shape[1:], dtype)
                self._pair = (key, slot)
                self._pairs[key].append(full)
                self._full[full.data_ptr()] = full
                h = self._halves.get(full.data_ptr())
                if h is None or h[0] is not full:
                    h = self._halves[full.data_ptr()] = (full, full[:shape[0]], full[shape[0]:])
                return h[1]
            full = self._pairs[key][self._pair_pos[key]]
            self._pair_pos[key] += 1
            assert tuple(full.shape) == (2 * shape[0],) + shape[1:] and full.dtype == dtype, 'paired allocation sequences differ'
            return self._halves[full.data_ptr()][2]
        i, cache = self._cpos, self._cache
        if i < len(cache):
            e = cache[i]
            if e[0] == self.off and e[1] == self.zoff and e[2] == shape and e[3] is dtype and e[4] == zero:
                self._cpos = i + 1
                self.off, self.zoff = e[5], e[6]
                if self.off > self.peak:
                    self.peak = self.off
                if e[8] and DRY is None:
                    zero_fill(e[7])
                return e[7]
        off0, zoff0 = self.off, self.zoff
        t, big_zero = self._carve(shape, dtype, zero)
        entry = (off0, zoff0, shape, dtype, zero, self.off, self.zoff, t, big_zero)
        if i < len(cache):
            cache[i] = entry
            del cache[i + 1:]
        else:
            cache.append(entry)
        self._cpos = i + 1
        return t

    def _carve(self, shape, dtype, zero):
        n = int(math.prod(shape))
        nbytes = n * self._ESZ[dtype]
        if zero and nbytes <= 65536:
            zs = (self.zoff + 255) // 256 * 256
            if zs + nbytes <= self.ZPOOL:
                self.zoff = zs + nbytes
                return self.zpool[zs:zs + nbytes].view(dtype).view(*shape), False
        start = (self.off + 255) // 256 * 256
        if start + nbytes > self.buf.numel():
            raise MemoryError('arena exhausted: need %d more bytes' % (start + nbytes - self.buf.numel()))
        self.off = start + nbytes
        self.peak = max(self.peak, self.off)
        t = self.buf[start:start + nbytes].view(dtype).view(*shape)
        if zero and DRY is None:
            zero_fill(t)
        return t, bool(zero)

    def mark(self) -> int:
        return self.off

    def release(self, mark: int, defer: bool = False):
        if defer and self.lazy_ok and SIDE is not None and PROF is None and DRY is None:
            return
        side_join()
        self.off = mark


def same_pad_before(n: int, k: int, s: int) -> int:
    out = -(-n // s)
    return max((out - 1) * s + k - n, 0) // 2


class Src:

    def __init__(self, x0: torch.Tensor, dims: Tuple[int, int, int, int], c0: int, x1: Optional[torch.Tensor] = None,
                 c1: int = 0, shift0: int = 0, f32: bool = False, scale=None, shift=None, act: int = ACT_NONE,
                 noise=None, noise_pad: int = 0):
        self.x0, self.x1, self.c0, self.c1, self.shift0, self.f32 = x0, x1, c0, c1, shift0, f32
        self.N, self.D, self.H, self.W = dims
        self.scale, self.shift, self.act, self.noise, self.noise_pad = scale, shift, act, noise, noise_pad

    @property
    def C(self):
        return self.c0 + self.c1

    def recipe(self) -> dict:
        return dict(N=self.N, dims=(self.D, self.H, self.W), c0=self.c0, c1=self.c1, shift0=self.shift0, f32=bool(self.f32),
                    affine=self.scale is not None, act=self.act, noise=self.noise is not None, noise_pad=self.noise_pad)

    def fill(self, d: ConvDesc):
        d.src0, d.src1 = _p(self.x0), _p(self.x1)
        d.c_src0, d.c_src1, d.src0_shift, d.src_f32 = self.c0, self.c1, self.shift0, int(self.f32)
        d.N, d.D, d.H, d.W = self.N, self.D, self.H, self.W
        d.in_scale, d.in_shift, d.act = _p(self.scale), _p(self.shift), self.act
        d.noise, d.noise_pad = _p(self.noise), self.noise_pad


def _set_taps(d: ConvDesc, taps: List[Tuple[int, int, int]]):
    d.ntaps = len(taps)
    for i, (a, b, c) in enumerate(taps):
        d.tap_d[i], d.tap_h[i], d.tap_w[i] = a, b, c


def _ck_candidates(C_: int) -> List[int]:
    if C_ == 1:
        return [16]
    return [c for c in (64, 48, 32, 16) if C_ % c == 0]


class ConvLayer:

# ... 146 lines not shown
            return 0
        if sum(len(c['taps']) for c in self.d_classes) > _lib.VG_MAX_TAPS or len(self.d_classes) > 8:
            return 0
        for c in self.d_classes:
            c.setdefault('ck', 16)
        d = self._fused_desc(None, 1, None, False, probe=True, plan=False)
        return max(0, lib.vg_conv3d_dma_bn(C.byref(d)))

    def _pick_ck(self, C_, taps, istr, in_dims, iters, rows, wpack=0) -> int:
        d = ConvDesc()
        d.wpack, d.wpack_wmin = wpack, -self.pb[2]
        d.src0 = d.out = d.wpacked = 1 << 20
        d.c_src0, d.c_src1, d.N = C_, 0, 1
        d.D, d.H, d.W = in_dims
        d.istr, d.pad_mode, d.ostr = istr, PAD_ZERO, 1
        _set_taps(d, taps)
        d.OD, d.OH, d.OW = iters
        d.BD, d.BH, d.BW = iters
        d.Cout = rows
        d.f32 = self.f32
        if not wpack and not self.f32 and os.environ.get('VG_CONV_THIN2', '1') != '0' and lib.vg_conv3d_thin_np(C.byref(d)) == 2:
            return 16
        best, best_key = None, None
        plan = (C.c_int32 * 4)()
        for ck in _ck_candidates(C_):
            d.CK = ck
            if lib.vg_conv3d_plan(C.byref(d), plan) != 0:
                continue
            key = (plan[0] * plan[1], 1 if plan[2] <= 80 * 1024 else 0, ck)
            if ck < 32 and best is not None and best_key[0] >= key[0]:
                continue
            if best_key is None or key > best_key:
                best, best_key = ck, key
        if best is None:
            raise _lib.VgError('no LDS-feasible tile for %s' % self.name)
        return best

    def pack_items(self):
        T = self.f_T
        items = [(self.w, self.f_idx, self.f_wp, self.f_cin, self.cout, T, 0, self.f_ck, self.f32, self.f_bn)]
        for c in self.d_classes:
            items.append((self.w, c['idx'], c['wp'], self.cin, self.cout, len(c['taps']), 1, c['ck'], self.f32, self.d_bn))
        return items

    def enable_up(self, c_up: int):
        self.wp_up, self.c_up = None, 0
        if (self.f32 or self.k != 3 or self.stride != 1 or self.pad_mode != PAD_REFLECT or c_up <= 0 or c_up % 16 or c_up >= self.cin
                or self.f_bn or self.f_ck != 16 or self.wpack or os.environ.get('VG_CONV_THIN_UP', '0') == '0'):
            return
        self.c_up = c_up
        self.ctor = dict(self.ctor, c_up=c_up)
        self.wp_up = torch.zeros((c_up // 16) * 4 * self.cout * 192, dtype=self.f_wp.dtype, device=self.f_wp.device)

    def pack_up(self):
        if getattr(self, 'wp_up', None) is not None:
            check(lib.vg_pack_up_weights(_p(self.w), self.cin, self.cout, self.c_up, _p(self.wp_up), stream()), 'vg_pack_up_weights ' + self.name)

    def pack_cell(self):
        if getattr(self, 'cell', None) is not None:
            check(lib.vg_pack_cell_weights(_p(self.w), self.cout, _p(self.cell['wp']), stream()), 'vg_pack_cell_weights ' + self.name)

    def pack(self):
        T = self.f_T
        s = stream()
        self.pack_cell()
        self.pack_up()
        if self.f_bn:
            check(lib.vg_pack_weights_dma(_p(self.w), T, self.f_cin, self.cout, _p(self.f_idx), T, 0, self.f_bn, _p(self.f_wp), s), 'pack')
        else:
            check(lib.vg_pack_weights(_p(self.w), max(T, self.k ** 3 if not self.wpack else T), self.f_cin, self.cout, _p(self.f_idx), T, 0,
                                      self.f_ck, _p(self.f_wp), self.f32, s), 'pack')
        for c in self.d_classes:
            if self.d_bn:
                check(lib.vg_pack_weights_dma(_p(self.w), self.k ** 3, self.cin, self.cout, _p(c['idx']), len(c['taps']), 1, self.d_bn,
                                              _p(c['wp']), s), 'pack')
            else:
                check(lib.vg_pack_weights(_p(self.w), self.k ** 3, self.cin, self.cout, _p(c['idx']), len(c['taps']), 1, c['ck'],
                                          _p(c['wp']), self.f32, s), 'pack')

    def _fwd_desc(self, src: Src) -> ConvDesc:
        t = getattr(self, '_fwd_tmpl', None)
        if t is None:
            t = ConvDesc()
            t.istr, t.pad_mode = self.stride, self.pad_mode
            t.wpack, t.wpack_wmin = self.wpack, -self.pb[2]
            _set_taps(t, self.f_taps)
            t.OD, t.OH, t.OW = self.out_dims
            t.ostr, t.ooff_d, t.ooff_h, t.ooff_w = 1, 0, 0, 0
            t.BD, t.BH, t.BW = self.out_dims
            t.Cout, t.wpacked, t.CK = self.cout, _p(self.f_wp), self.f_ck
            t.f32 = self.f32
            t.wlayout = self.f_bn
            self._fwd_tmpl = t
        d = ConvDesc()
        C.memmove(C.byref(d), C.byref(t), C.sizeof(ConvDesc))
        src.fill(d)
        if getattr(self, 'wp_up', None) is not None and d.src0_shift and d.c_src0 == self.c_up:
            d.wpacked_up = _p(self.wp_up)
        return d

    def forward(self, src: Src, out: torch.Tensor, sums=None, res=None, res_scale=None, res_shift=None,
                tanh: bool = False, accumulate: bool = False, fin: Optional[FinDesc] = None, res_c1: bool = False):
        assert src.C == self.cin and (src.D, src.H, src.W) == tuple(self.in_dims)
        d = self._fwd_desc(src)
        if fin is not None:
            assert sums is not None
            d.fin = C.addressof(fin)
            d._fin_keep = fin
            if REC is not None:
                REC.keep.append(fin)
        d.bias = _p(self.b)
        d.res, d.res_scale, d.res_shift = _p(res), _p(res_scale), _p(res_shift)
        d.res_c1 = int(bool(res_c1) and res is not None)
        assert not d.res_c1 or res.dtype == torch.float32
        d.tanh_out = int(tanh)
        d.out, d.out_f32, d.accumulate = _p(out), int(out.dtype == torch.float32), int(bool(accumulate))
        d.out_sums = _p(sums)
        s_ = stream()
        conv_scratch(d, s_, out.device.index)
        if DRY is not None:
            DRY.tag = ('fwd', self.name)
            DRY.recipe = dict(kind='fwd', layer=self.ctor, src=src.recipe(), res=res is not None, res_c1=bool(res_c1), tanh=bool(tanh),
                              sums=sums is not None, out_f32=out.dtype == torch.float32,
                              fin=None if fin is None else dict(count=fin.count, jobs=tuple(
                                  dict(c_off=q.c_off, c_tot=q.c_tot, gamma=bool(q.gamma), beta=bool(q.beta), mult=bool(q.mult))
                                  for q in fin.job[:fin.njobs])))
        e0 = PROF.begin() if PROF is not None else None
        check(lib.vg_conv3d(C.byref(d), s_), 'vg_conv3d ' + self.name)
        if e0 is not None:
            esz = 4 if self.f32 else 2
            PROF.end('conv_fwd', 2.0 * src.N * math.prod(self.out_dims) * self.cout * self.cin * self.k ** 3, e0,
                     src.N * esz * (math.prod(self.in_dims) * self.cin + math.prod(self.out_dims) * self.cout), conv_variant(d), self.name)

    def wgrad(self, src: Src, dy: torch.Tensor, inline: bool = False):
        if SIDE is not None and PROF is None and DRY is None and not inline:
            cur = current_stream_obj()
            sd = _side_of(cur)
            wait_stream(sd, cur)
            self._wgrad(src, dy, sd.cuda_stream)
        else:
            self._wgrad(src, dy)

    def _wgrad(self, src: Src, dy: torch.Tensor, on_stream: Optional[int] = None):
        d = self._fwd_desc(src)
        s_ = stream() if on_stream is None else on_stream
        if DRY is not None:
            DRY.tag = ('wgrad', self.name)
            DRY.recipe = dict(kind='wgrad', layer=self.ctor, src=src.recipe(), dy_f32=dy.dtype == torch.float32)
        e0 = PROF.begin() if PROF is not None else None
        key = (dy.device, s_)
        sc = WGRAD_SCRATCH.get(key)
        if sc is None:
            sc = WGRAD_SCRATCH[key] = torch.empty(WGRAD_SCRATCH_ELEMS, dtype=torch.float32, device=dy.device)
        widx = self.f_idx_host if self.w_idx_host is None else self.w_idx_host
        check(lib.vg_conv3d_wgrad(C.byref(d), _p(dy), int(dy.dtype == torch.float32), widx, self.f_T,
                                  _p(self.gw_w), _p(self.gb), _p(sc), sc.numel() * 4, s_), 'vg_conv3d_wgrad ' + self.name)
        if e0 is not None:
            esz = 4 if self.f32 else 2
            vb = C.create_string_buffer(512)
            _lib.lib.vg_conv3d_wgrad_variant(C.byref(d), int(dy.dtype == torch.float32), widx, self.f_T, sc.numel() * 4, vb, 512)
            PROF.end('conv_wgrad', 2.0 * src.N * math.prod(self.out_dims) * self.cout * self.cin * self.k ** 3, e0,
                     src.N * esz * (math.prod(self.in_dims) * self.cin + math.prod(self.out_dims) * self.cout), vb.value.decode(), self.name)

    def _fused_desc(self, dy, N, out, accumulate, probe=False, plan=True):
        d = ConvDesc()
        dummy = 1 << 20
        d.src0, d.src1 = (dummy if probe else _p(dy)), None
        d.c_src0, d.c_src1, d.src0_shift = self.cout, 0, 0
        d.src_f32 = 0 if probe else int(dy.dtype == torch.float32 and self.cout == 1)
        d.N = N
        d.D, d.H, d.W = self.out_dims
        d.act, d.istr, d.pad_mode = ACT_NONE, 1, PAD_ZERO
        taps = [t for c in self.d_classes for t in c['taps']]
        _set_taps(d, taps)
        d.OD, d.OH, d.OW = [max(c['iters'][a] for c in self.d_classes) for a in range(3)]
        d.ostr = self.stride
        d.ooff_d, d.ooff_h, d.ooff_w = self.d_classes[0]['off']
        d.BD, d.BH, d.BW = self.buf_dims
        d.Cout, d.CK = self.cin, self.d_classes[0]['ck']
        d.f32 = self.f32
        d.nclass = len(self.d_classes)
        t0 = 0
        for i, c in enumerate(self.d_classes):
            d.cls_tap0[i] = t0
            t0 += len(c['taps'])
            d.cls_w[i] = dummy if probe else c['wp'].data_ptr()
            for a in range(3):
                d.cls_ooff[i][a] = c['off'][a]
                d.cls_iters[i][a] = c['iters'][a]
        d.cls_tap0[len(self.d_classes)] = t0
        d.wpacked = d.cls_w[0]
        d.wlayout = getattr(self, 'd_bn', 0)
        if probe and not plan:
            return d
        if probe:
            d.out = dummy
            plan = (C.c_int32 * 4)()
            ok = lib.vg_conv3d_plan(C.byref(d), plan) == 0
            self._last_plan = tuple(plan)
            return d if ok else None
        d.out, d.out_f32, d.accumulate = _p(out), int(out.dtype == torch.float32), int(accumulate)
        return d

    def dgrad(self, dy: torch.Tensor, N: int, out: torch.Tensor, accumulate: bool, bstat=None, bias=None) -> bool:
        use_bs = bstat is not None and BSTAT and not accumulate and not self.f32 and out.dtype in (torch.bfloat16, torch.float16) and bstat.norm \
            and ((len(self.d_classes) == 1 and self.stride == 1 and self.k == 3 and self.pad == 'reflect'
                  and self.d_classes[0]['ck'] == 16 and self.cin % 16 == 0 and self.cout % 16 == 0 and not bstat.mult)
                 or (bool(self.d_bn) and BSTAT_DMA))
        if DRY is not None:
            DRY.tag = ('dgrad', self.name)
            DRY.recipe = dict(kind='dgrad', layer=self.ctor, N=N, accumulate=bool(accumulate), dy_f32=dy.dtype == torch.float32,
                              out_f32=out.dtype == torch.float32, bstat=None if not use_bs else dict(
                                  cat=bool(bstat.x1), c_x0=bstat.c_x0, act=bstat.act, pad=bool(bstat.g_padded), mult=bool(bstat.mult),
                                  alias_n0=bstat.alias_n0, alias_shift=bstat.alias_shift))
        if REC is not None and use_bs:
            REC.keep.append(bstat)
        if self.d_fused:
            t = getattr(self, '_dg_tmpl', None)
            if t is None:
                t = self._dg_tmpl = self._fused_desc(dy, N, out, accumulate)
            d = ConvDesc()
            C.memmove(C.byref(d), C.byref(t), C.sizeof(ConvDesc))
            d.src0, d.N = _p(dy), N
            d.src_f32 = int(dy.dtype == torch.float32 and self.cout == 1)
            d.out, d.out_f32, d.accumulate = _p(out), int(out.dtype == torch.float32), int(accumulate)
            d.bstat = C.addressof(bstat) if use_bs else None
            d.bias = _p(bias)
            s_ = stream()
            conv_scratch(d, s_, out.device.index)
            e0 = PROF.begin() if PROF is not None else None
            check(lib.vg_conv3d(C.byref(d), s_), 'vg_conv3d(dgrad, fused classes) ' + self.name)
            if e0 is not None:
                PROF.end('conv_dgrad', 2.0 * N * math.prod(self.out_dims) * self.cin * self.cout * self.k ** 3, e0,
                         N * 2 * (math.prod(self.out_dims) * self.cout + math.prod(self.buf_dims) * self.cin), conv_variant(d), self.name)
            return use_bs
        for c in self.d_classes:
            t = c.get('tmpl')
            if t is None:
                t = ConvDesc()
                t.src1 = None
                t.c_src0, t.c_src1, t.src0_shift = self.cout, 0, 0
                t.D, t.H, t.W = self.out_dims
                t.act, t.istr, t.pad_mode = ACT_NONE, 1, PAD_ZERO
                _set_taps(t, c['taps'])
                t.OD, t.OH, t.OW = c['iters']
                t.ostr = self.stride
                t.ooff_d, t.ooff_h, t.ooff_w = c['off']
                t.BD, t.BH, t.BW = self.buf_dims
                t.Cout, t.wpacked, t.CK = self.cin, _p(c['wp']), c['ck']
                t.f32 = self.f32
                c['tmpl'] = t
            d = ConvDesc()
            C.memmove(C.byref(d), C.byref(t), C.sizeof(ConvDesc))
            d.src0, d.N = _p(dy), N
            d.src_f32 = int(dy.dtype == torch.float32 and self.cout == 1)
            d.out, d.out_f32, d.accumulate = _p(out), int(out.dtype == torch.float32), int(accumulate)
            d.bstat = C.addressof(bstat) if use_bs else None
            d.bias = _p(bias)
            s_ = stream()
            conv_scratch(d, s_, out.device.index)
            e0 = PROF.begin() if PROF is not None else None
            check(lib.vg_conv3d(C.byref(d), s_), 'vg_conv3d(dgrad) ' + self.name)
            if e0 is not None:
                PROF.end('conv_dgrad', 2.0 * N * math.prod(self.out_dims) * self.cin * self.cout * len(c['taps']), e0,
                         N * (4 if self.f32 else 2) * (math.prod(self.out_dims) * self.cout * len(c['taps']) / self.k ** 3
                                                       + math.prod(c['iters']) * self.cin), conv_variant(d), self.name)
        return use_bs


    def _sc_desc(self, dy, N):
        c = self.d_classes[0]
        d = ConvDesc()
        d.src1 = None
        d.c_src0, d.c_src1, d.src0_shift = self.cout, 0, 0
        d.D, d.H, d.W = self.out_dims
        d.act, d.istr, d.pad_mode = ACT_NONE, 1, PAD_ZERO
        _set_taps(d, c['taps'])
        d.OD, d.OH, d.OW = c['iters']
        d.ostr = self.stride
        d.ooff_d, d.ooff_h, d.ooff_w = c['off']
        d.BD, d.BH, d.BW = self.buf_dims
        d.Cout, d.wpacked, d.CK = self.cin, _p(c['wp']), c['ck']
        d.f32 = self.f32
        d.src0, d.N = _p(dy), N
        return d

    def dgrad_input(self, ar: 'Arena', dy: torch.Tensor, N: int, dx: torch.Tensor):
        assert self.cin == 1 and self.pad == 'reflect'
        if self.cell is None or DRY is not None or dy.dtype not in (torch.bfloat16, torch.float16):
            dp = ar.alloc((N,) + tuple(self.buf_dims) + (1,), self.dtype)
            self.dgrad(dy, N, dp, accumulate=False)
            actnorm_bwd(dp, True, None, (N,) + tuple(self.in_dims), 1, dx, act=ACT_NONE, norm=False, accumulate=False)
            return
        c = self.cell
        cells = ar.alloc((N,) + c['dims'] + (16,), self.dtype)
        t = c.get('tmpl')
        if t is None:
            t = c['tmpl'] = ConvDesc()
            t.src1 = None
            t.c_src0, t.c_src1, t.src0_shift = self.cout, 0, 0
            t.D, t.H, t.W = self.out_dims
            t.act, t.istr, t.pad_mode, t.ostr = ACT_NONE, 1, PAD_ZERO, 1
            _set_taps(t, c['taps'])
            t.OD, t.OH, t.OW = c['dims']
            t.BD, t.BH, t.BW = c['dims']
            t.Cout, t.wpacked, t.CK = 16, _p(c['wp']), 16
# ... 386 lines not shown
```

Before: 122.6 Mvoxels/s.

## Fold wgrad partial-slab reduction into last-arriving block via ticket counter

Weight-gradient kernels that write per-block partial slabs now take an atomic ticket at the end, and the last block to arrive sums all slabs and atomically adds the result into dw. This removes the separate reduce_partials launch when the slab footprint is small (up to 256 KB). The c1m LDS reduction also replaces per-lane shared-memory atomics with a serialized per-wave accumulate. The cost is a serial tail: one block performs the whole reduction. Correctness also depends on ticket counters living in a zeroed region at the front of the scratch buffer, which shrinks the usable scratch.

```diff
diff --git a/van_gan_amd/csrc/vg_c1k3.h b/van_gan_amd/csrc/vg_c1k3.h
--- a/van_gan_amd/csrc/vg_c1k3.h
+++ b/van_gan_amd/csrc/vg_c1k3.h
@@ -1,5 +1,6 @@
 #pragma once
 #include "vg_common.h"
+#include "vg_fold.h"
 
 struct C1K3 {
     const void* x; int x_f32; float sc, sf; int act, pad_mode;
@@ -27,7 +28,8 @@
     const void* w; int Ktot, CK;
     const float* bias; void* out; float* sums;
     const void* dy; float* dw; float* db; float* part;
+    unsigned* ticket;
     VgFin fin;
 };
 int c1m_fwd(const vg_conv_desc* d, hipStream_t s);
-int c1m_wgrad(const vg_conv_desc* d, const void* dy, int dy_f32, int T_total, float* dw, float* db, float* scratch, int64_t scratch_bytes, hipStream_t s);
+int c1m_wgrad(const vg_conv_desc* d, const void* dy, int dy_f32, int T_total, float* dw, float* db, float* scratch, int64_t scratch_bytes, unsigned* tickets, hipStream_t s);
diff --git a/van_gan_amd/csrc/vg_c1k3.hip b/van_gan_amd/csrc/vg_c1k3.hip
--- a/van_gan_amd/csrc/vg_c1k3.hip
+++ b/van_gan_amd/csrc/vg_c1k3.hip
@@ -242,15 +242,20 @@
         }
     }
     float* red = (float*)dyt;
-    __syncthreads();
-    for (int i = tid; i < MTS * NT * 256; i += 256) red[i] = 0.f;
-    __syncthreads();
-#pragma unroll
-    for (int mt = 0; mt < MTS; ++mt)
-#pragma unroll
-        for (int nt = 0; nt < NT; ++nt)
-#pragma unroll
-            for (int e = 0; e < 4; ++e) atomicAdd(&red[((mt * NT + nt) * 4 + e) * 64 + lane], acc[mt][nt][e]);
+    for (int w = 0; w < 4; ++w) {
+        __syncthreads();
+        if (wave == w) {
+#pragma unroll
+            for (int mt = 0; mt < MTS; ++mt)
+#pragma unroll
+                for (int nt = 0; nt < NT; ++nt)
+#pragma unroll
+                    for (int e = 0; e < 4; ++e) {
+                        float* r = red + ((mt * NT + nt) * 4 + e) * 64 + lane;
+                        *r = w == 0 ? acc[mt][nt][e] : *r + acc[mt][nt][e];
+                    }
+        }
+    }
     __syncthreads();
     float* slab = p.part ? p.part + ((size_t)blockIdx.y * gridDim.x + blockIdx.x) * (KS * KS * KS * C) : nullptr;
     for (int i = tid; i < MTS * NT * 256; i += 256) {
@@ -259,9 +264,11 @@
         const float v = red[i];
         if (r < G::NRT && e < KS) {
             const int idx = (r * KS + e) * C + co;
-            if (slab) slab[idx] = v; else atomicAdd(&p.dw[idx], v);
+            if (slab) vg_fold_store(slab + idx, v, p.ticket != nullptr); else atomicAdd(&p.dw[idx], v);
         } else if (r == G::NRT && e == 0 && p.db) atomicAdd(&p.db[co], v);
     }
+    if (p.ticket)
+        vg_fold_partials(p.part, gridDim.x * gridDim.y, KS * KS * KS * C, p.dw, p.ticket, 1, KS * KS * KS * C, true, [](int) { return (size_t)0; }, (int*)img);
 }
 }
 
@@ -313,7 +320,7 @@
     if (c.noise) hipLaunchKernelGGL((c1m_wgrad_kernel<S, KS, KS - 2, TH, NT, true>), grid, dim3(256), 0, s, c);
     else hipLaunchKernelGGL((c1m_wgrad_kernel<S, KS, KS - 2, TH, NT, false>), grid, dim3(256), 0, s, c);
 }
-int c1m_wgrad(const vg_conv_desc* d, const void* dy, int dy_f32, int T_total, float* dw, float* db, float* scratch, int64_t scratch_bytes, hipStream_t s) {
+int c1m_wgrad(const vg_conv_desc* d, const void* dy, int dy_f32, int T_total, float* dw, float* db, float* scratch, int64_t scratch_bytes, unsigned* tickets, hipStream_t s) {
     C1M c;
     if (dy_f32 || !vg_tune("C1M_WGRAD", 1) || !c1m_fill(d, c)) return 1;
     const int KS = d->wpack;
@@ -323,10 +330,11 @@
     const dim3 grid = c1m_grid(c, d->N, th, vg_tune("C1M_WGRAD_WGS", KS == 3 ? 2 : 1));
     const int nslab = (int)(grid.x * grid.y), dw_elems = KS * KS * KS * c.C;
     c.part = (nslab > 4 && scratch && (int64_t)nslab * dw_elems * 4 <= scratch_bytes && vg_tune("C1M_WGRAD_PART", 1)) ? scratch : nullptr;
+    c.ticket = c.part && vg_fold_pays(nslab, dw_elems, 1) ? tickets : nullptr;
     if (vg_dry("c1m_wgrad<%s,%d,%d,%d,n%d>|part%d", d->src_f32 ? "f32" : "bf16", KS, KS - 2, c.C / 16, c.noise ? 1 : 0, c.part ? 1 : 0)) return VG_OK;
     if (KS == 3) { if (d->src_f32) c1m_launch_wgrad<float, 3, 8, 1>(c, grid, s); else c1m_launch_wgrad<bf16_t, 3, 8, 1>(c, grid, s); }
     else { if (d->src_f32) c1m_launch_wgrad<float, 4, 4, 4>(c, grid, s); else c1m_launch_wgrad<bf16_t, 4, 4, 4>(c, grid, s); }
-    if (c.part) vg_launch_reduce_partials(c.part, nslab, dw_elems, dw, s);
+    if (c.part && !c.ticket) vg_launch_reduce_partials(c.part, nslab, dw_elems, dw, s);
     return vg_check_launch();
 }
 
diff --git a/van_gan_amd/csrc/vg_common.h b/van_gan_amd/csrc/vg_common.h
--- a/van_gan_amd/csrc/vg_common.h
+++ b/van_gan_amd/csrc/vg_common.h
@@ -144,11 +144,11 @@
 }
 int vg_pointwise_conv(const vg_conv_desc* d, hipStream_t s);
 int vg_pointwise_wgrad(const vg_conv_desc* d, const void* dy, int dy_f32, int T_total, float* dw, float* db, float* scratch,
-                       int64_t scratch_bytes, hipStream_t s);
+                       int64_t scratch_bytes, unsigned* tickets, hipStream_t s);
 int vg_wgrad_dma(const vg_conv_desc* d, const void* dy, int dy_f32, const int32_t* tap_idx_host, int T_total, float* dw, float* db,
-                 float* scratch, int64_t scratch_bytes, hipStream_t s);
+                 float* scratch, int64_t scratch_bytes, unsigned* tickets, hipStream_t s);
 int vg_wgrad_pw_dma(const vg_conv_desc* d, const void* dy, int dy_f32, int T_total, float* dw, float* db, float* scratch,
-                    int64_t scratch_bytes, hipStream_t s);
+                    int64_t scratch_bytes, unsigned* tickets, hipStream_t s);
 int vg_wgrad_thin(const vg_conv_desc* d, const void* dy, int dy_f32, const int32_t* tap_idx_host, int T_total, float* dw, float* db,
                   float* scratch, int64_t scratch_bytes, hipStream_t s);
 int vg_conv_dma(const vg_conv_desc* d, hipStream_t s, bool* did_stats = nullptr);
diff --git a/van_gan_amd/csrc/vg_fold.h b/van_gan_amd/csrc/vg_fold.h
--- /dev/null
+++ b/van_gan_amd/csrc/vg_fold.h
@@ -0,0 +1,86 @@
+#pragma once
+#include "vg_common.h"
+
+#define VG_FOLD_MAX_BYTES (256 << 10)
+#define VG_FOLD_MAX_COLS (VG_SCRATCH_CTR_BYTES / 4)
+
+int vg_fold_max_bytes();
+
+static inline bool vg_fold_pays(int nb, int64_t col_elems, int64_t ncols) {
+    return nb > 1 && ncols <= VG_FOLD_MAX_COLS && (int64_t)nb * col_elems * 4 <= (int64_t)vg_fold_max_bytes();
+}
+
+__device__ __forceinline__ void vg_fold_store(float* p, float v, bool fold) {
+    if (fold) __hip_atomic_store(p, v, __ATOMIC_RELAXED, __HIP_MEMORY_SCOPE_AGENT);
+    else *p = v;
+}
+
+template <class RowIdx>
+__device__ __forceinline__ void vg_fold_partials(const float* part, int nb, int dw_elems, float* dw, unsigned* ticket,
+                                                 int nrows, int len, bool vec, RowIdx row_idx, int* flag) {
+    asm volatile("s_waitcnt vmcnt(0)" ::: "memory");
+    __syncthreads();
+    if (threadIdx.x == 0) {
+        const unsigned old = __hip_atomic_fetch_add(ticket, 1u, __ATOMIC_RELAXED, __HIP_MEMORY_SCOPE_AGENT);
+        const int last = old == (unsigned)nb - 1u ? 1 : 0;
+        if (last) __hip_atomic_store(ticket, 0u, __ATOMIC_RELAXED, __HIP_MEMORY_SCOPE_AGENT);
+        *flag = last;
+    }
+    __syncthreads();
+    if (!*flag) return;
+    const unsigned stride = (unsigned)dw_elems * 4u;
+    const __amdgpu_buffer_rsrc_t rs = __builtin_amdgcn_make_buffer_rsrc((void*)part, 0, (int)min((size_t)nb * stride, (size_t)0x7fffffff), 0x00020000);
+    typedef __attribute__((ext_vector_type(4))) int i32x4;
+    if (vec) {
+        const int len4 = len >> 2;
+        for (int u = threadIdx.x; u < nrows * len4; u += blockDim.x) {
+            const int r = u / len4;
+            const size_t i = row_idx(r) + (size_t)(u - r * len4) * 4;
+            const unsigned off = (unsigned)i * 4u;
+            f32x4 s[4];
+#pragma unroll
+            for (int w = 0; w < 4; ++w) s[w] = (f32x4){0.f, 0.f, 0.f, 0.f};
+            int b = 0;
+            for (; b + 16 <= nb; b += 16) {
+                i32x4 v[16];
+#pragma unroll
+                for (int k = 0; k < 16; ++k) v[k] = __builtin_amdgcn_raw_buffer_load_b128(rs, off + (unsigned)(b + k) * stride, 0, 16);
+#pragma unroll
+                for (int k = 0; k < 16; ++k) s[k & 3] += __builtin_bit_cast(f32x4, v[k]);
+            }
+            for (; b < nb; b += 4) {
+                i32x4 v[4];
+#pragma unroll
+                for (int w = 0; w < 4; ++w) v[w] = __builtin_amdgcn_raw_buffer_load_b128(rs, off + (unsigned)min(b + w, nb - 1) * stride, 0, 16);
+#pragma unroll
+                for (int w = 0; w < 4; ++w) if (b + w < nb) s[w] += __builtin_bit_cast(f32x4, v[w]);
+            }
+            const f32x4 t = ((s[0] + s[1]) + s[2]) + s[3];
+#pragma unroll
+            for (int k = 0; k < 4; ++k) atomicAdd(dw + i + k, t[k]);
+        }
+    } else {
+        for (int u = threadIdx.x; u < nrows * len; u += blockDim.x) {
+            const int r = u / len;
+            const size_t i = row_idx(r) + (size_t)(u - r * len);
+            const unsigned off = (unsigned)i * 4u;
+            float s[4] = {0.f, 0.f, 0.f, 0.f};
+            int b = 0;
+            for (; b + 16 <= nb; b += 16) {
+                float v[16];
+#pragma unroll
+                for (int k = 0; k < 16; ++k) v[k] = __builtin_bit_cast(float, __builtin_amdgcn_raw_buffer_load_b32(rs, off + (unsigned)(b + k) * stride, 0, 16));
+#pragma unroll
+                for (int k = 0; k < 16; ++k) s[k & 3] += v[k];
+            }
+            for (; b < nb; b += 4) {
+                float v[4];
+#pragma unroll
+                for (int w = 0; w < 4; ++w) v[w] = __builtin_bit_cast(float, __builtin_amdgcn_raw_buffer_load_b32(rs, off + (unsigned)min(b + w, nb - 1) * stride, 0, 16));
+#pragma unroll
+                for (int w = 0; w < 4; ++w) if (b + w < nb) s[w] += v[w];
+            }
+            atomicAdd(dw + i, ((s[0] + s[1]) + s[2]) + s[3]);
+        }
+    }
+}
diff --git a/van_gan_amd/csrc/vg_pointwise.hip b/van_gan_amd/csrc/vg_pointwise.hip
--- a/van_gan_amd/csrc/vg_pointwise.hip
+++ b/van_gan_amd/csrc/vg_pointwise.hip
@@ -510,6 +510,7 @@
     int N, ID, IH, IW, OD, OH, OW, istr, SO;
     int gin, roles, rp, vpb;
     float* dw; float* db; float* part; int dw_elems;
+    unsigned* ticket;
 };
 
 __global__ __launch_bounds__(256) void pw_wgrad_cc_kernel(const PWW p) {
@@ -601,10 +602,12 @@
             const int rcg = ro % p.gin, rcob = ro / p.gin, co = rcob * 16 + i;
             if (ch < 8) {
                 const size_t idx = (size_t)(rcg * 8 + ch) * p.Cout + co;
-                if (slab) slab[idx] = sacc; else atomicAdd(&p.dw[idx], sacc);
+                if (slab) vg_fold_store(slab + idx, sacc, p.ticket != nullptr); else atomicAdd(&p.dw[idx], sacc);
             } else if (rcg == 0 && p.db) atomicAdd(&p.db[co], sacc);
         }
     }
+    if (p.ticket)
+        vg_fold_partials(p.part, gridDim.x * gridDim.y, p.dw_elems, p.dw, p.ticket, 1, p.dw_elems, true, [](int) { return (size_t)0; }, (int*)red);
 }
 
 template <typename T, bool MULTI_X>
@@ -958,7 +961,7 @@
 }
 
 int pw_wgrad_cc(const vg_conv_desc* d, const void* dy, int dy_f32, int T_total, float* dw, float* db, float* scratch,
-                int64_t scratch_bytes, hipStream_t s) {
+                int64_t scratch_bytes, unsigned* tickets, hipStream_t s) {
     if (!pw_enabled() || !vg_tune("PW_WGRAD_CC", 1)) return 1;
     if (T_total != 1 || d->ntaps != 1 || d->tap_d[0] || d->tap_h[0] || d->tap_w[0] || d->noise || d->wpack || d->nclass > 1) return 1;
     if (d->f32 || d->src_f32 || dy_f32 || d->in_scale || d->act != VG_ACT_NONE) return 1;
@@ -984,9 +987,10 @@
     if (b < 1) b = 1;
     const int nslab = (int)b * d->N;
     p.part = (nslab > 4 && scratch && (int64_t)nslab * p.dw_elems * 4 <= scratch_bytes) ? scratch : nullptr;
+    p.ticket = p.part && vg_fold_pays(nslab, p.dw_elems, 1) ? tickets : nullptr;
     if (vg_dry("pw_wgrad_cc<r%d>|part%d", p.roles, p.part ? 1 : 0)) return VG_OK;
     hipLaunchKernelGGL(pw_wgrad_cc_kernel, dim3((int)b, d->N), dim3(256), 0, s, p);
-    if (p.part) vg_launch_reduce_partials(p.part, nslab, p.dw_elems, dw, s);
+    if (p.part && !p.ticket) vg_launch_reduce_partials(p.part, nslab, p.dw_elems, dw, s);
     return vg_check_launch();
 }
 
@@ -1088,8 +1092,8 @@
 }
 
 int vg_pointwise_wgrad(const vg_conv_desc* d, const void* dy, int dy_f32, int T_total, float* dw, float* db, float* scratch,
-                       int64_t scratch_bytes, hipStream_t s) {
-    if (pw_enabled()) { const int mrc = c1m_wgrad(d, dy, dy_f32, T_total, dw, db, scratch, scratch_bytes, s); if (mrc <= 0) return mrc; }
+                       int64_t scratch_bytes, unsigned* tickets, hipStream_t s) {
+    if (pw_enabled()) { const int mrc = c1m_wgrad(d, dy, dy_f32, T_total, dw, db, scratch, scratch_bytes, tickets, s); if (mrc <= 0) return mrc; }
     if (pw_enabled() && T_total == 9 && !(dy_f32 && !d->f32)) {
         C1K3 c;
         if (c1k3_fill(d, c)) {
@@ -1111,7 +1115,7 @@
             return vg_check_launch();
         }
     }
-    { const int wrc = pw_wgrad_cc(d, dy, dy_f32, T_total, dw, db, scratch, scratch_bytes, s); if (wrc <= 0) return wrc; }
+    { const int wrc = pw_wgrad_cc(d, dy, dy_f32, T_total, dw, db, scratch, scratch_bytes, tickets, s); if (wrc <= 0) return wrc; }
     if (!pw_shape_ok(d) || T_total != 1) return 1;
     const int Cin = d->c_src0;
     PW p = {};
diff --git a/van_gan_amd/csrc/vg_wgrad.hip b/van_gan_amd/csrc/vg_wgrad.hip
--- a/van_gan_amd/csrc/vg_wgrad.hip
+++ b/van_gan_amd/csrc/vg_wgrad.hip
@@ -1,4 +1,5 @@
 #include "vg_gather.h"
+#include "vg_fold.h"
 
 struct WgradK {
     const void* dy; int dy_f32; int Cout;
@@ -8,6 +9,7 @@
     float* dw; float* db;
     int total_tiles, DYS;
     float* part; int dw_elems;
+    unsigned* tickets;
 };
 
 #ifndef VG_WGRAD_UB
@@ -250,7 +252,7 @@
             for (int e = 0; e < 4; ++e)
                 if (ci0 + e < g.Cw) {
                     const size_t i = ((size_t)tapsrc[tap] * g.Cw + ci0 + e) * p.Cout + co;
-                    if (p.part) p.part[(size_t)blockIdx.x * p.dw_elems + i] = acc[j][q][e];
+                    if (p.part) vg_fold_store(p.part + (size_t)blockIdx.x * p.dw_elems + i, acc[j][q][e], p.tickets != nullptr);
                     else atomicAdd(&p.dw[i], acc[j][q][e]);
                 }
         }
@@ -267,6 +269,14 @@
             if (co < p.Cout) atomicAdd(&p.db[co], red[tid]);
         }
     }
+    if (p.tickets) {
+        const int ci0 = cib * p.CIB, nci = min(p.CIB, g.Cw - ci0), co0 = cob * p.COB, nco = min(p.COB, p.Cout - co0);
+        const int* ts = tapsrc + tap0;
+        const int Cw = g.Cw, Cout = p.Cout;
+        const bool vec = !((nco | Cout | p.dw_elems) & 3);
+        vg_fold_partials(p.part, gridDim.x, p.dw_elems, p.dw, p.tickets + blockIdx.y, ntap_here * nci, nco, vec,
+                         [=](int r) { const int t = r / nci; return ((size_t)ts[t] * Cw + ci0 + (r - t * nci)) * Cout + co0; }, (int*)halo);
+    }
 }
 
 __global__ __launch_bounds__(256) void reduce_partials_kernel(const float* part, int nb, int n, float* dw) {
@@ -290,6 +300,14 @@
     if (w == 0 && i < n) atomicAdd(&dw[i], sm[0][lane] + sm[1][lane] + sm[2][lane] + sm[3][lane]);
 }
 
+int vg_fold_max_bytes() {
+#ifdef VG_DEBUG_ABLATE
+    const int kb = vg_tune("FOLD_KB", 0);
+    if (kb) return kb < 0 ? 0 : (kb > (1 << 20) ? 1 << 30 : kb << 10);
+#endif
+    return VG_FOLD_MAX_BYTES;
+}
+
 void vg_launch_reduce_partials(const float* part, int nb, int n, float* dw, hipStream_t s) {
     hipLaunchKernelGGL(reduce_partials_kernel, dim3((n + 63) / 64), dim3(256), 0, s, part, nb, n, dw);
 }
@@ -315,10 +333,13 @@
     if (!d || !dy || !dw || !tap_idx_host) return VG_EINVAL;
     if (d->Cout < 1 || (d->Cout != 1 && (d->Cout % 8))) return VG_EINVAL;
     if (dy_f32 && d->Cout != 1 && !d->f32) return VG_EINVAL;
+    unsigned* tickets = nullptr;
+    if (scratch && scratch_bytes > VG_SCRATCH_CTR_BYTES) { tickets = (unsigned*)scratch; scratch += VG_SCRATCH_CTR_BYTES / 4; scratch_bytes -= VG_SCRATCH_CTR_BYTES; }
+    else { scratch = nullptr; scratch_bytes = 0; }
     if (d->src0 && tap_idx_host[0] == 0) {
-        const int wrc = vg_wgrad_pw_dma(d, dy, dy_f32, T_total, dw, db, scratch, scratch_bytes, (hipStream_t)stream);
+        const int wrc = vg_wgrad_pw_dma(d, dy, dy_f32, T_total, dw, db, scratch, scratch_bytes, tickets, (hipStream_t)stream);
         if (wrc <= 0) return wrc;
-        const int prc = vg_pointwise_wgrad(d, dy, dy_f32, T_total, dw, db, scratch, scratch_bytes, (hipStream_t)stream);
+        const int prc = vg_pointwise_wgrad(d, dy, dy_f32, T_total, dw, db, scratch, scratch_bytes, tickets, (hipStream_t)stream);
         if (prc <= 0) return prc;
     }
     {
@@ -326,7 +347,7 @@
         if (trc <= 0) return trc;
     }
     {
-        const int drc = vg_wgrad_dma(d, dy, dy_f32, tap_idx_host, T_total, dw, db, scratch, scratch_bytes, (hipStream_t)stream);
+        const int drc = vg_wgrad_dma(d, dy, dy_f32, tap_idx_host, T_total, dw, db, scratch, scratch_bytes, tickets, (hipStream_t)stream);
         if (drc <= 0) return drc;
     }
     const int Cin = d->c_src0 + d->c_src1;
@@ -380,8 +401,9 @@
     const int wg_target = wg_env > 0 ? wg_env : (256 * per_cu < 384 ? 256 * per_cu : 384);
     int bx = wg_target / by; if (bx < 1) bx = 1; if (bx > k.total_tiles) bx = k.total_tiles;
     k.dw_elems = T_total * (d->wpack ? d->wpack : Cin) * d->Cout;
-    k.part = nullptr;
+    k.part = nullptr; k.tickets = nullptr;
     if (bx > 8 && scratch && (int64_t)bx * k.dw_elems * 4 <= scratch_bytes) k.part = scratch;
+    if (k.part && vg_fold_pays(bx, cdiv64(k.dw_elems, by), by)) k.tickets = tickets;
     const dim3 grid(bx, by, 1);
     hipStream_t s = (hipStream_t)stream;
     const int rw = (k.tpg * rows_per_tap + 3) / 4;
@@ -407,7 +429,7 @@
         else if (rw == 7) launch_wgrad<bf16_t, 7, 4>(g, k, grid, lds, s);
         else launch_wgrad<bf16_t, 6, 4>(g, k, grid, lds, s);
     }
-    if (k.part) {
+    if (k.part && !k.tickets) {
         hipLaunchKernelGGL(reduce_partials_kernel, dim3((k.dw_elems + 63) / 64), dim3(256), 0, s, k.part, bx, k.dw_elems, dw);
     }
     return vg_check_launch();
diff --git a/van_gan_amd/csrc/vg_wgrad_dma.hip b/van_gan_amd/csrc/vg_wgrad_dma.hip
--- a/van_gan_amd/csrc/vg_wgrad_dma.hip
+++ b/van_gan_amd/csrc/vg_wgrad_dma.hip
@@ -1,4 +1,5 @@
 #include "vg_dma_common.h"
+#include "vg_fold.h"
 
 __global__ __launch_bounds__(256) void materialize_kernel(const MatK p) {
     const int tid = threadIdx.x;
@@ -76,6 +77,7 @@
     int HD, HH, HW, HWE;
     int imgp, nA, nB, bufb, nbuf;
     float* dw; float* db; float* part; int dw_elems;
+    unsigned* tickets;
     unsigned m_imgp, m_hhw, m_hw, m_pl, m_tpn, m_tw, m_th, m_ncob;
     int co2l;
     const char* x0; const char* x1; int c0, c1, sh0;
@@ -356,7 +358,7 @@
 #pragma unroll
             for (int e = 0; e < 4; ++e) {
                 const size_t i = ((size_t)p.tap_src[tap] * p.Cin + ci0 + e) * p.Cout + co;
-                if (p.part) p.part[(size_t)blockIdx.x * p.dw_elems + i] = acc[j][q][e];
+                if (p.part) vg_fold_store(p.part + (size_t)blockIdx.x * p.dw_elems + i, acc[j][q][e], p.tickets != nullptr);
                 else atomicAdd(&p.dw[i], acc[j][q][e]);
             }
         }
@@ -374,6 +376,11 @@
         }
         __syncthreads();
         if (tid < CO) atomicAdd(&p.db[cob * CO + tid], red[tid]);
+    }
+    if (p.tickets) {
+        const int nci = p.PL * 16, ci0 = cib * nci, co0 = cob * CO;
+        vg_fold_partials(p.part, gridDim.x, p.dw_elems, p.dw, p.tickets + blockIdx.y, p.ntaps * nci, CO, true,
+                         [&](int r) { const int t = r / nci; return ((size_t)p.tap_src[t] * p.Cin + ci0 + (r - t * nci)) * p.Cout + co0; }, (int*)smem);
     }
     if (stamp && tid == 0) {
         asm volatile("s_waitcnt vmcnt(0)" ::: "memory");
@@ -398,7 +405,7 @@
 }
 
 int vg_wgrad_dma(const vg_conv_desc* d, const void* dy, int dy_f32, const int32_t* tap_idx_host, int T_total, float* dw, float* db,
-                 float* scratch, int64_t scratch_bytes, hipStream_t s) {
+                 float* scratch, int64_t scratch_bytes, unsigned* tickets, hipStream_t s) {
     if (!vg_tune("WGRAD_DMA", 1)) return 1;
     const int Cin = d->c_src0 + d->c_src1;
     if (d->f32 || dy_f32 || d->src_f32 || d->wpack || Cin < 16 || (Cin % 16) || (d->Cout % 16) || d->ntaps < 8 || d->ntaps > VG_MAX_TAPS) return 1;
@@ -521,6 +528,7 @@
     const int bx = best.bx;
     k.P = (const char*)scratch; k.dy = (const char*)dy;
     k.part = bx > 1 ? (float*)((char*)scratch + p_bytes) : nullptr;
+    k.tickets = k.part && vg_fold_pays(bx, dw_elems / columns, columns) ? tickets : nullptr;
     k.x0 = (const char*)d->src0; k.x1 = (const char*)d->src1; k.c0 = d->c_src0; k.c1 = d->c_src1; k.sh0 = d->src0_shift ? 1 : 0;
     k.D = d->D; k.H = d->H; k.W = d->W; k.pmin_d = mn[0]; k.pmin_h = mn[1]; k.pmin_w = mn[2];
     k.in_scale = d->in_scale; k.in_shift = d->in_shift;
@@ -540,7 +548,7 @@
     if (Q == 4) launch_wd<8, 4>(k, direct, grid, lds, s);
     else if (Q == 2) { if (Rsel == 4) launch_wd<4, 2>(k, direct, grid, lds, s); else launch_wd<8, 2>(k, direct, grid, lds, s); }
     else { if (Rsel == 4) launch_wd<4, 1>(k, direct, grid, lds, s); else if (Rsel == 8) launch_wd<8, 1>(k, direct, grid, lds, s); else launch_wd<12, 1>(k, direct, grid, lds, s); }
-    if (k.part) vg_launch_reduce_partials(k.part, bx, k.dw_elems, dw, s);
+    if (k.part && !k.tickets) vg_launch_reduce_partials(k.part, bx, k.dw_elems, dw, s);
     return vg_check_launch();
 }
 
@@ -553,6 +561,7 @@
     int ppp, nA, nB, bufb, nbuf;
     unsigned m_tpn, m_tw, m_th, m_ppp, m_ncob;
     float* dw; float* db; float* part; int dw_elems;
+    unsigned* tickets;
 };
 
 template <int R, int Q>
@@ -705,7 +714,7 @@
 #pragma unroll
                 for (int e = 0; e < 4; ++e) {
                     const size_t i = (size_t)(ci0 + e) * p.Cout + co;
-                    if (p.part) p.part[(size_t)blockIdx.x * p.dw_elems + i] = acc[j][q][e];
+                    if (p.part) vg_fold_store(p.part + (size_t)blockIdx.x * p.dw_elems + i, acc[j][q][e], p.tickets != nullptr);
                     else atomicAdd(&p.dw[i], acc[j][q][e]);
                 }
             }
@@ -723,6 +732,11 @@
         }
         __syncthreads();
         if (tid < CO) atomicAdd(&p.db[cob * CO + tid], red[tid]);
+    }
+    if (p.tickets) {
+        const int co0 = cob * CO;
+        vg_fold_partials(p.part, gridDim.x, p.dw_elems, p.dw, p.tickets + blockIdx.y, p.Cin, CO, true,
+                         [&](int r) { return (size_t)r * p.Cout + co0; }, (int*)smem);
     }
 }
 
@@ -737,7 +751,7 @@
 }
 
 int vg_wgrad_pw_dma(const vg_conv_desc* d, const void* dy, int dy_f32, int T_total, float* dw, float* db, float* scratch,
-                    int64_t scratch_bytes, hipStream_t s) {
+                    int64_t scratch_bytes, unsigned* tickets, hipStream_t s) {
     if (!vg_tune("WGRAD_PW_DMA", 1)) return 1;
     const int Cin = d->c_src0 + d->c_src1;
     if (d->f32 || dy_f32 || d->src_f32 || d->wpack || d->ntaps != 1 || T_total != 1 || d->tap_d[0] || d->tap_h[0] || d->tap_w[0]) return 1;
@@ -794,6 +808,7 @@
     const int64_t part_bytes = (int64_t)bx * k.dw_elems * 4;
     if (part_bytes > scratch_bytes) return 1;
     k.part = (float*)scratch;
+    k.tickets = vg_fold_pays(bx, k.dw_elems / ncob, ncob) ? tickets : nullptr;
     int lds = k.nbuf * k.bufb; { const int rl = 4 * R * Q * 1024; if (rl > lds) lds = rl; }
     if (vg_dry("wgrad_pw_dma<%d,%d>|bm%d|rs%d|s%d|u%d|nb%d|walk%d", R, Q, BM, RS, d->istr, k.sh0, k.nbuf, k.total_tiles > bx ? 1 : 0)) return VG_OK;
     const dim3 grid(bx, ncob, 1);
@@ -801,6 +816,6 @@
     else if (Q == 2) launch_wpw<6, 2>(k, grid, lds, s);
     else if (R == 4) launch_wpw<4, 4>(k, grid, lds, s);
     else launch_wpw<6, 4>(k, grid, lds, s);
-    vg_launch_reduce_partials(k.part, bx, k.dw_elems, dw, s);
+    if (!k.tickets) vg_launch_reduce_partials(k.part, bx, k.dw_elems, dw, s);
     return vg_check_launch();
 }
diff --git a/van_gan_amd/ops.py b/van_gan_amd/ops.py
--- a/van_gan_amd/ops.py
+++ b/van_gan_amd/ops.py
@@ -377,7 +377,7 @@
 
 
 WGRAD_SCRATCH = {}
-WGRAD_SCRATCH_ELEMS = 96 << 20
+WGRAD_SCRATCH_ELEMS = (96 << 20) + _lib.SCRATCH_CTR_BYTES // 4
 
 
 class Arena:
@@ -830,6 +830,8 @@
         sc = WGRAD_SCRATCH.get(key)
         if sc is None:
             sc = WGRAD_SCRATCH[key] = torch.empty(WGRAD_SCRATCH_ELEMS, dtype=torch.float32, device=dy.device)
+            if DRY is None:
+                check(_lib.lib.vg_memset_zero(_p(sc), _lib.SCRATCH_CTR_BYTES, s_), 'vg_memset_zero')
         widx = self.f_idx_host if self.w_idx_host is None else self.w_idx_host
         check(lib.vg_conv3d_wgrad(C.byref(d), _p(dy), int(dy.dtype == torch.float32), widx, self.f_T,
                                   _p(self.gw_w), _p(self.gb), _p(sc), sc.numel() * 4, s_), 'vg_conv3d_wgrad ' + self.name)
```

Result: no change. 122.7 Mvoxels/s (median of 3 runs) (+0.1%).
